# acbull/pyHGT

Hardware: NVIDIA H100
Metric: HGTConv fwd edges/sec (higher is better)
Workload: dtype f32

## Files before the change

include/hgt_b200.h:

```cpp
#ifndef HGT_B200_H
#define HGT_B200_H

#include <stddef.h>
#include <stdint.h>

#ifdef __cplusplus
extern "C" {
#endif

#define HGT_RTE_MAX_LEN 240

const char* hgt_last_error(void);
int hgt_abi_version(void);
uint64_t hgt_kernel_launches(void);


int hgt_plan_workspace_bytes(int64_t n_nodes, int64_t n_edges, size_t* out_bytes);

int hgt_plan_nodes(const int64_t* node_type, int64_t n_nodes, int32_t num_types,
                   int32_t* rank, int32_t* perm, int32_t* type_count, int32_t* sorted_flag,
                   void* workspace, size_t workspace_bytes, void* stream);

int hgt_plan_edges_sort(const int64_t* edge_index, const int64_t* edge_type, const int64_t* node_type,
                        const int32_t* rank, int64_t n_nodes, int64_t n_edges,
// ... 72 lines not shown

typedef struct {
  int64_t out_off;
  int64_t ld;
} hgt_lin_cblock;

int hgt_fold_weights(const float* const* wq, const float* const* bq,
                     const float* const* wk, const float* const* bk,
                     const float* const* wv, const float* const* bv,
                     const float* relation_att, const float* relation_msg, const float* relation_pri,
                     int32_t num_types, int32_t num_relations, int32_t n_heads, int32_t d_in, int32_t d_out,
                     int32_t n_pairs, const int32_t* pair_type, const int32_t* pair_rel,
                     const int32_t* cat_row0, const int32_t* q_row0,
                     float* w_cat, float* b_cat, void* stream);

int hgt_concat_linears(const float* const* w, const float* const* b, int32_t num_types,
                       int32_t rows, int32_t cols, float* w_cat, float* b_cat, void* stream);


int hgt_typed_linear_workspace_bytes(const hgt_lin_group* h_groups, int32_t n_groups, int32_t K,
                                     int32_t cb_width, int32_t impl, size_t* out_bytes);
int hgt_typed_linear(const float* A, int64_t lda, const float* W, const float* bias, int32_t K,
                     int32_t cb_width, const hgt_lin_group* groups, const hgt_lin_group* h_groups,
                     int32_t n_groups, const hgt_lin_cblock* cblocks, float* out, int32_t impl,
                     void* workspace, size_t workspace_bytes, void* stream);
int hgt_typed_linear_presplit_workspace_bytes(const hgt_lin_group* h_groups, int32_t n_groups, int32_t K,
                                              int32_t cb_width, size_t* out_bytes);
int hgt_typed_linear_presplit(const void* a_hi, const void* a_lo, const float* W, const float* bias, int32_t K,
                              int32_t cb_width, const hgt_lin_group* groups, const hgt_lin_group* h_groups,
                              int32_t n_groups, const hgt_lin_cblock* cblocks, float* out,
                              void* workspace, size_t workspace_bytes, void* stream);
int hgt_typed_linear_bf16(const float* A, int64_t lda, const float* W, const float* bias, int32_t K,
                          int32_t cb_width, const hgt_lin_group* groups, const hgt_lin_group* h_groups,
                          int32_t n_groups, const hgt_lin_cblock* cblocks, void* out, int32_t impl,
                          void* workspace, size_t workspace_bytes, void* stream);
int hgt_typed_linear_presplit_bf16(const void* a_hi, const void* a_lo, const float* W, const float* bias, int32_t K,
                                   int32_t cb_width, const hgt_lin_group* groups, const hgt_lin_group* h_groups,
                                   int32_t n_groups, const hgt_lin_cblock* cblocks, void* out,
                                   void* workspace, size_t workspace_bytes, void* stream);
int hgt_typed_linear_bf16a(const void* A, int64_t lda, const float* W, const float* bias, int32_t K, int32_t cb_width,
                           const hgt_lin_group* groups, const hgt_lin_group* h_groups, int32_t n_groups,
                           const hgt_lin_cblock* cblocks, float* out, int32_t impl, void* workspace,
                           size_t workspace_bytes, void* stream);

int hgt_typed_linear_t24(const float* A, int64_t lda, const float* W, const float* bias, int32_t K,
                         int32_t cb_width, const hgt_lin_group* groups, const hgt_lin_group* h_groups,
                         int32_t n_groups, const hgt_lin_cblock* cblocks, float* out, int64_t t24_off, void* out24,
                         int32_t impl, void* workspace, size_t workspace_bytes, void* stream);
int hgt_typed_linear_presplit_t24(const void* a_hi, const void* a_lo, const float* W, const float* bias, int32_t K,
                                  int32_t cb_width, const hgt_lin_group* groups, const hgt_lin_group* h_groups,
                                  int32_t n_groups, const hgt_lin_cblock* cblocks, float* out, int64_t t24_off,
                                  void* out24, void* workspace, size_t workspace_bytes, void* stream);


int hgt_edge_workspace_bytes(int32_t n_split_tiles, int32_t d, int32_t n_heads, size_t* out_bytes);
int hgt_edge_forward(const float* q, const float* kv, const float* kvr,
                     const int32_t* row_ptr, const int32_t* kv_row, const int32_t* rte_row,
                     const int32_t* csr_eid, const int32_t* tiles, int32_t n_tiles, int32_t n_split_tiles,
                     const int32_t* hubs, int32_t n_hubs,
                     int64_t n_nodes, int64_t n_edges, int32_t d, int32_t n_heads, int32_t apply_gelu,
                     float* agg_out, float* att_out, float* stats_out, void* g_hi, void* g_lo,
                     void* workspace, size_t workspace_bytes, int32_t variant, const int32_t* d_tile_counts,
                     const int32_t* type_row0, int32_t num_types, const int32_t* type_active, void* stream);

int hgt_edge_backward(const float* q, const float* kv, const float* kvr, const float* agg, const float* dagg,
                      const float* stats, const int32_t* row_ptr, const int32_t* kv_row, const int32_t* rte_row,
                      const int32_t* tiles, int32_t n_tiles, int64_t n_nodes, int32_t d, int32_t n_heads,
                      int64_t kv_rows_total, int64_t kvr_rows_total,
                      float* dq, float* dkv, float* dkvr, void* workspace, size_t workspace_bytes,
                      const int32_t* d_tile_counts, void* stream);

int hgt_edge_backward_det_workspace_bytes(int32_t n_split_dst, int32_t n_split_rows, int32_t d, size_t* out_bytes);
int hgt_edge_backward_dst(const float* q, const float* kv, const float* kvr, const float* agg, const float* dagg,
                          const float* stats, const int32_t* row_ptr, const int32_t* kv_row, const int32_t* rte_row,
                          const int32_t* tiles, int32_t n_tiles, int32_t n_split, const int32_t* hubs, int32_t n_hubs,
                          int64_t n_nodes, int32_t d, int32_t n_heads, float* dq, float* D,
                          void* workspace, size_t workspace_bytes, const int32_t* d_tile_counts, void* stream);
int hgt_edge_backward_rows(const float* q, const float* dagg, const float* stats, const float* D, const float* own,
                           const float* oth, const int32_t* src_ptr, const int32_t* src_dst, const int32_t* src_oth,
                           int32_t n_rows, int64_t own_rows_total, const int32_t* tiles, int32_t n_tiles,
                           int32_t n_split, const int32_t* hubs, int32_t n_hubs, int32_t d, int32_t n_heads,
                           float* grad, void* workspace, size_t workspace_bytes, const int32_t* d_tile_counts,
                           void* stream);

int hgt_edge_forward_bf16(const float* q, const void* kv, const void* kvr,
                          const int32_t* row_ptr, const int32_t* kv_row, const int32_t* rte_row,
                          const int32_t* csr_eid, const int32_t* tiles, int32_t n_tiles, int32_t n_split_tiles,
                          const int32_t* hubs, int32_t n_hubs,
                          int64_t n_nodes, int64_t n_edges, int32_t d, int32_t n_heads, int32_t apply_gelu,
                          float* agg_out, float* att_out, float* stats_out, void* g_hi, void* g_lo,
                          void* workspace, size_t workspace_bytes, int32_t variant, const int32_t* d_tile_counts,
                          const int32_t* type_row0, int32_t num_types, const int32_t* type_active, void* stream);
int hgt_edge_forward_t24(const float* q, const void* kv, const void* kvr,
                         const int32_t* row_ptr, const int32_t* kv_row, const int32_t* rte_row,
                         const int32_t* csr_eid, const int32_t* tiles, int32_t n_tiles, int32_t n_split_tiles,
                         const int32_t* hubs, int32_t n_hubs,
                         int64_t n_nodes, int64_t n_edges, int32_t d, int32_t n_heads, int32_t apply_gelu,
                         float* agg_out, float* att_out, float* stats_out, void* g_hi, void* g_lo,
                         void* workspace, size_t workspace_bytes, int32_t variant, const int32_t* d_tile_counts,
                         const int32_t* type_row0, int32_t num_types, const int32_t* type_active, void* stream);
int hgt_edge_backward_bf16(const float* q, const void* kv, const void* kvr, const float* agg, const float* dagg,
                           const float* stats, const int32_t* row_ptr, const int32_t* kv_row, const int32_t* rte_row,
                           const int32_t* tiles, int32_t n_tiles, int64_t n_nodes, int32_t d, int32_t n_heads,
                           int64_t kv_rows_total, int64_t kvr_rows_total,
                           float* dq, float* dkv, float* dkvr, void* workspace, size_t workspace_bytes,
                           const int32_t* d_tile_counts, void* stream);
int hgt_edge_backward_dst_bf16(const float* q, const void* kv, const void* kvr, const float* agg, const float* dagg,
                               const float* stats, const int32_t* row_ptr, const int32_t* kv_row,
                               const int32_t* rte_row, const int32_t* tiles, int32_t n_tiles, int32_t n_split,
                               const int32_t* hubs, int32_t n_hubs, int64_t n_nodes, int32_t d, int32_t n_heads,
                               float* dq, float* D, void* workspace, size_t workspace_bytes,
                               const int32_t* d_tile_counts, void* stream);
int hgt_edge_backward_rows_bf16(const float* q, const float* dagg, const float* stats, const float* D, const void* own,
                                const void* oth, const int32_t* src_ptr, const int32_t* src_dst,
                                const int32_t* src_oth, int32_t n_rows, int64_t own_rows_total, const int32_t* tiles,
                                int32_t n_tiles, int32_t n_split, const int32_t* hubs, int32_t n_hubs, int32_t d,
                                int32_t n_heads, float* grad, void* workspace, size_t workspace_bytes,
                                const int32_t* d_tile_counts, void* stream);

int hgt_edge_att_grad_workspace_bytes(int32_t n_split, int32_t n_heads, size_t* out_bytes);
int hgt_edge_att_grad_prep(const float* att, const float* datt, const int32_t* csr_eid, const int32_t* row_ptr,
                           const int32_t* tiles, int32_t n_tiles, int32_t n_split, const int32_t* hubs, int32_t n_hubs,
                           int64_t n_nodes, int32_t n_heads, float* c_att, float* datt_csr, void* workspace,
                           size_t workspace_bytes, const int32_t* d_tile_counts, void* stream);
int hgt_edge_backward_att(const float* q, const float* kv, const float* kvr, const float* agg, const float* dagg,
                          const float* stats, const float* datt_csr, const float* c_att, const int32_t* row_ptr,
                          const int32_t* kv_row, const int32_t* rte_row, const int32_t* tiles, int32_t n_tiles,
                          int64_t n_nodes, int32_t d, int32_t n_heads, int64_t kv_rows_total, int64_t kvr_rows_total,
                          float* dq, float* dkv, float* dkvr, void* workspace, size_t workspace_bytes,
                          const int32_t* d_tile_counts, void* stream);
int hgt_edge_backward_dst_att(const float* q, const float* kv, const float* kvr, const float* agg, const float* dagg,
                              const float* stats, const float* datt_csr, const float* c_att, const int32_t* row_ptr,
                              const int32_t* kv_row, const int32_t* rte_row, const int32_t* tiles, int32_t n_tiles,
                              int32_t n_split, const int32_t* hubs, int32_t n_hubs, int64_t n_nodes, int32_t d,
                              int32_t n_heads, float* dq, float* D, void* workspace, size_t workspace_bytes,
                              const int32_t* d_tile_counts, void* stream);
int hgt_edge_backward_rows_att(const float* q, const float* dagg, const float* stats, const float* D,
                               const float* datt_csr, const float* own, const float* oth, const int32_t* src_ptr,
                               const int32_t* src_dst, const int32_t* src_oth, const int32_t* src_pos, int32_t n_rows,
                               int64_t own_rows_total, const int32_t* tiles, int32_t n_tiles, int32_t n_split,
                               const int32_t* hubs, int32_t n_hubs, int32_t d, int32_t n_heads, float* grad,
                               void* workspace, size_t workspace_bytes, const int32_t* d_tile_counts, void* stream);
int hgt_edge_backward_att_bf16(const float* q, const void* kv, const void* kvr, const float* agg, const float* dagg,
                               const float* stats, const float* datt_csr, const float* c_att, const int32_t* row_ptr,
                               const int32_t* kv_row, const int32_t* rte_row, const int32_t* tiles, int32_t n_tiles,
                               int64_t n_nodes, int32_t d, int32_t n_heads, int64_t kv_rows_total,
                               int64_t kvr_rows_total, float* dq, float* dkv, float* dkvr, void* workspace,
                               size_t workspace_bytes, const int32_t* d_tile_counts, void* stream);
int hgt_edge_backward_dst_att_bf16(const float* q, const void* kv, const void* kvr, const float* agg, const float* dagg,
                                   const float* stats, const float* datt_csr, const float* c_att,
                                   const int32_t* row_ptr, const int32_t* kv_row, const int32_t* rte_row,
                                   const int32_t* tiles, int32_t n_tiles, int32_t n_split, const int32_t* hubs,
                                   int32_t n_hubs, int64_t n_nodes, int32_t d, int32_t n_heads, float* dq, float* D,
// ... 354 lines not shown
```

pyhgt_b200/_lib.py:

```python
import ctypes
import os

import numpy as np

HERE = os.path.dirname(os.path.abspath(__file__))
LIB_PATH = os.path.join(HERE, "libhgt_b200.so")

_c = ctypes
_p = _c.c_void_p
_i32 = _c.c_int32
_i64 = _c.c_int64
_sz = _c.c_size_t
_f32 = _c.c_float

SIGNATURES = {
    "hgt_abi_version": [],
    "hgt_plan_workspace_bytes": [_i64, _i64, _c.POINTER(_sz)],
    "hgt_plan_nodes": [_p, _i64, _i32, _p, _p, _p, _p, _p, _sz, _p],
    "hgt_plan_edges_sort": [_p, _p, _p, _p, _i64, _i64, _i32, _i32, _p, _p, _p, _p, _p, _sz, _p],
    "hgt_plan_edges_fill": [_p, _p, _p, _p, _p, _p, _i64, _i64, _i32, _i32, _p, _p, _p, _i32, _i32, _p, _p, _p, _p],
    "hgt_plan_tiles": [_p, _i64, _i64, _i32, _i32, _p, _i64, _p, _i64, _p, _c.POINTER(_i32), _p, _sz, _p],
    "hgt_gather_rows": [_p, _p, _i64, _i32, _p, _p],
    "hgt_halo_pull": [_c.c_uint64, _p, _p, _i64, _i32, _i64, _p, _p],
    "hgt_halo_pull_split": [_c.c_uint64, _p, _p, _p, _i64, _i32, _i32, _i64, _p, _p, _p, _p],
    "hgt_halo_push_split": [_p, _p, _p, _p, _i64, _i32, _i32, _i64, _c.c_uint64, _c.c_uint64, _p, _p],
    "hgt_fold_weights": [_p, _p, _p, _p, _p, _p, _p, _p, _p, _i32, _i32, _i32, _i32, _i32, _i32, _p, _p, _p, _p,
                         _p, _p, _p],
    "hgt_concat_linears": [_p, _p, _i32, _i32, _i32, _p, _p, _p],
    "hgt_typed_linear_workspace_bytes": [_p, _i32, _i32, _i32, _i32, _c.POINTER(_sz)],
    "hgt_typed_linear": [_p, _i64, _p, _p, _i32, _i32, _p, _p, _i32, _p, _p, _i32, _p, _sz, _p],
    "hgt_edge_workspace_bytes": [_i32, _i32, _i32, _c.POINTER(_sz)],
    "hgt_edge_forward": [_p, _p, _p, _p, _p, _p, _p, _p, _i32, _i32, _p, _i32, _i64, _i64, _i32, _i32, _i32, _p, _p,
                         _p, _p, _p, _p, _sz, _i32, _p, _p, _i32, _p, _p],
    "hgt_typed_linear_presplit_workspace_bytes": [_p, _i32, _i32, _i32, _c.POINTER(_sz)],
    "hgt_typed_linear_presplit": [_p, _p, _p, _p, _i32, _i32, _p, _p, _i32, _p, _p, _p, _sz, _p],
    "hgt_edge_backward": [_p, _p, _p, _p, _p, _p, _p, _p, _p, _p, _i32, _i64, _i32, _i32, _i64, _i64, _p, _p, _p, _p, _sz,
                          _p, _p],
    "hgt_typed_linear_bwd_workspace_bytes": [_p, _i32, _p, _i32, _i32, _i64, _i64, _i32, _i32, _i32, _c.POINTER(_sz)],
    "hgt_typed_linear_bwd": [_p, _p, _p, _i64, _p, _i64, _p, _p, _p, _i32, _i32, _p, _p, _i32, _p, _p, _i32, _p, _p, _p,
                             _i32, _p, _sz, _p],
    "hgt_act_split": [_p, _i64, _i64, _i32, _i32, _p, _p, _p, _p],
    "hgt_update_backward": [_p, _p, _p, _p, _i32, _p, _p, _p, _p, _i64, _i32, _p, _p, _p, _p, _p, _p],
    "hgt_fold_backward": [_p, _p, _p, _p, _p, _p, _p, _p, _p, _i32, _i32, _i32, _i32, _i32, _i32, _p, _p, _p, _p, _p, _p,
                          _p, _p, _p, _p, _p],
    "hgt_conv_workspace_bytes": [_p, _c.POINTER(_sz)],
    "hgt_conv_forward": [_p, _p, _sz, _p],
    "hgt_update_epilogue": [_p, _p, _p, _i32, _p, _p, _p, _p, _p, _i64, _i32, _p, _p, _p, _p],
    "hgt_plan_dst_end": [_p, _p, _p, _i64, _i32, _p, _p],
    "hgt_update_epilogue_dst": [_p, _p, _p, _i32, _p, _p, _p, _p, _p, _p, _i64, _i32, _p, _p, _p, _p],
    "hgt_plan_source_index": [_p, _p, _p, _i64, _i64, _i32, _p, _p, _p, _p, _sz, _p],
    "hgt_plan_source_index_pos": [_p, _p, _p, _i64, _i64, _i32, _p, _p, _p, _p, _p, _sz, _p],
    "hgt_edge_backward_det_workspace_bytes": [_i32, _i32, _i32, _c.POINTER(_sz)],
    "hgt_edge_backward_dst": [_p, _p, _p, _p, _p, _p, _p, _p, _p, _p, _i32, _i32, _p, _i32, _i64, _i32, _i32, _p, _p, _p,
                              _sz, _p, _p],
    "hgt_edge_backward_rows": [_p, _p, _p, _p, _p, _p, _p, _p, _p, _i32, _i64, _p, _i32, _i32, _p, _i32, _i32, _i32, _p,
                               _p, _sz, _p, _p],
    "hgt_typed_linear_bwd_det_workspace_bytes": [_p, _i32, _p, _i32, _i32, _i64, _i64, _i32, _i32, _i32,
                                                 _c.POINTER(_sz)],
    "hgt_typed_linear_bwd_det": [_p, _p, _p, _i64, _p, _i64, _p, _p, _p, _i32, _i32, _p, _p, _i32, _p, _p, _i32, _p, _p,
                                 _p, _i32, _p, _sz, _p],
    "hgt_update_backward_det_workspace_bytes": [_i64, _i32, _i32, _c.POINTER(_sz)],
    "hgt_update_backward_det": [_p, _p, _p, _p, _i32, _p, _p, _p, _p, _i64, _i32, _p, _p, _p, _p, _p, _p, _sz, _p],
    "hgt_fold_backward_det": [_p, _p, _p, _p, _p, _p, _p, _p, _p, _i32, _i32, _i32, _i32, _i32, _i32, _p, _p, _p, _p, _p,
                              _p, _p, _p, _p, _p, _p],
    "hgt_typed_linear_bf16": [_p, _i64, _p, _p, _i32, _i32, _p, _p, _i32, _p, _p, _i32, _p, _sz, _p],
    "hgt_typed_linear_presplit_bf16": [_p, _p, _p, _p, _i32, _i32, _p, _p, _i32, _p, _p, _p, _sz, _p],
    "hgt_typed_linear_t24": [_p, _i64, _p, _p, _i32, _i32, _p, _p, _i32, _p, _p, _i64, _p, _i32, _p, _sz, _p],
    "hgt_typed_linear_presplit_t24": [_p, _p, _p, _p, _i32, _i32, _p, _p, _i32, _p, _p, _i64, _p, _p, _sz, _p],
    "hgt_edge_forward_bf16": [_p, _p, _p, _p, _p, _p, _p, _p, _i32, _i32, _p, _i32, _i64, _i64, _i32, _i32, _i32, _p, _p,
                              _p, _p, _p, _p, _sz, _i32, _p, _p, _i32, _p, _p],
    "hgt_edge_forward_t24": [_p, _p, _p, _p, _p, _p, _p, _p, _i32, _i32, _p, _i32, _i64, _i64, _i32, _i32, _i32, _p, _p,
                             _p, _p, _p, _p, _sz, _i32, _p, _p, _i32, _p, _p],
    "hgt_edge_backward_bf16": [_p, _p, _p, _p, _p, _p, _p, _p, _p, _p, _i32, _i64, _i32, _i32, _i64, _i64, _p, _p, _p, _p,
                               _sz, _p, _p],
    "hgt_edge_backward_dst_bf16": [_p, _p, _p, _p, _p, _p, _p, _p, _p, _p, _i32, _i32, _p, _i32, _i64, _i32, _i32, _p, _p,
                                   _p, _sz, _p, _p],
    "hgt_edge_backward_rows_bf16": [_p, _p, _p, _p, _p, _p, _p, _p, _p, _i32, _i64, _p, _i32, _i32, _p, _i32, _i32, _i32,
                                    _p, _p, _sz, _p, _p],
    "hgt_edge_att_grad_workspace_bytes": [_i32, _i32, _c.POINTER(_sz)],
    "hgt_edge_att_grad_prep": [_p, _p, _p, _p, _p, _i32, _i32, _p, _i32, _i64, _i32, _p, _p, _p, _sz, _p, _p],
    "hgt_edge_backward_att": [_p, _p, _p, _p, _p, _p, _p, _p, _p, _p, _p, _p, _i32, _i64, _i32, _i32, _i64, _i64, _p, _p,
                              _p, _p, _sz, _p, _p],
    "hgt_edge_backward_dst_att": [_p, _p, _p, _p, _p, _p, _p, _p, _p, _p, _p, _p, _i32, _i32, _p, _i32, _i64, _i32, _i32,
                                  _p, _p, _p, _sz, _p, _p],
    "hgt_edge_backward_rows_att": [_p, _p, _p, _p, _p, _p, _p, _p, _p, _p, _p, _i32, _i64, _p, _i32, _i32, _p, _i32, _i32,
                                   _i32, _p, _p, _sz, _p, _p],
    "hgt_edge_backward_att_bf16": [_p, _p, _p, _p, _p, _p, _p, _p, _p, _p, _p, _p, _i32, _i64, _i32, _i32, _i64, _i64, _p,
                                   _p, _p, _p, _sz, _p, _p],
    "hgt_edge_backward_dst_att_bf16": [_p, _p, _p, _p, _p, _p, _p, _p, _p, _p, _p, _p, _i32, _i32, _p, _i32, _i64, _i32,
                                       _i32, _p, _p, _p, _sz, _p, _p],
    "hgt_edge_backward_rows_att_bf16": [_p, _p, _p, _p, _p, _p, _p, _p, _p, _p, _p, _i32, _i64, _p, _i32, _i32, _p, _i32,
                                        _i32, _i32, _p, _p, _sz, _p, _p],
    "hgt_gsample_batch_add_budget_workspace_bytes": [_i32, _i64, _i32, _i64, _c.POINTER(_sz)],
    "hgt_gsample_batch_add_budget": [_p, _p, _p, _i32, _p, _p, _p, _p, _i64, _p, _i64, _i32, _i64, _i64, _p, _p, _sz,
                                     _p],
    "hgt_gsample_batch_select_workspace_bytes": [_i32, _i64, _c.POINTER(_sz)],
    "hgt_gsample_batch_select": [_p, _p, _p, _p, _i64, _i64, _i64, _p, _p, _p, _p, _p, _sz, _p],
    "hgt_gsample_rebuild_workspace_bytes": [_i64, _c.POINTER(_sz)],
    "hgt_gsample_batch_rebuild_count": [_p, _p, _i32, _p, _p, _i64, _i64, _p, _p, _p, _p, _p, _sz, _p],
    "hgt_gsample_batch_rebuild_write": [_p, _p, _i32, _p, _p, _p, _p, _p, _p, _p, _i64, _p, _i64, _p, _i32, _p, _p, _p,
                                        _p, _p, _p, _p],
    "hgt_host_register": [_p, _sz, _c.POINTER(_p)],
    "hgt_host_unregister": [_p],
    "hgt_gsample_gather_features_bf16": [_p, _i32, _p, _p, _i64, _p, _p],
    "hgt_gsample_batch_rebuild_count_host": [_p, _p, _i32, _p, _p, _i64, _i64, _p, _p, _i64, _p, _p, _p, _p, _p, _sz,
                                             _p],
    "hgt_gsample_batch_rebuild_write_host": [_p, _p, _i32, _p, _p, _p, _p, _p, _p, _p, _i64, _p, _i64, _p, _i64, _p,
                                             _i32, _p, _p, _p, _p, _p, _p, _p],
    "hgt_gsample_hash_insert_seeds": [_p, _i64, _p, _p, _p, _p, _p, _p],
    "hgt_gsample_hash_add_budget": [_p, _p, _p, _i32, _p, _p, _p, _p, _i64, _p, _i64, _i32, _i64, _i64, _p, _p, _sz,
                                    _p],
    "hgt_gsample_hash_select_workspace_bytes": [_i32, _i64, _c.POINTER(_sz)],
    "hgt_gsample_hash_select": [_p, _p, _p, _p, _i64, _i64, _i64, _p, _p, _p, _p, _p, _sz, _p],
    "hgt_gsample_hash_rebuild_count": [_p, _p, _i32, _p, _p, _i64, _i64, _p, _p, _p, _p, _p, _sz, _p],
    "hgt_gsample_hash_rebuild_write": [_p, _p, _i32, _p, _p, _p, _p, _p, _p, _p, _i64, _p, _i64, _p, _i32, _p, _p, _p,
                                       _p, _p, _p, _p],
    "hgt_gsample_hash_rebuild_count_host": [_p, _p, _i32, _p, _p, _i64, _i64, _p, _p, _i64, _p, _p, _p, _p, _p, _sz,
                                            _p],
    "hgt_gsample_hash_rebuild_write_host": [_p, _p, _i32, _p, _p, _p, _p, _p, _p, _p, _i64, _p, _i64, _p, _i64, _p,
                                            _i32, _p, _p, _p, _p, _p, _p, _p],
    "hgt_merge_batches": [_p, _i32, _i32, _p, _p, _i64, _i64, _i64, _i32, _p, _p, _p, _p, _p, _p, _p],
    "hgt_gsample_gather_rows_bf16": [_p, _i32, _p, _p, _i64, _p, _p],
    "hgt_merge_batches_bf16": [_p, _i32, _i32, _p, _p, _i64, _i64, _i64, _i32, _p, _p, _p, _p, _p, _p, _p],
    "hgt_typed_linear_bf16a": [_p, _i64, _p, _p, _i32, _i32, _p, _p, _i32, _p, _p, _i32, _p, _sz, _p],
    "hgt_typed_linear_bwd_bf16a": [_p, _i64, _p, _i64, _i32, _i32, _p, _p, _i32, _p, _p, _p, _i32, _p, _sz, _p],
# ... 35 lines not shown
    _fields_ = ([(n, ctypes.c_int64) for n in _I64] + [(n, ctypes.c_int32) for n in _I32] +
                [(n, ctypes.c_void_p) for n in _PTR])


LIN_GROUP_DTYPE = np.dtype([("a_row0", "<i8"), ("m", "<i8"), ("w_row0", "<i4"), ("n_cblocks", "<i4"),
                            ("cb_first", "<i4"), ("has_bias", "<i4")])
LIN_CBLOCK_DTYPE = np.dtype([("out_off", "<i8"), ("ld", "<i8")])
assert LIN_GROUP_DTYPE.itemsize == 32 and LIN_CBLOCK_DTYPE.itemsize == 16

_lib = None


class HgtError(RuntimeError):
    pass


def load():
    global _lib
    if _lib is not None:
        return _lib
    if not os.path.exists(LIB_PATH):
        raise HgtError("libhgt_b200.so not found at %s — run `python -m pyhgt_b200.build` "
                       "(or __graft_entry__.build()); there is no CPU fallback" % LIB_PATH)
    lib = ctypes.CDLL(LIB_PATH)
    lib.hgt_last_error.restype = _c.c_char_p
    lib.hgt_last_error.argtypes = []
    for name, args in SIGNATURES.items():
        fn = getattr(lib, name)
        fn.restype = _c.c_int
        fn.argtypes = args
    lib.hgt_kernel_launches.restype = _c.c_uint64
    lib.hgt_kernel_launches.argtypes = []
    lib.hgt_conv_args_size.restype = _c.c_uint64
    lib.hgt_conv_args_size.argtypes = []
    lib.hgt_sampler_budget_update.restype = _c.c_int64
    lib.hgt_sampler_budget_update.argtypes = [_p, _p, _i64, _i64, _i64, _i64, _i64, _p, _p, _p, _p, _p, _p, _p]
    lib.hgt_sampler_add_budget.restype = _c.c_int64
    lib.hgt_sampler_add_budget.argtypes = [_p, _p, _i64, _p, _c.c_int32, _p, _c.c_int32, _i64, _p, _p, _i64, _i64, _p]
    _lib = lib
    return lib


def check(rc, what):
    if rc != 0:
        msg = load().hgt_last_error()
        raise HgtError("%s failed (code %d): %s" % (what, rc, msg.decode() if msg else "?"))


def call(name, *args):
    lib = load()
    check(getattr(lib, name)(*args), name)


def kernel_launches():
    return int(load().hgt_kernel_launches())


def ptr(t):
    return None if t is None else t.data_ptr()
```

pyhgt_b200/conv.py:

```python
import ctypes
import math

import torch
import torch.nn as nn
import torch.nn.functional as F

from . import _lib
from . import plan as _plan


def glorot(tensor):
    if tensor is not None:
        a = math.sqrt(6.0 / (tensor.size(-2) + tensor.size(-1)))
        tensor.data.uniform_(-a, a)


class RelTemporalEncoding(nn.Module):

    def __init__(self, n_hid, max_len=240, dropout=0.2):
        super().__init__()
        position = torch.arange(0., max_len).unsqueeze(1)
        div_term = torch.exp(torch.arange(0, n_hid, 2) * -(math.log(10000.0) / n_hid))
        emb = nn.Embedding(max_len, n_hid)
        emb.weight.data[:, 0::2] = torch.sin(position * div_term) / math.sqrt(n_hid)
        emb.weight.data[:, 1::2] = torch.cos(position * div_term) / math.sqrt(n_hid)
        emb.requires_grad = False
        self.emb = emb
        self.lin = nn.Linear(n_hid, n_hid)

    def forward(self, x, t):
        return x + self.lin(self.emb(t))


def _stream():
    return torch.cuda.current_stream().cuda_stream


_TABLE_SUFFIX = {torch.float32: "", torch.bfloat16: "_bf16", torch.uint8: "_t24"}


def _output_rows(rows, d, dev, lt, out_map):
    if lt.type_active_dev is not None and out_map is None:
        return torch.zeros((rows, d), dtype=torch.float32, device=dev)
    return torch.empty((rows, d), dtype=torch.float32, device=dev)


def _split_hint(node_inp, x, N, d_in, impl):
    hint = getattr(node_inp, "_hgt_split", None)
    if (hint is None or hint[2] != node_inp._version or x is not node_inp or tuple(hint[0].shape) != (N, d_in)
            or d_in % 16 or d_in < 64 or (hint[1] is None and impl != 3)):
        return None
    return (hint[0], None if impl == 3 else hint[1])


class _PointerTable:

    def __init__(self):
        self.key = None
        self.dev = None

    def get(self, tensors, device):
        key = tuple(t.data_ptr() for t in tensors) + (str(device),)
        if key != self.key:
            if torch.device(device).type == "cuda" and torch.cuda.is_current_stream_capturing():
                raise _lib.HgtError("a parameter moved while a CUDA graph was being captured: run the step once eagerly "
                                    "(warm-up) so the pointer tables match the parameters the graph will use")
            self.dev = torch.tensor([t.data_ptr() for t in tensors], dtype=torch.int64).to(device)
            self.key = key
        return self.dev


class HGTConv(nn.Module):
    keep_att = True
    recompute_tables = False
    fused_dropout = False
    edge_variant = 0
    linear_impl = 0
    event_sink = None
    _has_skip = True
    emit_split = False
    fused_call = True

    def __init__(self, in_dim, out_dim, num_types, num_relations, n_heads, dropout=0.2, use_norm=True,
                 use_RTE=True, **kwargs):
        super().__init__()
        self.in_dim = in_dim
        self.out_dim = out_dim
        self.num_types = num_types
        self.num_relations = num_relations
        self.total_rel = num_types * num_relations * num_types
        self.n_heads = n_heads
# ... 9 lines not shown
        self.a_linears = nn.ModuleList()
        self.norms = nn.ModuleList()
        for _ in range(num_types):
            self.k_linears.append(nn.Linear(in_dim, out_dim))
            self.q_linears.append(nn.Linear(in_dim, out_dim))
            self.v_linears.append(nn.Linear(in_dim, out_dim))
            self.a_linears.append(nn.Linear(out_dim, out_dim))
            if use_norm:
                self.norms.append(nn.LayerNorm(out_dim))
        self.relation_pri = nn.Parameter(torch.ones(num_relations, self.n_heads))
        self.relation_att = nn.Parameter(torch.Tensor(num_relations, n_heads, self.d_k, self.d_k))
        self.relation_msg = nn.Parameter(torch.Tensor(num_relations, n_heads, self.d_k, self.d_k))
        if self._has_skip:
            self.skip = nn.Parameter(torch.ones(num_types))
        self.drop = nn.Dropout(dropout)
        if self.use_RTE:
            self.emb = RelTemporalEncoding(in_dim)
        glorot(self.relation_att)
        glorot(self.relation_msg)
        self._ptr_tables = {}

    def __repr__(self):
        return '{}(in_dim={}, out_dim={}, num_types={}, num_types={})'.format(
            self.__class__.__name__, self.in_dim, self.out_dim, self.num_types, self.num_relations)

    def __getstate__(self):
        state = self.__dict__.copy()
        state.pop("_args_cache", None)
        state["_ptr_tables"] = {}
        if state.get("att") is not None:
            state["att"] = state["att"].detach()
        return state

    def _ptrs(self, name, tensors, device):
        tab = self._ptr_tables.get(name)
        if tab is None:
            tab = self._ptr_tables[name] = _PointerTable()
        return tab.get(tensors, device)

    @staticmethod
    def _stage(name):
        class _T:
            def __enter__(self_):
                self_.on = HGTConv.event_sink is not None
                if self_.on:
                    self_.a, self_.b = torch.cuda.Event(enable_timing=True), torch.cuda.Event(enable_timing=True)
                    self_.a.record()
            def __exit__(self_, *exc):
                if self_.on:
                    self_.b.record()
                    HGTConv.event_sink.append((name, self_.a, self_.b))
        return _T()

    def _typed_linear(self, a, lda, w, bias, k, width, table, out, impl, st, out32=None, t24_off=0):
        g_dev, g_host, n_g, c_dev = table
        ws_bytes = ctypes.c_size_t()
        _lib.call("hgt_typed_linear_workspace_bytes", g_host.ctypes.data, n_g, k, width, impl, ctypes.byref(ws_bytes))
        ws = torch.empty(max(ws_bytes.value, 1), dtype=torch.uint8, device=out.device)
        outs = (_lib.ptr(out32), t24_off, out.data_ptr()) if out.dtype == torch.uint8 else (out.data_ptr(),)
        fn = "hgt_typed_linear_bf16a" if a.dtype == torch.bfloat16 else "hgt_typed_linear" + _TABLE_SUFFIX[out.dtype]
        _lib.call(fn, a.data_ptr(), lda, w.data_ptr(), _lib.ptr(bias), k, width, g_dev.data_ptr(),
                  g_host.ctypes.data, n_g, c_dev.data_ptr(), *outs, impl, ws.data_ptr(), ws.numel(), st)

    def _check_inputs(self, node_inp, edge_time):
        if node_inp.device.type != "cuda":
            raise _lib.HgtError("pyhgt_b200.HGTConv runs on CUDA tensors only (got %s): there is no CPU "
                                "fallback" % node_inp.device)
        if node_inp.dtype != torch.float32:
            raise ValueError("node_inp must be float32 (the reference is fp32 throughout), got %s" % node_inp.dtype)
        if node_inp.dim() != 2 or node_inp.shape[1] != self.in_dim:
            raise ValueError("node_inp must be [N, %d], got %s" % (self.in_dim, tuple(node_inp.shape)))
        if self.in_dim != self.out_dim:
            raise ValueError("HGTConv needs in_dim == out_dim for the skip connection (conv.py:131)")
        if self.use_RTE and edge_time is None:
            raise ValueError("use_RTE=True needs edge_time (conv.py:91-92)")
        if self.out_dim % self.n_heads != 0:
            raise ValueError("out_dim=%d is not divisible by n_heads=%d" % (self.out_dim, self.n_heads))

    def forward(self, node_inp, node_type, edge_index, edge_type, edge_time=None):
        self._check_inputs(node_inp, edge_time)
        if torch.is_grad_enabled() and (node_inp.requires_grad or any(p.requires_grad for p in self.parameters())):
            from .autograd import hgt_conv_autograd
            return hgt_conv_autograd(self, node_inp, node_type, edge_index, edge_type, edge_time)
        out, att, _ = self._forward_impl(node_inp, node_type, edge_index, edge_type, edge_time,
                                         want_att=self.keep_att, save=False)
        self.att = att
        return out

    def _forward_view(self, node_inp, view, edge_time):
        self._check_inputs(node_inp, edge_time)
        self.att = None
        if torch.is_grad_enabled() and (node_inp.requires_grad or any(p.requires_grad for p in self.parameters())):
            from .autograd import hgt_conv_autograd
            return hgt_conv_autograd(self, node_inp, None, None, None, None, active=view.active,
                                     kv_runs=view.kv_runs, plan=view.plan, want_att=False)
        out, _, _ = self._forward_impl(node_inp, None, None, None, None, want_att=False, save=False,
                                       active_per_type=view.active, kv_runs=view.kv_runs, plan=view.plan)
        return out

    def _forward_fused(self, node_inp, node_type, edge_index, edge_type, edge_time, want_att,
                       active_per_type=None, out_map=None, out_rows=None, x_split=None, kv_runs=None, plan=None, impl=None,
                       dst=False):
        if impl is None:
            impl = self.linear_impl
        dev = node_inp.device
        d_in, d, H, T, R = self.in_dim, self.out_dim, self.n_heads, self.num_types, self.num_relations
        if plan is None:
            plan = _plan.get_plan(node_type, edge_index, edge_type, edge_time if self.use_RTE else None, T, R)
        N, E = plan.n_nodes, plan.n_edges
        if node_inp.shape[0] != N:
            raise ValueError("node_inp has %d rows but node_type has %d" % (node_inp.shape[0], N))
        lt = _plan.layer_tables(plan, d_in, d, active_per_type, kv_runs, dst)
        tabs = [self._ptrs("wq", [l.weight for l in self.q_linears], dev),
# ... 113 lines not shown
                          drop_seed(o.device).data_ptr(), p_fused, st)
            elif lt.type_dst_dev is not None:
                _lib.call("hgt_update_epilogue_dst", o.data_ptr(), x_sorted.data_ptr(), plan.type_row0_dev.data_ptr(), T,
                          self.skip.data_ptr(), _lib.ptr(norm_w), _lib.ptr(norm_b), perm_ptr, lt.type_dst_dev.data_ptr(),
                          c["ba_cat"].data_ptr(), N, d, out.data_ptr(), _lib.ptr(o_hi), _lib.ptr(o_lo), st)
            else:
                _lib.call("hgt_update_epilogue", o.data_ptr(), x_sorted.data_ptr(), plan.type_row0_dev.data_ptr(), T,
                          self.skip.data_ptr(), _lib.ptr(norm_w), _lib.ptr(norm_b), perm_ptr,
                          _lib.ptr(lt.type_active_dev), N, d, out.data_ptr(), _lib.ptr(o_hi), _lib.ptr(o_lo), st)
        if o_hi is not None:
            out._hgt_split = (o_hi, o_lo, out._version)
        return out, c["att"], (c if save else None)

    def _core(self, node_inp, node_type, edge_index, edge_type, edge_time, want_att, save, active_per_type,
              gelu_before_a, x_split=None, kv_runs=None, bf16=False, plan=None, impl=None, dst=False):
        if impl is None:
            impl = self.linear_impl
        one = impl == 3
        dev = node_inp.device
        d_in, d = self.in_dim, self.out_dim
        H, T, R = self.n_heads, self.num_types, self.num_relations
        st = _stream()
        if plan is None:
            plan = _plan.get_plan(node_type, edge_index, edge_type, edge_time if self.use_RTE else None, T, R)
        N, E, P = plan.n_nodes, plan.n_edges, plan.n_pairs
        if node_inp.shape[0] != N:
            raise ValueError("node_inp has %d rows but node_type has %d" % (node_inp.shape[0], N))
        lt = _plan.layer_tables(plan, d_in, d, active_per_type, kv_runs, dst)
        f32 = dict(dtype=torch.float32, device=dev)
        x = node_inp.contiguous()
        if x_split is None and plan.sorted_types and impl != 1:
            x_split = _split_hint(node_inp, x, N, d_in, impl)
        if plan.sorted_types:
            x_sorted = x
        else:
            with self._stage("gather_rows"):
                x_sorted = torch.empty_like(x)
                _lib.call("hgt_gather_rows", x.data_ptr(), plan.perm.data_ptr(), N, d_in, x_sorted.data_ptr(), st)

        w_cat = torch.empty((max(lt.cat_rows, 1), d_in), **f32)
        b_cat = torch.empty(max(lt.cat_rows, 1), **f32)
        wq = self._ptrs("wq", [l.weight for l in self.q_linears], dev)
        bq = self._ptrs("bq", [l.bias for l in self.q_linears], dev)
        wk = self._ptrs("wk", [l.weight for l in self.k_linears], dev)
        bk = self._ptrs("bk", [l.bias for l in self.k_linears], dev)
        wv = self._ptrs("wv", [l.weight for l in self.v_linears], dev)
        bv = self._ptrs("bv", [l.bias for l in self.v_linears], dev)
        _lib.call("hgt_fold_weights", wq.data_ptr(), bq.data_ptr(), wk.data_ptr(), bk.data_ptr(), wv.data_ptr(),
                  bv.data_ptr(), self.relation_att.data_ptr(), self.relation_msg.data_ptr(),
                  self.relation_pri.data_ptr(), T, R, H, d_in, d, P, plan.pair_type_dev.data_ptr(),
                  plan.pair_rel_dev.data_ptr(), lt.cat_row0_dev.data_ptr(), lt.q_row0_dev.data_ptr(),
                  w_cat.data_ptr(), b_cat.data_ptr(), st)

        t24 = not save and not bf16 and d % 8 == 0
        tab_dtype = torch.bfloat16 if bf16 else torch.uint8 if t24 else torch.float32
        row_len = 2 * d * (3 if t24 else 1)
        proj = None
        if bf16:
            q_tab = torch.empty(N * d, **f32)
            kv_tab = torch.empty((plan.kv_rows + 1) * row_len, dtype=tab_dtype, device=dev)
            calls = ((lt.q_groups, q_tab, None), (lt.kv_groups, kv_tab, None))
        elif t24:
            q_buf = torch.empty(lt.kv_off, **f32)
            q_tab = q_buf[lt.q_off:lt.q_off + N * d]
            kv_tab = torch.empty((plan.kv_rows + 1) * row_len, dtype=tab_dtype, device=dev)
            calls = ((lt.proj_groups, kv_tab, q_buf),)
        else:
            proj = torch.empty(lt.proj_elems, **f32)
            q_tab = proj[lt.q_off:lt.q_off + N * d]
            kv_tab = proj[lt.kv_off:]
            calls = ((lt.proj_groups, proj, None),)
        kv_tab[plan.kv_rows * row_len:].zero_()
        with self._stage("proj_linear"):
            xs = x_split if plan.sorted_types else None
            for tab, out, out32 in calls:
                if xs is None:
                    self._typed_linear(x_sorted, d_in, w_cat, b_cat, d_in, d, tab, out, impl, st, out32, lt.kv_off)
                    continue
                g_dev, g_host, n_g, c_dev = tab
                wsb = ctypes.c_size_t()
                _lib.call("hgt_typed_linear_presplit_workspace_bytes", g_host.ctypes.data, n_g, d_in, d,
                          ctypes.byref(wsb))
                ws1 = torch.empty(max(wsb.value, 1), dtype=torch.uint8, device=dev)
                outs = (out32.data_ptr(), lt.kv_off, out.data_ptr()) if t24 else (out.data_ptr(),)
                _lib.call("hgt_typed_linear_presplit" + _TABLE_SUFFIX[out.dtype], xs[0].data_ptr(),
                          None if one else _lib.ptr(xs[1]), w_cat.data_ptr(), b_cat.data_ptr(), d_in, d, g_dev.data_ptr(),
                          g_host.ctypes.data, n_g, c_dev.data_ptr(), *outs, ws1.data_ptr(), ws1.numel(), st)
        kvr = None
        if self.use_RTE:
            rt = torch.empty((_plan.RTE_MAX_LEN, d_in), **f32)
            self._typed_linear(self.emb.emb.weight, d_in, self.emb.lin.weight, self.emb.lin.bias, d_in, d_in,
                               lt.rt_group, rt, 1, st)
            kvr = torch.empty((P * _plan.RTE_MAX_LEN + 1) * row_len, dtype=tab_dtype, device=dev)
            kvr[P * _plan.RTE_MAX_LEN * row_len:].zero_()
            self._typed_linear(rt, d_in, w_cat, None, d_in, d, lt.rte_groups, kvr, 1, st)

        ws_bytes = ctypes.c_size_t()
        _lib.call("hgt_edge_workspace_bytes", plan.n_split, d, H, ctypes.byref(ws_bytes))
        ws = torch.empty(ws_bytes.value, dtype=torch.uint8, device=dev)
        fuse_split = (gelu_before_a and not save and impl != 1 and d % 16 == 0 and d >= 64
                      and not (self.training and self.drop.p > 0))
        g_act = None if fuse_split else torch.empty((N, d), **f32)
        g_hi = torch.empty((N, d), dtype=torch.bfloat16, device=dev) if fuse_split else None
        g_lo = torch.empty((N, d), dtype=torch.bfloat16, device=dev) if fuse_split and not one else None
        att = torch.empty((E, H), **f32) if want_att else None
        stats = torch.empty((N, 2 * H), **f32) if save else None
        with self._stage("edge"):
            _lib.call("hgt_edge_forward" + _TABLE_SUFFIX[tab_dtype], q_tab.data_ptr(), kv_tab.data_ptr(), _lib.ptr(kvr), plan.row_ptr.data_ptr(),
                      plan.kv_row.data_ptr(), _lib.ptr(plan.rte_row) if self.use_RTE else None,
                      plan.csr_eid.data_ptr(), plan.tiles.data_ptr(), plan.n_tiles, plan.n_split,
                      plan.hubs.data_ptr(), plan.n_hubs, N, E, d, H, 1 if (gelu_before_a and not save) else 0,
                      _lib.ptr(g_act), _lib.ptr(att), _lib.ptr(stats), _lib.ptr(g_hi), _lib.ptr(g_lo), ws.data_ptr(),
                      ws.numel(), self.edge_variant, _lib.ptr(plan.tile_counts_dev), plan.type_row0_dev.data_ptr(), T,
                      _lib.ptr(lt.type_active_dev if lt.type_dst_dev is None else lt.type_dst_dev), st)

        agg = None
        if save or not gelu_before_a:
            agg = g_act
            g_act = F.gelu(agg) if gelu_before_a else agg
        wa_cat = torch.empty((T * d, d), **f32)
        ba_cat = torch.empty(T * d, **f32)
        wa = self._ptrs("wa", [l.weight for l in self.a_linears], dev)
        ba = self._ptrs("ba", [l.bias for l in self.a_linears], dev)
        _lib.call("hgt_concat_linears", wa.data_ptr(), ba.data_ptr(), T, d, d, wa_cat.data_ptr(), ba_cat.data_ptr(), st)
        o = torch.empty((N, d), **f32)
        with self._stage("upd_linear"):
            if fuse_split:
                g_dev, g_host, n_g, c_dev = lt.upd_groups
                wsb = ctypes.c_size_t()
                _lib.call("hgt_typed_linear_presplit_workspace_bytes", g_host.ctypes.data, n_g, d, d, ctypes.byref(wsb))
                ws2 = torch.empty(max(wsb.value, 1), dtype=torch.uint8, device=dev)
                _lib.call("hgt_typed_linear_presplit", g_hi.data_ptr(), _lib.ptr(g_lo), wa_cat.data_ptr(),
                          ba_cat.data_ptr(), d, d, g_dev.data_ptr(), g_host.ctypes.data, n_g, c_dev.data_ptr(),
                          o.data_ptr(), ws2.data_ptr(), ws2.numel(), st)
            else:
                self._typed_linear(g_act, d, wa_cat, ba_cat, d, d, lt.upd_groups, o, impl, st)
        if self.training and self.drop.p > 0 and not self.fused_dropout:
            o = self.drop(o)
        return dict(plan=plan, lt=lt, x_sorted=x_sorted, w_cat=w_cat, proj=proj, q=q_tab, kv=kv_tab, kvr=kvr, agg=agg, o=o, stats=stats,
                    att=att, N=N, d=d, T=T, st=st, ba_cat=ba_cat)


class DenseHGTConv(HGTConv):
    _has_skip = False

    def __init__(self, in_dim, out_dim, num_types, num_relations, n_heads, dropout=0.2, use_norm=True,
                 use_RTE=True, **kwargs):
        super().__init__(in_dim, out_dim, num_types, num_relations, n_heads, dropout, use_norm, use_RTE, **kwargs)
        self.mid_linear = nn.Linear(out_dim, out_dim * 2)
        self.out_linear = nn.Linear(out_dim * 2, out_dim)
        self.out_norm = nn.LayerNorm(out_dim)

    def forward(self, node_inp, node_type, edge_index, edge_type, edge_time=None):
        self._check_inputs(node_inp, edge_time)
        from .autograd import dense_hgt_forward
        return dense_hgt_forward(self, node_inp, node_type, edge_index, edge_type, edge_time)


class GeneralConv(nn.Module):

    def __init__(self, conv_name, in_hid, out_hid, num_types, num_relations, n_heads, dropout, use_norm=True,
# ... 14 lines not shown
```

pyhgt_b200/csrc/common.cuh:

```cuda
#pragma once
#include <cuda_runtime.h>
#include <curand_philox4x32_x.h>
#include <stdint.h>
#include <stdio.h>
#include <stdarg.h>

#include "hgt_b200.h"

#define HGT_SM_COUNT_FALLBACK 132

void hgt_set_error(const char* fmt, ...);
int hgt_sm_count();

#define HGT_CHECK_CUDA(expr)                                                                      \
  do {                                                                                            \
    cudaError_t _e = (expr);                                                                      \
    if (_e != cudaSuccess) {                                                                      \
      hgt_set_error("%s:%d: %s failed: %s", __FILE__, __LINE__, #expr, cudaGetErrorString(_e));   \
      return 2;                                                                                   \
    }                                                                                             \
  } while (0)

#define HGT_REQUIRE(cond, ...)                                                                    \
  do {                                                                                            \
    if (!(cond)) {                                                                                \
      hgt_set_error(__VA_ARGS__);                                                                 \
      return 1;                                                                                   \
    }                                                                                             \
  } while (0)

extern unsigned long long g_hgt_launches;
#define HGT_LAUNCH_CHECK()                  \
  do {                                      \
    ++g_hgt_launches;                       \
    HGT_CHECK_CUDA(cudaGetLastError());     \
  } while (0)

static inline size_t hgt_align_up(size_t x, size_t a) { return (x + a - 1) / a * a; }

__device__ __forceinline__ float hgt_gelu_erf(float x) {
  return 0.5f * x * (1.0f + erff(x * 0.70710678118654752440f));
}

struct hgt_t24 {};

__host__ __device__ __forceinline__ uint32_t hgt_t24_round(uint32_t b) {
  const uint32_t r = (b + 0x7fu + ((b >> 8) & 1u)) & 0xffffff00u;
  return (b & 0x7fffffffu) > 0x7f800000u ? ((b | 0x00400000u) & 0xffffff00u) : r;
}

struct hgt_t24_at {
  unsigned char* hi;
  unsigned char* lo;
  __host__ __device__ __forceinline__ hgt_t24_at(void* base, int64_t off, int64_t ld) {
    const int64_t row = off / ld, col = off - row * ld;
    hi = static_cast<unsigned char*>(base) + row * 3 * ld + 2 * col;
    lo = static_cast<unsigned char*>(base) + row * 3 * ld + 2 * ld + col;
  }
};

struct HgtDrop {
  uint32_t thr;
  float scale;
  float keep;
};
static inline HgtDrop hgt_drop_params(float p) {
  HgtDrop r;
  if (p >= 1.0f) {
    r.thr = 0xffffffffu;
    r.scale = r.keep = 0.f;
  } else {
    r.thr = (uint32_t)((double)p * 4294967296.0);
    r.keep = 1.0f - p;
    r.scale = 1.0f / r.keep;
  }
  return r;
}

__device__ __forceinline__ uint2 hgt_drop_key(const uint64_t* __restrict__ seed) {
  const uint64_t s = *seed;
  return make_uint2((uint32_t)s, (uint32_t)(s >> 32));
}

__device__ __forceinline__ uint32_t hgt_drop_keep4(uint2 key, uint64_t q, uint32_t thr) {
  const uint4 r = curand_Philox4x32_10(make_uint4((uint32_t)q, (uint32_t)(q >> 32), 0u, 0u), key);
  return (uint32_t)(r.x >= thr) | ((uint32_t)(r.y >= thr) << 1) | ((uint32_t)(r.z >= thr) << 2) |
         ((uint32_t)(r.w >= thr) << 3);
}

template <int NPL>
__device__ __forceinline__ uint32_t hgt_drop_row_bits(uint2 key, int64_t row, int d, uint32_t thr, int lane) {
  const int nchunk = (d + 3) >> 2;
  uint32_t bits = 0;
#pragma unroll
  for (int i0 = 0; i0 < NPL; i0 += 4) {
    const int chunk = (lane >> 2) + 8 * (i0 + (lane & 3));
    const uint32_t mine = chunk < nchunk ? hgt_drop_keep4(key, (uint64_t)row * nchunk + chunk, thr) : 0u;
#pragma unroll
    for (int j = 0; j < 4; ++j) {
      const uint32_t theirs = __shfl_sync(0xffffffffu, mine, (lane & ~3) + j);
      if (i0 + j < NPL) bits |= ((theirs >> (lane & 3)) & 1u) << (i0 + j);
    }
  }
  return bits;
}

__device__ __forceinline__ float hgt_drop_apply(float v, uint32_t kept, float scale) { return kept ? v * scale : 0.f; }
```

pyhgt_b200/csrc/edge.cu:

```cuda
#include <cuda_bf16.h>

#include <type_traits>

#include "common.cuh"

namespace {

constexpr int kWarpsPerCta = 16;
constexpr int kCtaThreads = kWarpsPerCta * 32;

struct EdgeParams {
  const float* q;
  const void* kv;
  const void* kvr;
  const int32_t* row_ptr;
  const int32_t* kv_row;
  const int32_t* rte_row;
  const int32_t* csr_eid;
  const int32_t* tiles;
  int32_t n_tiles;
  const int32_t* d_counts;
  const int32_t* type_row0;
  const int32_t* type_active;
  int32_t T;
// ... 36 lines not shown
  if constexpr (VEC == 4) {
    asm volatile("ld.global.nc.L1::no_allocate.v4.f32 {%0,%1,%2,%3}, [%4];"
                 : "=f"(dst[0]), "=f"(dst[1]), "=f"(dst[2]), "=f"(dst[3]) : "l"(p));
  } else if constexpr (VEC == 2) {
    asm volatile("ld.global.nc.L1::no_allocate.v2.f32 {%0,%1}, [%2];" : "=f"(dst[0]), "=f"(dst[1]) : "l"(p));
  } else {
    asm volatile("ld.global.nc.L1::no_allocate.f32 %0, [%1];" : "=f"(dst[0]) : "l"(p));
  }
}
__device__ __forceinline__ float bf16_lo(uint32_t u) { return __uint_as_float(u << 16); }
__device__ __forceinline__ float bf16_hi(uint32_t u) { return __uint_as_float(u & 0xffff0000u); }

template <int VEC>
__device__ __forceinline__ void load_vec(float (&dst)[VEC], const __nv_bfloat16* p) {
  if constexpr (VEC == 4) {
    const uint2 u = *reinterpret_cast<const uint2*>(p);
    dst[0] = bf16_lo(u.x); dst[1] = bf16_hi(u.x); dst[2] = bf16_lo(u.y); dst[3] = bf16_hi(u.y);
  } else if constexpr (VEC == 2) {
    const uint32_t u = *reinterpret_cast<const uint32_t*>(p);
    dst[0] = bf16_lo(u); dst[1] = bf16_hi(u);
  } else {
    dst[0] = __bfloat162float(*p);
  }
}
template <int VEC>
__device__ __forceinline__ void load_vec_nc(float (&dst)[VEC], const __nv_bfloat16* p) {
  if constexpr (VEC == 4) {
    uint32_t a, b;
    asm volatile("ld.global.nc.L1::no_allocate.v2.b32 {%0,%1}, [%2];" : "=r"(a), "=r"(b) : "l"(p));
    dst[0] = bf16_lo(a); dst[1] = bf16_hi(a); dst[2] = bf16_lo(b); dst[3] = bf16_hi(b);
  } else if constexpr (VEC == 2) {
    uint32_t a;
    asm volatile("ld.global.nc.L1::no_allocate.b32 %0, [%1];" : "=r"(a) : "l"(p));
    dst[0] = bf16_lo(a); dst[1] = bf16_hi(a);
  } else {
    unsigned short a;
    asm volatile("ld.global.nc.L1::no_allocate.b16 %0, [%1];" : "=h"(a) : "l"(p));
    dst[0] = __uint_as_float((uint32_t)a << 16);
  }
}

template <int VEC>
__device__ __forceinline__ void t24_decode(float (&dst)[VEC], uint32_t h0, uint32_t h1, uint32_t l) {
  const uint32_t z0 = l << 8;
  dst[0] = __uint_as_float(__byte_perm(h0, z0, 0x1054));
  if constexpr (VEC >= 2) dst[1] = __uint_as_float(__byte_perm(h0, z0, 0x3264));
  if constexpr (VEC == 4) {
    const uint32_t z1 = l >> 8;
    dst[2] = __uint_as_float(__byte_perm(h1, z1, 0x1057));
    dst[3] = __uint_as_float(__byte_perm(h1, z1, 0x3267));
  }
}

template <class KV> constexpr int64_t kv_elem_bytes() { return std::is_same<KV, hgt_t24>::value ? 3 : sizeof(KV); }

template <class KV, int VEC, bool NC>
__device__ __forceinline__ void load_kv(float (&dst)[VEC], const unsigned char* row, int e, int n) {
  if constexpr (std::is_same<KV, hgt_t24>::value) {
    const unsigned char* hp = row + 2 * e;
    const unsigned char* lp = row + 2 * n + e;
    uint32_t h0 = 0, h1 = 0, l = 0;
    if constexpr (NC) {
      if constexpr (VEC == 4) {
        asm volatile("ld.global.nc.L1::no_allocate.v2.b32 {%0,%1}, [%2];" : "=r"(h0), "=r"(h1) : "l"(hp));
        asm volatile("ld.global.nc.L1::no_allocate.b32 %0, [%1];" : "=r"(l) : "l"(lp));
      } else if constexpr (VEC == 2) {
        asm volatile("ld.global.nc.L1::no_allocate.b32 %0, [%1];" : "=r"(h0) : "l"(hp));
        asm volatile("ld.global.nc.L1::no_allocate.u16 %0, [%1];" : "=r"(l) : "l"(lp));
      } else {
        asm volatile("ld.global.nc.L1::no_allocate.u16 %0, [%1];" : "=r"(h0) : "l"(hp));
        asm volatile("ld.global.nc.L1::no_allocate.u8 %0, [%1];" : "=r"(l) : "l"(lp));
      }
    } else {
      if constexpr (VEC == 4) {
        const uint2 h = *reinterpret_cast<const uint2*>(hp);
        h0 = h.x; h1 = h.y;
        l = *reinterpret_cast<const uint32_t*>(lp);
      } else if constexpr (VEC == 2) {
        h0 = *reinterpret_cast<const uint32_t*>(hp);
        l = *reinterpret_cast<const uint16_t*>(lp);
      } else {
        h0 = *reinterpret_cast<const uint16_t*>(hp);
        l = *lp;
      }
    }
    t24_decode<VEC>(dst, h0, h1, l);
  } else {
    const KV* p = reinterpret_cast<const KV*>(row) + e;
    if constexpr (NC) load_vec_nc<VEC>(dst, p);
    else load_vec<VEC>(dst, p);
  }
}

template <int VEC>
__device__ __forceinline__ void store_vec(float* p, const float (&src)[VEC]) {
  using V = typename VecT<VEC>::type;
  V v;
  float* f = reinterpret_cast<float*>(&v);
#pragma unroll
  for (int i = 0; i < VEC; ++i) f[i] = src[i];
  *reinterpret_cast<V*>(p) = v;
}

template <int VEC>
__device__ __forceinline__ void store_split_bf16(__nv_bfloat16* hi, __nv_bfloat16* lo, const float (&src)[VEC]) {
  __nv_bfloat16 h[VEC], l[VEC];
#pragma unroll
  for (int i = 0; i < VEC; ++i) {
    h[i] = __float2bfloat16_rn(src[i]);
    l[i] = __float2bfloat16_rn(src[i] - __bfloat162float(h[i]));
  }
  if constexpr (VEC == 4) {
    *reinterpret_cast<uint2*>(hi) = *reinterpret_cast<uint2*>(h);
    if (lo) *reinterpret_cast<uint2*>(lo) = *reinterpret_cast<uint2*>(l);
  } else if constexpr (VEC == 2) {
    *reinterpret_cast<uint32_t*>(hi) = *reinterpret_cast<uint32_t*>(h);
    if (lo) *reinterpret_cast<uint32_t*>(lo) = *reinterpret_cast<uint32_t*>(l);
  } else {
    hi[0] = h[0];
    if (lo) lo[0] = l[0];
  }
}

__device__ __forceinline__ float head_reduce(float v, int lph) {
  for (int o = lph >> 1; o > 0; o >>= 1) v += __shfl_xor_sync(0xffffffffu, v, o);
  return v;
}

template <int VEC, int NCH>
struct LaneState {
  float m, l;
  float acc[NCH][VEC];
  __device__ __forceinline__ void reset() {
    m = -INFINITY;
    l = 0.f;
#pragma unroll
    for (int t = 0; t < NCH; ++t)
#pragma unroll
      for (int v = 0; v < VEC; ++v) acc[t][v] = 0.f;
// ... 13 lines not shown
  }
  template <int VEC>
  __device__ __forceinline__ int off(int t) const {
    int o = (sub + t * lph) * VEC;
    return (head_ok && o < dk) ? base + o : -1;
  }
};

template <int VEC, int NCH>
__device__ __forceinline__ void finalize_destination(const EdgeParams& p, const LaneMap& lm, int lane, int dst,
                                                      LaneState<VEC, NCH>& st, int seg_begin, int seg_end,
                                                      bool split_piece, int pslot) {
  if (split_piece) {
    float* w = p.partial + (int64_t)pslot * partial_stride(p.H, p.d);
    if (lm.head_ok && lm.sub == 0) { w[lm.h] = st.m; w[p.H + lm.h] = st.l; }
#pragma unroll
    for (int t = 0; t < NCH; ++t) {
      int o = lm.off<VEC>(t);
      if (o >= 0) store_vec<VEC>(w + partial_acc_off(p.H) + o, st.acc[t]);
    }
    return;
  }
  const float inv = 1.0f / (st.l + 1e-16f);
  float* orow = p.agg_out + (int64_t)dst * p.d;
#pragma unroll
  for (int t = 0; t < NCH; ++t) {
    int o = lm.off<VEC>(t);
    if (o >= 0) {
      float r[VEC];
#pragma unroll
      for (int v = 0; v < VEC; ++v) {
        float x = st.acc[t][v] * inv;
        r[v] = p.apply_gelu ? hgt_gelu_erf(x) : x;
      }
      if (p.agg_out) store_vec<VEC>(orow + o, r);
      if (p.g_hi) store_split_bf16<VEC>(p.g_hi + (int64_t)dst * p.d + o, p.g_lo ? p.g_lo + (int64_t)dst * p.d + o : nullptr, r);
    }
  }
  if (p.stats_out && lm.head_ok && lm.sub == 0) {
    p.stats_out[(int64_t)dst * 2 * p.H + lm.h] = st.m;
    p.stats_out[(int64_t)dst * 2 * p.H + p.H + lm.h] = st.l;
  }
  if (p.att_out && lm.head_ok && lm.sub == 0) {
    for (int c = seg_begin; c < seg_end; ++c) {
      float* a = p.att_out + (int64_t)p.csr_eid[c] * p.H + lm.h;
      *a = __expf(*a - st.m) * inv;
    }
  }
}

template <class KV, int VEC, int NCH>
__global__ void __launch_bounds__(kCtaThreads, 1)
k_edge_fwd_ldg(EdgeParams p) {
  constexpr int W = std::is_same<KV, hgt_t24>::value ? 2 * NCH * VEC : NCH * VEC;
  constexpr int EDGE_UNROLL = (W >= 32) ? 1 : (W >= 16 ? 2 : 4);
  const int lane = threadIdx.x & 31;
  const LaneMap lm(p, lane);
  const unsigned char* const kvt = static_cast<const unsigned char*>(p.kv);
  const unsigned char* const kvrt = static_cast<const unsigned char*>(p.kvr);
  const bool rte = kvrt != nullptr;
  const int n = 2 * p.d;
  const int64_t row_bytes = n * kv_elem_bytes<KV>();
  int offs[NCH];
#pragma unroll
  for (int t = 0; t < NCH; ++t) offs[t] = lm.off<VEC>(t);

  const int n_tiles = p.d_counts ? p.d_counts[0] : p.n_tiles;
  for (;;) {
    int tile = 0;
    if (lane == 0) tile = atomicAdd(p.tile_counter, 1);
    tile = __shfl_sync(0xffffffffu, tile, 0);
    if (tile >= n_tiles) break;
    const int4 tl = reinterpret_cast<const int4*>(p.tiles)[tile];
    const bool split = tl.y < 0;
    const int d_begin = tl.x, d_end = split ? tl.x + 1 : tl.y;
    int seg_begin = tl.z;
    for (int dst = d_begin; dst < d_end; ++dst) {
      const int seg_end = split ? tl.w : p.row_ptr[dst + 1];
      if (p.type_active && seg_end == seg_begin && dst_inactive(p, dst)) continue;
      LaneState<VEC, NCH> st;
      st.reset();
      if (seg_end > seg_begin) {
        float q[NCH][VEC];
        const float* qrow = p.q + (int64_t)dst * p.d;
#pragma unroll
        for (int t = 0; t < NCH; ++t) {
          if (offs[t] >= 0) load_vec<VEC>(q[t], qrow + offs[t]);
          else {
#pragma unroll
            for (int v = 0; v < VEC; ++v) q[t][v] = 0.f;
          }
        }
        for (int c0 = seg_begin; c0 < seg_end; c0 += EDGE_UNROLL) {
          float kk[EDGE_UNROLL][NCH][VEC], vv[EDGE_UNROLL][NCH][VEC];
          int nb = min(EDGE_UNROLL, seg_end - c0);
#pragma unroll
          for (int u = 0; u < EDGE_UNROLL; ++u) {
            if (u < nb) {
              const unsigned char* row = kvt + (int64_t)p.kv_row[c0 + u] * row_bytes;
#pragma unroll
              for (int t = 0; t < NCH; ++t) {
                if (offs[t] >= 0) {
                  load_kv<KV, VEC, true>(kk[u][t], row, offs[t], n);
                  load_kv<KV, VEC, true>(vv[u][t], row, p.d + offs[t], n);
                } else {
#pragma unroll
                  for (int v = 0; v < VEC; ++v) { kk[u][t][v] = 0.f; vv[u][t][v] = 0.f; }
                }
              }
            }
          }
          if (rte) {
#pragma unroll
            for (int u = 0; u < EDGE_UNROLL; ++u) {
              if (u < nb) {
// ... 50 lines not shown
              for (int u = 0; u < EDGE_UNROLL; ++u)
                if (u < nb) a = fmaf(pw[u], vv[u][t][v], a);
              st.acc[t][v] = a;
            }
        }
      }
      finalize_destination<VEC, NCH>(p, lm, lane, dst, st, seg_begin, seg_end, split, split ? -tl.y - 1 : 0);
      seg_begin = seg_end;
    }
  }
}

__device__ __forceinline__ uint32_t smem_u32(const void* p) {
  return static_cast<uint32_t>(__cvta_generic_to_shared(p));
}
__device__ __forceinline__ void mbar_init(uint32_t bar, uint32_t count) {
  asm volatile("mbarrier.init.shared::cta.b64 [%0], %1;" ::"r"(bar), "r"(count) : "memory");
}
__device__ __forceinline__ void mbar_expect_tx(uint32_t bar, uint32_t bytes) {
  asm volatile("mbarrier.arrive.expect_tx.shared::cta.b64 _, [%0], %1;" ::"r"(bar), "r"(bytes) : "memory");
}
__device__ __forceinline__ bool mbar_try_wait(uint32_t bar, uint32_t parity) {
  uint32_t ok;
  asm volatile(
      "{\n\t"
      ".reg .pred p;\n\t"
      "mbarrier.try_wait.parity.shared::cta.b64 p, [%1], %2;\n\t"
      "selp.u32 %0, 1, 0, p;\n\t"
      "}"
      : "=r"(ok) : "r"(bar), "r"(parity) : "memory");
  return ok != 0;
}
__device__ __forceinline__ void mbar_wait(uint32_t bar, uint32_t parity) {
  while (!mbar_try_wait(bar, parity)) {}
}
__device__ __forceinline__ void bulk_g2s(uint32_t dst_smem, const void* src_gmem, uint32_t bytes, uint32_t bar) {
  asm volatile("cp.async.bulk.shared::cluster.global.mbarrier::complete_tx::bytes [%0], [%1], %2, [%3];" ::"r"(
                   dst_smem), "l"(src_gmem), "r"(bytes), "r"(bar)
               : "memory");
}

template <class KV, int VEC, int NCH>
__global__ void __launch_bounds__(kCtaThreads, (VEC * NCH <= 4) ? 2 : 1)
k_edge_fwd_tma(EdgeParams p) {
  extern __shared__ __align__(128) unsigned char smem_raw[];
  const int lane = threadIdx.x & 31;
  const int warp = threadIdx.x >> 5;
  const LaneMap lm(p, lane);
  const unsigned char* const kvt = static_cast<const unsigned char*>(p.kv);
  const unsigned char* const kvrt = static_cast<const unsigned char*>(p.kvr);
  const bool rte = kvrt != nullptr;
  const int S = p.stages;
  const int n = 2 * p.d;
  const uint32_t row_bytes = (uint32_t)(n * kv_elem_bytes<KV>());
  const uint32_t slot_bytes = rte ? 2u * row_bytes : row_bytes;
  unsigned char* ring = smem_raw + (size_t)warp * S * slot_bytes;
  uint64_t* bars = reinterpret_cast<uint64_t*>(smem_raw + (size_t)kWarpsPerCta * S * slot_bytes) + warp * S;
  if (lane == 0) {
    for (int s = 0; s < S; ++s) mbar_init(smem_u32(&bars[s]), 1);
    asm volatile("fence.mbarrier_init.release.cluster;" ::: "memory");
  }
  __syncwarp();
  int offs[NCH];
#pragma unroll
  for (int t = 0; t < NCH; ++t) offs[t] = lm.off<VEC>(t);

  uint32_t it = 0;

  const int n_tiles = p.d_counts ? p.d_counts[0] : p.n_tiles;
  for (;;) {
    int tile = 0;
    if (lane == 0) tile = atomicAdd(p.tile_counter, 1);
    tile = __shfl_sync(0xffffffffu, tile, 0);
    if (tile >= n_tiles) break;
    const int4 tl = reinterpret_cast<const int4*>(p.tiles)[tile];
    const bool split = tl.y < 0;
    const int d_begin = tl.x, d_end = split ? tl.x + 1 : tl.y;
    const int e0 = tl.z;
    const int e1 = tl.w;
    int ibase = e0;
    int idxA = (ibase + lane < e1) ? p.kv_row[ibase + lane] : 0;
    int idxB = (ibase + 32 + lane < e1) ? p.kv_row[ibase + 32 + lane] : 0;
    int ridxA = 0, ridxB = 0;
    if (rte) {
      ridxA = (ibase + lane < e1) ? p.rte_row[ibase + lane] : 0;
      ridxB = (ibase + 32 + lane < e1) ? p.rte_row[ibase + 32 + lane] : 0;
    }
    uint32_t issue_it = it;
    auto issue = [&](int c) {
      while (c - ibase >= 32) {
        ibase += 32;
        idxA = idxB;
        idxB = (ibase + 32 + lane < e1) ? p.kv_row[ibase + 32 + lane] : 0;
        if (rte) {
          ridxA = ridxB;
          ridxB = (ibase + 32 + lane < e1) ? p.rte_row[ibase + 32 + lane] : 0;
        }
      }
      const int row = __shfl_sync(0xffffffffu, idxA, c - ibase);
      const int rrow = rte ? __shfl_sync(0xffffffffu, ridxA, c - ibase) : 0;
      const uint32_t slot = issue_it % S;
      if (lane == 0) {
        const uint32_t bar = smem_u32(&bars[slot]);
        const uint32_t dst = smem_u32(ring + (size_t)slot * slot_bytes);
        mbar_expect_tx(bar, slot_bytes);
        bulk_g2s(dst, kvt + (int64_t)row * row_bytes, row_bytes, bar);
        if (rte) bulk_g2s(dst + row_bytes, kvrt + (int64_t)rrow * row_bytes, row_bytes, bar);
// ... 179 lines not shown
extern "C" int hgt_edge_workspace_bytes(int32_t n_split_tiles, int32_t d, int32_t n_heads, size_t* out_bytes) {
  HGT_REQUIRE(out_bytes, "hgt_edge_workspace_bytes: out_bytes is NULL");
  *out_bytes = 256 + sizeof(float) * (size_t)(n_split_tiles > 0 ? n_split_tiles : 0) * partial_stride(n_heads, d);
  return 0;
}

extern "C" int hgt_edge_forward(const float* q, const float* kv, const float* kvr, const int32_t* row_ptr,
                                const int32_t* kv_row, const int32_t* rte_row, const int32_t* csr_eid,
                                const int32_t* tiles, int32_t n_tiles, int32_t n_split_tiles, const int32_t* hubs,
                                int32_t n_hubs, int64_t n_nodes,
                                int64_t n_edges, int32_t d, int32_t n_heads, int32_t apply_gelu, float* agg_out,
                                float* att_out, float* stats_out, void* g_hi, void* g_lo, void* workspace,
                                size_t workspace_bytes, int32_t variant, const int32_t* d_tile_counts,
                                const int32_t* type_row0, int32_t num_types, const int32_t* type_active,
                                void* stream_) {
  (void)n_edges;
  return edge_forward<float>(q, kv, kvr, row_ptr, kv_row, rte_row, csr_eid, tiles, n_tiles, n_split_tiles, hubs, n_hubs,
                             n_nodes, d, n_heads, apply_gelu, agg_out, att_out, stats_out, g_hi, g_lo, workspace,
                             workspace_bytes, variant, d_tile_counts, type_row0, num_types, type_active,
                             (cudaStream_t)stream_);
}

extern "C" int hgt_edge_forward_bf16(const float* q, const void* kv, const void* kvr, const int32_t* row_ptr,
                                     const int32_t* kv_row, const int32_t* rte_row, const int32_t* csr_eid,
                                     const int32_t* tiles, int32_t n_tiles, int32_t n_split_tiles, const int32_t* hubs,
                                     int32_t n_hubs, int64_t n_nodes, int64_t n_edges, int32_t d, int32_t n_heads,
                                     int32_t apply_gelu, float* agg_out, float* att_out, float* stats_out, void* g_hi,
                                     void* g_lo, void* workspace, size_t workspace_bytes, int32_t variant,
                                     const int32_t* d_tile_counts, const int32_t* type_row0, int32_t num_types,
                                     const int32_t* type_active, void* stream_) {
  (void)n_edges;
  return edge_forward<__nv_bfloat16>(q, static_cast<const __nv_bfloat16*>(kv), static_cast<const __nv_bfloat16*>(kvr),
                                     row_ptr, kv_row, rte_row, csr_eid, tiles, n_tiles, n_split_tiles, hubs, n_hubs,
                                     n_nodes, d, n_heads, apply_gelu, agg_out, att_out, stats_out, g_hi, g_lo,
                                     workspace, workspace_bytes, variant, d_tile_counts, type_row0, num_types,
                                     type_active, (cudaStream_t)stream_);
}

extern "C" int hgt_edge_forward_t24(const float* q, const void* kv, const void* kvr, const int32_t* row_ptr,
                                    const int32_t* kv_row, const int32_t* rte_row, const int32_t* csr_eid,
                                    const int32_t* tiles, int32_t n_tiles, int32_t n_split_tiles, const int32_t* hubs,
                                    int32_t n_hubs, int64_t n_nodes, int64_t n_edges, int32_t d, int32_t n_heads,
                                    int32_t apply_gelu, float* agg_out, float* att_out, float* stats_out, void* g_hi,
                                    void* g_lo, void* workspace, size_t workspace_bytes, int32_t variant,
                                    const int32_t* d_tile_counts, const int32_t* type_row0, int32_t num_types,
                                    const int32_t* type_active, void* stream_) {
  (void)n_edges;
  return edge_forward<hgt_t24>(q, static_cast<const hgt_t24*>(kv), static_cast<const hgt_t24*>(kvr), row_ptr, kv_row,
                               rte_row, csr_eid, tiles, n_tiles, n_split_tiles, hubs, n_hubs, n_nodes, d, n_heads,
                               apply_gelu, agg_out, att_out, stats_out, g_hi, g_lo, workspace, workspace_bytes, variant,
                               d_tile_counts, type_row0, num_types, type_active, (cudaStream_t)stream_);
}

namespace {

template <class KV>
int edge_forward(const float* q, const KV* kv, const KV* kvr, const int32_t* row_ptr, const int32_t* kv_row,
                 const int32_t* rte_row, const int32_t* csr_eid, const int32_t* tiles, int32_t n_tiles,
                 int32_t n_split_tiles, const int32_t* hubs, int32_t n_hubs, int64_t n_nodes, int32_t d,
                 int32_t n_heads, int32_t apply_gelu, float* agg_out, float* att_out, float* stats_out, void* g_hi,
                 void* g_lo, void* workspace, size_t workspace_bytes, int32_t variant, const int32_t* d_tile_counts,
                 const int32_t* type_row0, int32_t num_types, const int32_t* type_active, cudaStream_t st) {
  HGT_REQUIRE(n_heads >= 1 && n_heads <= 32, "hgt_edge_forward: n_heads=%d unsupported (1..32)", n_heads);
  HGT_REQUIRE(d % n_heads == 0, "hgt_edge_forward: d=%d not divisible by n_heads=%d", d, n_heads);
  HGT_REQUIRE((kvr != nullptr) == (rte_row != nullptr), "hgt_edge_forward: kvr and rte_row must go together");
  HGT_REQUIRE((g_hi != nullptr || g_lo == nullptr) && (agg_out != nullptr || g_hi != nullptr),
              "hgt_edge_forward: need agg_out and/or g_hi (g_lo only with g_hi)");
  HGT_REQUIRE(g_hi == nullptr || d % 8 == 0, "hgt_edge_forward: split output needs d %% 8 == 0 (d=%d)", d);
  size_t need = 0;
  hgt_edge_workspace_bytes(n_split_tiles, d, n_heads, &need);
  HGT_REQUIRE(workspace_bytes >= need, "hgt_edge_forward: workspace too small (%zu < %zu)", workspace_bytes, need);
  if (n_nodes == 0 || n_tiles == 0) return 0;

  EdgeParams p;
  p.q = q; p.kv = kv; p.kvr = kvr; p.row_ptr = row_ptr; p.kv_row = kv_row; p.rte_row = rte_row;
  p.csr_eid = csr_eid; p.tiles = tiles; p.n_tiles = n_tiles; p.d_counts = d_tile_counts; p.d = d;
  p.type_row0 = type_row0; p.type_active = (type_row0 && num_types > 0) ? type_active : nullptr; p.T = num_types; p.H = n_heads; p.DK = d / n_heads;
  int hp = 1, shift = 5;
  while (hp < n_heads) hp <<= 1;
  p.LPH = 32 / hp;
  for (shift = 0; (1 << shift) < p.LPH; ++shift) {}
  p.lph_shift = shift;
  p.apply_gelu = apply_gelu;
  p.agg_out = agg_out; p.att_out = att_out; p.stats_out = stats_out;
  p.g_hi = reinterpret_cast<__nv_bfloat16*>(g_hi); p.g_lo = reinterpret_cast<__nv_bfloat16*>(g_lo);
  p.tile_counter = reinterpret_cast<int32_t*>(workspace);
  p.partial = reinterpret_cast<float*>(reinterpret_cast<char*>(workspace) + 256);

  int vec = 1;
  for (int v : {4, 2}) {
    if (p.DK % v == 0 && p.DK / v >= p.LPH) { vec = v; break; }
  }
  int chunks = (p.DK + vec * p.LPH - 1) / (vec * p.LPH);
  int nch = 1;
  while (nch < chunks) nch <<= 1;
  HGT_REQUIRE(nch <= 8, "hgt_edge_forward: head width d_k=%d with %d heads needs %d chunks per lane (max 8)",
              p.DK, n_heads, chunks);

  const int sms = hgt_sm_count();
  int grid = sms;
  size_t smem = 0;
  HGT_REQUIRE((!std::is_same<KV, hgt_t24>::value || d % 8 == 0), "hgt_edge_forward_t24: needs d %% 8 == 0 (d=%d)", d);
  const size_t row_bytes = 2 * (size_t)d * kv_elem_bytes<KV>();
  const size_t slot_bytes = kvr ? 2 * row_bytes : row_bytes;
  if (variant == 0) variant = 2;
  const bool two_ctas = vec * nch <= 4;
  if (variant == 2) {
    const size_t budget = two_ctas ? 100 * 1024 : 200 * 1024;
    int stages = (int)(budget / (kWarpsPerCta * slot_bytes));
    if (stages > 8) stages = 8;
    if (stages < 2 || row_bytes % 16 != 0) variant = 1;
    else {
      p.stages = stages;
      smem = (size_t)kWarpsPerCta * stages * (slot_bytes + 8);
    }
  }
  HGT_REQUIRE(variant == 1 || variant == 2, "hgt_edge_forward: unknown variant %d", variant);
  if (two_ctas && variant == 2) grid = 2 * sms;
  int max_ctas = (n_tiles + kWarpsPerCta - 1) / kWarpsPerCta;
  if (grid > max_ctas) grid = max_ctas;
  HGT_CHECK_CUDA(cudaMemsetAsync(p.tile_counter, 0, sizeof(int32_t), st));
  int rc;
  if (vec == 4) rc = dispatch_nch<KV, 4>(p, nch, variant, grid, smem, st);
  else if (vec == 2) rc = dispatch_nch<KV, 2>(p, nch, variant, grid, smem, st);
  else rc = dispatch_nch<KV, 1>(p, nch, variant, grid, smem, st);
  if (rc) return rc;
  if (n_split_tiles > 0) {
    HGT_REQUIRE(hubs != nullptr && n_hubs > 0, "hgt_edge_forward: split tiles present but no hub list given");
    k_merge_partials<<<n_hubs < 4 * sms ? n_hubs : 4 * sms, kMergeThreads, 0, st>>>(p, hubs, n_hubs);
    HGT_LAUNCH_CHECK();
  }
  return 0;
}

}
```

pyhgt_b200/csrc/layer.cu:

```cuda
#include "common.cuh"

int hgt_update_epilogue_impl(const float* o, const float* x, const int32_t* type_row0, int32_t num_types,
                             const float* skip, const float* norm_w, const float* norm_b, const float* const* norm_wp,
                             const float* const* norm_bp, const int32_t* perm, const int32_t* type_active,
                             const int32_t* type_dst, const float* bias, int64_t n_nodes, int32_t d, float* out,
                             void* out_hi, void* out_lo, const uint64_t* seed, float p, cudaStream_t st);
bool hgt_typed_linear_tc_supported(int64_t lda, int32_t K, int32_t cb_width);

namespace {

struct Carver {
  char* base;
  size_t off = 0;
  explicit Carver(void* b) : base(reinterpret_cast<char*>(b)) {}
  template <typename T>
  T* take(size_t count) {
    size_t o = off;
    off += hgt_align_up(count * sizeof(T), 256);
    return base ? reinterpret_cast<T*>(base + o) : nullptr;
  }
  void* take_bytes(size_t bytes) { return take<char>(bytes); }
};

struct Layout {
  float *x_sorted, *w_cat, *b_cat, *proj, *rt, *g_act, *wa_cat, *ba_cat, *o;
  void *kv, *kvr;
  void *g_hi, *g_lo, *ws_proj, *ws_edge, *ws_upd;
  size_t ws_proj_bytes, ws_edge_bytes, ws_upd_bytes, total;
  bool fuse_split, presplit_x, t24;
};

int plan_layout(const hgt_conv_args* a, void* base, Layout* L) {
  Carver c(base);
  const int64_t N = a->n_nodes;
  const int d = a->d_out, din = a->d_in;
  HGT_REQUIRE(a->linear_impl >= 0 && a->linear_impl <= 3, "hgt_conv_forward: unknown linear_impl %d", a->linear_impl);
  const bool one = a->linear_impl == 3;
  const bool tc_upd = a->linear_impl != 1 && hgt_typed_linear_tc_supported(d, d, d);
  L->fuse_split = tc_upd;
  L->presplit_x = a->x_hi != nullptr && (a->x_lo != nullptr || one) && a->perm == nullptr && a->linear_impl != 1 &&
                  hgt_typed_linear_tc_supported(din, din, d);
  L->x_sorted = a->perm ? c.take<float>((size_t)N * din) : nullptr;
  L->w_cat = c.take<float>((size_t)(a->cat_rows > 0 ? a->cat_rows : 1) * din);
  L->b_cat = c.take<float>((size_t)(a->cat_rows > 0 ? a->cat_rows : 1));
  L->t24 = d % 8 == 0;
  if (L->t24) {
    L->proj = c.take<float>((size_t)a->kv_off);
    L->kv = c.take_bytes((size_t)(a->kv_rows + 1) * 6 * d);
  } else {
    L->proj = c.take<float>((size_t)a->proj_elems);
    L->kv = base ? L->proj + a->kv_off : nullptr;
  }
  int rc;
  if (L->presplit_x)
    rc = hgt_typed_linear_presplit_workspace_bytes(a->h_proj_groups, a->n_proj_groups, din, d, &L->ws_proj_bytes);
  else
    rc = hgt_typed_linear_workspace_bytes(a->h_proj_groups, a->n_proj_groups, din, d, a->linear_impl, &L->ws_proj_bytes);
  if (rc) return rc;
  L->ws_proj = c.take_bytes(L->ws_proj_bytes + 256);
  L->rt = nullptr;
  L->kvr = nullptr;
  if (a->use_rte) {
    L->rt = c.take<float>((size_t)HGT_RTE_MAX_LEN * din);
    L->kvr = c.take_bytes(((size_t)a->n_pairs * HGT_RTE_MAX_LEN + 1) * 2 * d * (L->t24 ? 3 : 4));
  }
  if ((rc = hgt_edge_workspace_bytes(a->n_split, d, a->n_heads, &L->ws_edge_bytes))) return rc;
  L->ws_edge = c.take_bytes(L->ws_edge_bytes);
  L->g_act = nullptr;
  L->g_hi = L->g_lo = nullptr;
  if (L->fuse_split) {
    L->g_hi = c.take_bytes((size_t)N * d * 2);
    L->g_lo = one ? nullptr : c.take_bytes((size_t)N * d * 2);
  } else {
    L->g_act = c.take<float>((size_t)N * d);
  }
  L->wa_cat = c.take<float>((size_t)a->num_types * d * d);
  L->ba_cat = c.take<float>((size_t)a->num_types * d);
  if (L->fuse_split)
    rc = hgt_typed_linear_presplit_workspace_bytes(a->h_upd_groups, a->n_upd_groups, d, d, &L->ws_upd_bytes);
  else
    rc = hgt_typed_linear_workspace_bytes(a->h_upd_groups, a->n_upd_groups, d, d, a->linear_impl, &L->ws_upd_bytes);
  if (rc) return rc;
  L->ws_upd = c.take_bytes(L->ws_upd_bytes + 256);
  L->o = c.take<float>((size_t)N * d);
  L->total = c.off + 256;
  return 0;
}

}

extern "C" uint64_t hgt_conv_args_size(void) { return sizeof(hgt_conv_args); }

extern "C" int hgt_conv_workspace_bytes(const hgt_conv_args* a, size_t* out_bytes) {
  HGT_REQUIRE(a && out_bytes, "hgt_conv_workspace_bytes: NULL argument");
  Layout L;
  int rc = plan_layout(a, nullptr, &L);
  if (rc) return rc;
  *out_bytes = L.total;
  return 0;
}

extern "C" int hgt_conv_forward(const hgt_conv_args* a, void* workspace, size_t workspace_bytes, void* stream) {
  HGT_REQUIRE(a && workspace, "hgt_conv_forward: NULL argument");
  HGT_REQUIRE(a->d_in == a->d_out, "hgt_conv_forward: in_dim must equal out_dim (conv.py:131)");
  HGT_REQUIRE(!a->use_rte || a->rte_row, "hgt_conv_forward: use_rte needs rte_row");
  HGT_REQUIRE(!(a->type_active && a->type_dst), "hgt_conv_forward: type_active and type_dst exclude each other");
  cudaStream_t st = (cudaStream_t)stream;
  Layout L;
  void* base = reinterpret_cast<void*>(hgt_align_up(reinterpret_cast<size_t>(workspace), 256));
  int rc = plan_layout(a, base, &L);
  if (rc) return rc;
  HGT_REQUIRE(workspace_bytes >= L.total, "hgt_conv_forward: workspace too small (%zu < %zu)", workspace_bytes, L.total);
  const int64_t N = a->n_nodes;
  const int d = a->d_out, din = a->d_in, T = a->num_types, P = a->n_pairs;
  if (N == 0) return 0;

  const float* x_sorted = a->x;
  if (a->perm) {
    if ((rc = hgt_gather_rows(a->x, a->perm, N, din, L.x_sorted, stream))) return rc;
    x_sorted = L.x_sorted;
  }
  if ((rc = hgt_fold_weights(a->wq, a->bq, a->wk, a->bk, a->wv, a->bv, a->relation_att, a->relation_msg,
                             a->relation_pri, T, a->num_relations, a->n_heads, din, d, P, a->pair_type, a->pair_rel,
                             a->cat_row0, a->q_row0, L.w_cat, L.b_cat, stream)))
    return rc;
  const size_t row_bytes = (size_t)2 * d * (L.t24 ? 3 : 4);
  HGT_CHECK_CUDA(cudaMemsetAsync(static_cast<char*>(L.kv) + a->kv_rows * row_bytes, 0, row_bytes, st));
  const void* x_lo = a->linear_impl == 3 ? nullptr : a->x_lo;
  if (L.t24) {
    if (L.presplit_x)
      rc = hgt_typed_linear_presplit_t24(a->x_hi, x_lo, L.w_cat, L.b_cat, din, d, a->proj_groups, a->h_proj_groups,
                                         a->n_proj_groups, a->proj_cblocks, L.proj, a->kv_off, L.kv, L.ws_proj,
                                         L.ws_proj_bytes + 256, stream);
    else
      rc = hgt_typed_linear_t24(x_sorted, din, L.w_cat, L.b_cat, din, d, a->proj_groups, a->h_proj_groups,
                                a->n_proj_groups, a->proj_cblocks, L.proj, a->kv_off, L.kv, a->linear_impl, L.ws_proj,
                                L.ws_proj_bytes + 256, stream);
  } else if (L.presplit_x) {
    rc = hgt_typed_linear_presplit(a->x_hi, x_lo, L.w_cat, L.b_cat, din, d, a->proj_groups, a->h_proj_groups,
                                   a->n_proj_groups, a->proj_cblocks, L.proj, L.ws_proj, L.ws_proj_bytes + 256, stream);
  } else {
    rc = hgt_typed_linear(x_sorted, din, L.w_cat, L.b_cat, din, d, a->proj_groups, a->h_proj_groups, a->n_proj_groups,
                          a->proj_cblocks, L.proj, a->linear_impl, L.ws_proj, L.ws_proj_bytes + 256, stream);
  }
  if (rc) return rc;
  if (a->use_rte) {
    if ((rc = hgt_typed_linear(a->emb_weight, din, a->emb_lin_w, a->emb_lin_b, din, din, a->rt_groups, a->h_rt_groups, 1,
                               a->rt_cblocks, L.rt, 1, nullptr, 0, stream)))
      return rc;
    HGT_CHECK_CUDA(cudaMemsetAsync(static_cast<char*>(L.kvr) + (int64_t)P * HGT_RTE_MAX_LEN * row_bytes, 0, row_bytes, st));
    rc = L.t24 ? hgt_typed_linear_t24(L.rt, din, L.w_cat, nullptr, din, d, a->rte_groups, a->h_rte_groups,
                                      a->n_rte_groups, a->rte_cblocks, nullptr, 0, L.kvr, 1, nullptr, 0, stream)
               : hgt_typed_linear(L.rt, din, L.w_cat, nullptr, din, d, a->rte_groups, a->h_rte_groups, a->n_rte_groups,
                                  a->rte_cblocks, static_cast<float*>(L.kvr), 1, nullptr, 0, stream);
    if (rc) return rc;
  }
  const int32_t* dst_rows = a->type_active ? a->type_active : a->type_dst;
  const int32_t* rte_row = a->use_rte ? a->rte_row : nullptr;
  if (L.t24)
    rc = hgt_edge_forward_t24(L.proj + a->q_off, L.kv, L.kvr, a->row_ptr, a->kv_row, rte_row, a->csr_eid, a->tiles,
                              a->n_tiles, a->n_split, a->hubs, a->n_hubs, N, a->n_edges, d, a->n_heads, 1, L.g_act,
                              a->att, nullptr, L.g_hi, L.g_lo, L.ws_edge, L.ws_edge_bytes, a->edge_variant,
                              a->d_tile_counts, a->type_row0, T, dst_rows, stream);
  else
    rc = hgt_edge_forward(L.proj + a->q_off, static_cast<const float*>(L.kv), static_cast<const float*>(L.kvr),
                          a->row_ptr, a->kv_row, rte_row, a->csr_eid, a->tiles, a->n_tiles, a->n_split, a->hubs,
                          a->n_hubs, N, a->n_edges, d, a->n_heads, 1, L.g_act, a->att, nullptr, L.g_hi, L.g_lo,
                          L.ws_edge, L.ws_edge_bytes, a->edge_variant, a->d_tile_counts, a->type_row0, T, dst_rows,
                          stream);
  if (rc) return rc;
  if ((rc = hgt_concat_linears(a->wa, a->ba, T, d, d, L.wa_cat, L.ba_cat, stream))) return rc;
  if (L.fuse_split)
    rc = hgt_typed_linear_presplit(L.g_hi, L.g_lo, L.wa_cat, L.ba_cat, d, d, a->upd_groups, a->h_upd_groups,
                                   a->n_upd_groups, a->upd_cblocks, L.o, L.ws_upd, L.ws_upd_bytes + 256, stream);
  else
    rc = hgt_typed_linear(L.g_act, d, L.wa_cat, L.ba_cat, d, d, a->upd_groups, a->h_upd_groups, a->n_upd_groups,
                          a->upd_cblocks, L.o, a->linear_impl, L.ws_upd, L.ws_upd_bytes + 256, stream);
  if (rc) return rc;
  const int32_t* perm_out = a->out_map ? a->out_map : a->perm;
  return hgt_update_epilogue_impl(L.o, x_sorted, a->type_row0, T, a->skip, nullptr, nullptr,
                                  a->use_norm ? a->norm_w : nullptr, a->use_norm ? a->norm_b : nullptr, perm_out,
                                  a->type_active, a->type_dst, a->type_dst ? L.ba_cat : nullptr, N, d, a->out, a->out_hi,
                                  a->out_lo, nullptr, 0.f, st);
}
```

pyhgt_b200/csrc/linear.cu:

```cuda
#include <cuda_bf16.h>

#include <type_traits>

#include "common.cuh"

int hgt_typed_linear_tc(const float* A, int64_t lda, const float* W, const float* bias, int32_t K,
                        int32_t cb_width, const hgt_lin_group* groups, const hgt_lin_group* h_groups,
                        int32_t n_groups, const hgt_lin_cblock* cblocks, float* out, int32_t products,
                        void* workspace, size_t workspace_bytes, cudaStream_t st);
int hgt_typed_linear_tc(const float* A, int64_t lda, const float* W, const float* bias, int32_t K,
                        int32_t cb_width, const hgt_lin_group* groups, const hgt_lin_group* h_groups,
                        int32_t n_groups, const hgt_lin_cblock* cblocks, __nv_bfloat16* out, int32_t products,
                        void* workspace, size_t workspace_bytes, cudaStream_t st);
int hgt_typed_linear_tc(const float* A, int64_t lda, const float* W, const float* bias, int32_t K,
                        int32_t cb_width, const hgt_lin_group* groups, const hgt_lin_group* h_groups,
                        int32_t n_groups, const hgt_lin_cblock* cblocks, float* out32, int64_t t24_off, hgt_t24* out,
                        int32_t products, void* workspace, size_t workspace_bytes, cudaStream_t st);
int hgt_typed_linear_tc_bf16a(const __nv_bfloat16* A, int64_t lda, const float* W, const float* bias, int32_t K,
                              int32_t cb_width, const hgt_lin_group* groups, const hgt_lin_group* h_groups,
                              int32_t n_groups, const hgt_lin_cblock* cblocks, float* out, int32_t products,
                              void* workspace, size_t workspace_bytes, cudaStream_t st);
bool hgt_typed_linear_tc_supported(int64_t lda, int32_t K, int32_t cb_width);
size_t hgt_typed_linear_tc_workspace(const hgt_lin_group* h_groups, int32_t n_groups, int32_t K, int32_t cb_width,
                                     int32_t products);

namespace {

constexpr int kMaxGroups = 64;

__global__ void k_fold_pairs(const float* const* __restrict__ wk, const float* const* __restrict__ bk,
                             const float* const* __restrict__ wv, const float* const* __restrict__ bv,
                             const float* __restrict__ rel_att, const float* __restrict__ rel_msg,
                             const float* __restrict__ rel_pri, int H, int d_in, int d_out, int n_pairs,
                             const int32_t* __restrict__ pair_type, const int32_t* __restrict__ pair_rel,
                             const int32_t* __restrict__ cat_row0, float* __restrict__ w_cat,
                             float* __restrict__ b_cat) {
  const int dk = d_out / H;
  const int64_t per_block = (int64_t)d_out * (d_in + 1);
  int64_t i = blockIdx.x * (int64_t)blockDim.x + threadIdx.x;
  if (i >= per_block * 2 * n_pairs) return;
  int p = (int)(i / (2 * per_block));
  int64_t rem = i - (int64_t)p * 2 * per_block;
  int which = (int)(rem / per_block);
  rem -= which * per_block;
  int row = (int)(rem / (d_in + 1));
  int col = (int)(rem - (int64_t)row * (d_in + 1));
  int h = row / dk, c = row - h * dk;
  int t = pair_type[p], r = pair_rel[p];
  const float* rel = (which ? rel_msg : rel_att) + ((int64_t)(r * H + h) * dk) * dk;
  const float* w = which ? wv[t] : wk[t];
  const float* b = which ? bv[t] : bk[t];
  float acc = 0.f;
  if (col < d_in) {
    for (int a = 0; a < dk; ++a) acc = fmaf(rel[a * dk + c], w[(int64_t)(h * dk + a) * d_in + col], acc);
  } else {
    for (int a = 0; a < dk; ++a) acc = fmaf(rel[a * dk + c], b[h * dk + a], acc);
  }
  if (!which) acc *= rel_pri[r * H + h] * rsqrtf((float)dk);
  int64_t out_row = (int64_t)cat_row0[p] + which * d_out + row;
  if (col < d_in) w_cat[out_row * d_in + col] = acc;
  else b_cat[out_row] = acc;
}

__global__ void k_copy_linears(const float* const* __restrict__ w, const float* const* __restrict__ b, int T,
                               int rows, int cols, const int32_t* __restrict__ row0,
                               float* __restrict__ w_cat, float* __restrict__ b_cat) {
  const int64_t per = (int64_t)rows * (cols + 1);
  int64_t i = blockIdx.x * (int64_t)blockDim.x + threadIdx.x;
  if (i >= per * T) return;
// ... 45 lines not shown
  const int64_t w_row0 = (int64_t)grp.w_row0 + (int64_t)cb * cb_width + n0;
  const int rows_here = (int)min((int64_t)BM, grp.m - m0);
  const int cols_here = min(BN, cb_width - n0);

  const int tid = threadIdx.x;
  const int tm = tid / 16, tn = tid % 16;
  float acc[8][4];
#pragma unroll
  for (int i = 0; i < 8; ++i)
#pragma unroll
    for (int j = 0; j < 4; ++j) acc[i][j] = 0.f;

  const AT* Ag = A + (grp.a_row0 + m0) * lda;
  const float* Wg = W + w_row0 * (int64_t)K;

  for (int k0 = 0; k0 < K; k0 += BK) {
#pragma unroll
    for (int it = 0; it < 8; ++it) {
      int idx = tid + it * GEMM_THREADS;
      int r = idx / BK, kk = idx % BK;
      float v = 0.f;
      if (r < rows_here && k0 + kk < K) v = load_a(Ag + (int64_t)r * lda + k0 + kk);
      As[kk][r] = v;
    }
#pragma unroll
    for (int it = 0; it < 4; ++it) {
      int idx = tid + it * GEMM_THREADS;
      int r = idx / BK, kk = idx % BK;
      float v = 0.f;
      if (r < cols_here && k0 + kk < K) v = Wg[(int64_t)r * K + k0 + kk];
      Ws[kk][r] = v;
    }
    __syncthreads();
#pragma unroll
    for (int kk = 0; kk < BK; ++kk) {
      float4 a0 = *reinterpret_cast<const float4*>(&As[kk][tm * 8]);
      float4 a1 = *reinterpret_cast<const float4*>(&As[kk][tm * 8 + 4]);
      float4 b0 = *reinterpret_cast<const float4*>(&Ws[kk][tn * 4]);
      float a[8] = {a0.x, a0.y, a0.z, a0.w, a1.x, a1.y, a1.z, a1.w};
      float b[4] = {b0.x, b0.y, b0.z, b0.w};
#pragma unroll
      for (int i = 0; i < 8; ++i)
#pragma unroll
        for (int j = 0; j < 4; ++j) acc[i][j] = fmaf(a[i], b[j], acc[i][j]);
    }
    __syncthreads();
  }
  float bj[4] = {0.f, 0.f, 0.f, 0.f};
  if (grp.has_bias && bias) {
#pragma unroll
    for (int j = 0; j < 4; ++j)
      if (tn * 4 + j < cols_here) bj[j] = bias[w_row0 + tn * 4 + j];
  }
  if (std::is_same<OutT, hgt_t24>::value && cblk.out_off < t24_off) {
    float* Og = out32 + cblk.out_off + m0 * cblk.ld + n0;
#pragma unroll
    for (int i = 0; i < 8; ++i) {
      int r = tm * 8 + i;
      if (r >= rows_here) continue;
#pragma unroll
      for (int j = 0; j < 4; ++j) {
        int c = tn * 4 + j;
        if (c < cols_here) Og[(int64_t)r * cblk.ld + c] = acc[i][j] + bj[j];
      }
    }
  } else if constexpr (std::is_same<OutT, hgt_t24>::value) {
    const hgt_t24_at e(out, cblk.out_off - t24_off + m0 * cblk.ld + n0, cblk.ld);
    const int64_t rb = 3 * cblk.ld;
#pragma unroll
    for (int i = 0; i < 8; ++i) {
      int r = tm * 8 + i;
      if (r >= rows_here) continue;
#pragma unroll
      for (int j = 0; j < 4; ++j) {
        int c = tn * 4 + j;
        if (c < cols_here) {
          const uint32_t w = hgt_t24_round(__float_as_uint(acc[i][j] + bj[j]));
          *reinterpret_cast<uint16_t*>(e.hi + r * rb + 2 * c) = (uint16_t)(w >> 16);
          e.lo[r * rb + c] = (unsigned char)(w >> 8);
        }
      }
    }
  } else {
    OutT* Og = out + cblk.out_off + m0 * cblk.ld + n0;
#pragma unroll
    for (int i = 0; i < 8; ++i) {
      int r = tm * 8 + i;
      if (r >= rows_here) continue;
#pragma unroll
      for (int j = 0; j < 4; ++j) {
        int c = tn * 4 + j;
        if (c < cols_here) store_out(Og + (int64_t)r * cblk.ld + c, acc[i][j] + bj[j]);
      }
    }
  }
}

}

extern "C" int hgt_fold_weights(const float* const* wq, const float* const* bq, const float* const* wk,
                                const float* const* bk, const float* const* wv, const float* const* bv,
                                const float* relation_att, const float* relation_msg, const float* relation_pri,
                                int32_t num_types, int32_t num_relations, int32_t n_heads, int32_t d_in,
                                int32_t d_out, int32_t n_pairs, const int32_t* pair_type, const int32_t* pair_rel,
                                const int32_t* cat_row0, const int32_t* q_row0, float* w_cat, float* b_cat,
                                void* stream_) {
  cudaStream_t st = (cudaStream_t)stream_;
  HGT_REQUIRE(n_heads > 0 && d_out % n_heads == 0, "hgt_fold_weights: d_out=%d not divisible by n_heads=%d",
              d_out, n_heads);
  (void)num_relations;
  {
    int64_t total = (int64_t)num_types * d_out * (d_in + 1);
    k_copy_linears<<<(unsigned)((total + 255) / 256), 256, 0, st>>>(wq, bq, num_types, d_out, d_in, q_row0,
                                                                    w_cat, b_cat);
    HGT_LAUNCH_CHECK();
  }
  if (n_pairs > 0) {
    int64_t total = (int64_t)n_pairs * 2 * d_out * (d_in + 1);
    k_fold_pairs<<<(unsigned)((total + 255) / 256), 256, 0, st>>>(wk, bk, wv, bv, relation_att, relation_msg,
                                                                  relation_pri, n_heads, d_in, d_out, n_pairs,
                                                                  pair_type, pair_rel, cat_row0, w_cat, b_cat);
    HGT_LAUNCH_CHECK();
  }
  return 0;
}

extern "C" int hgt_concat_linears(const float* const* w, const float* const* b, int32_t num_types, int32_t rows,
                                  int32_t cols, float* w_cat, float* b_cat, void* stream_) {
  cudaStream_t st = (cudaStream_t)stream_;
  int64_t total = (int64_t)num_types * rows * (cols + 1);
  if (total == 0) return 0;
  k_copy_linears<<<(unsigned)((total + 255) / 256), 256, 0, st>>>(w, b, num_types, rows, cols, nullptr, w_cat,
                                                                  b_cat);
  HGT_LAUNCH_CHECK();
  return 0;
}

extern "C" int hgt_typed_linear_workspace_bytes(const hgt_lin_group* h_groups, int32_t n_groups, int32_t K,
                                                int32_t cb_width, int32_t impl, size_t* out_bytes) {
  HGT_REQUIRE(out_bytes && (h_groups || n_groups == 0), "hgt_typed_linear_workspace_bytes: NULL argument");
  HGT_REQUIRE(impl >= 0 && impl <= 3, "hgt_typed_linear_workspace_bytes: unknown impl %d", impl);
  const bool tc = hgt_typed_linear_tc_supported(K, K, cb_width);
  if (impl == 0) impl = tc ? 2 : 1;
  if (impl == 3 && !tc) impl = 1;
  *out_bytes = (impl >= 2 && n_groups > 0)
                   ? hgt_typed_linear_tc_workspace(h_groups, n_groups, K, cb_width, impl == 3 ? 1 : 3)
                   : 0;
  return 0;
}

namespace {

template <class AT, class OutT>
int typed_linear(const AT* A, int64_t lda, const float* W, const float* bias, int32_t K, int32_t cb_width,
                 const hgt_lin_group* groups, const hgt_lin_group* h_groups, int32_t n_groups,
                 const hgt_lin_cblock* cblocks, OutT* out, int32_t impl, void* workspace, size_t workspace_bytes,
                 cudaStream_t st, float* out32 = nullptr, int64_t t24_off = 0) {
  HGT_REQUIRE(n_groups >= 0, "hgt_typed_linear: n_groups=%d", n_groups);
  HGT_REQUIRE(K > 0 && cb_width > 0, "hgt_typed_linear: K=%d cb_width=%d", K, cb_width);
  if (n_groups == 0) return 0;
  if (n_groups > kMaxGroups) {
    for (int g0 = 0; g0 < n_groups; g0 += kMaxGroups) {
      const int n = n_groups - g0 < kMaxGroups ? n_groups - g0 : kMaxGroups;
      int rc = typed_linear(A, lda, W, bias, K, cb_width, groups + g0, h_groups + g0, n, cblocks, out, impl, workspace,
                            workspace_bytes, st, out32, t24_off);
      if (rc) return rc;
    }
    return 0;
  }
  const bool tc = hgt_typed_linear_tc_supported(lda, K, cb_width);
  if (impl == 0) impl = tc ? 2 : 1;
  if (impl == 3 && !tc) impl = 1;
  if (impl == 2 || impl == 3) {
    HGT_REQUIRE(tc, "hgt_typed_linear: tensor-core kernel does not support lda=%lld K=%d cb_width=%d",
                (long long)lda, K, cb_width);
    if constexpr (std::is_same<AT, __nv_bfloat16>::value)
      return hgt_typed_linear_tc_bf16a(A, lda, W, bias, K, cb_width, groups, h_groups, n_groups, cblocks, out,
                                       impl == 3 ? 1 : 3, workspace, workspace_bytes, st);
    else if constexpr (std::is_same<OutT, hgt_t24>::value)
      return hgt_typed_linear_tc(A, lda, W, bias, K, cb_width, groups, h_groups, n_groups, cblocks, out32, t24_off, out,
                                 impl == 3 ? 1 : 3, workspace, workspace_bytes, st);
    else
      return hgt_typed_linear_tc(A, lda, W, bias, K, cb_width, groups, h_groups, n_groups, cblocks, out,
                                 impl == 3 ? 1 : 3, workspace, workspace_bytes, st);
  }
  HGT_REQUIRE(impl == 1, "hgt_typed_linear: unknown impl %d", impl);
  TilePrefix tp;
  tp.n_tiles_n = (cb_width + BN - 1) / BN;
  int64_t total = 0;
  for (int g = 0; g < n_groups; ++g) {
    tp.first_tile[g] = (int32_t)total;
    int64_t mt = (h_groups[g].m + BM - 1) / BM;
    total += mt * h_groups[g].n_cblocks * tp.n_tiles_n;
    HGT_REQUIRE(total < 2147483647ll, "hgt_typed_linear: too many tiles");
  }
  tp.first_tile[n_groups] = (int32_t)total;
  if (total == 0) return 0;
  k_typed_linear_simt<AT, OutT><<<(unsigned)total, GEMM_THREADS, 0, st>>>(A, lda, W, bias, K, cb_width, groups, n_groups,
                                                                      cblocks, out, tp, out32, t24_off);
  HGT_LAUNCH_CHECK();
  return 0;
}

}

extern "C" int hgt_typed_linear(const float* A, int64_t lda, const float* W, const float* bias, int32_t K,
                                int32_t cb_width, const hgt_lin_group* groups, const hgt_lin_group* h_groups,
                                int32_t n_groups, const hgt_lin_cblock* cblocks, float* out, int32_t impl,
                                void* workspace, size_t workspace_bytes, void* stream_) {
  return typed_linear(A, lda, W, bias, K, cb_width, groups, h_groups, n_groups, cblocks, out, impl, workspace,
                      workspace_bytes, (cudaStream_t)stream_);
}

extern "C" int hgt_typed_linear_bf16(const float* A, int64_t lda, const float* W, const float* bias, int32_t K,
                                     int32_t cb_width, const hgt_lin_group* groups, const hgt_lin_group* h_groups,
                                     int32_t n_groups, const hgt_lin_cblock* cblocks, void* out, int32_t impl,
                                     void* workspace, size_t workspace_bytes, void* stream_) {
  return typed_linear(A, lda, W, bias, K, cb_width, groups, h_groups, n_groups, cblocks,
                      static_cast<__nv_bfloat16*>(out), impl, workspace, workspace_bytes, (cudaStream_t)stream_);
}

extern "C" int hgt_typed_linear_t24(const float* A, int64_t lda, const float* W, const float* bias, int32_t K,
                                    int32_t cb_width, const hgt_lin_group* groups, const hgt_lin_group* h_groups,
                                    int32_t n_groups, const hgt_lin_cblock* cblocks, float* out, int64_t t24_off,
                                    void* out24, int32_t impl, void* workspace, size_t workspace_bytes, void* stream_) {
  return typed_linear(A, lda, W, bias, K, cb_width, groups, h_groups, n_groups, cblocks, static_cast<hgt_t24*>(out24),
                      impl, workspace, workspace_bytes, (cudaStream_t)stream_, out, t24_off);
}

extern "C" int hgt_typed_linear_bf16a(const void* A, int64_t lda, const float* W, const float* bias, int32_t K,
                                      int32_t cb_width, const hgt_lin_group* groups, const hgt_lin_group* h_groups,
                                      int32_t n_groups, const hgt_lin_cblock* cblocks, float* out, int32_t impl,
                                      void* workspace, size_t workspace_bytes, void* stream_) {
  return typed_linear(static_cast<const __nv_bfloat16*>(A), lda, W, bias, K, cb_width, groups, h_groups, n_groups,
                      cblocks, out, impl, workspace, workspace_bytes, (cudaStream_t)stream_);
}
```

pyhgt_b200/csrc/linear_tc.cu:

```cuda
#include <cuda.h>
#include <cuda_bf16.h>

#include <stdlib.h>

#include "common.cuh"
#include "tc_ptx.cuh"

namespace {

using namespace tcp;

constexpr int kMaxGroups = 64;
template <int BN> constexpr int fwd_bk() { return BN == 64 ? 64 : 32; }
template <int BN> constexpr bool fwd_tma_store() { return BN != 64; }
template <int BN> constexpr uint32_t fwd_out_stage() { return fwd_tma_store<BN>() ? TMA_STAGE_BYTES : OUT_STAGE_BYTES; }

__global__ void k_split_bf16(const float* __restrict__ in, int64_t ld_in, int64_t rows, int K, int Kp,
                             __nv_bfloat16* __restrict__ hi, __nv_bfloat16* __restrict__ lo) {
  const int vec_per_row = Kp / 4;
  int64_t i = blockIdx.x * (int64_t)blockDim.x + threadIdx.x;
  if (i >= rows * vec_per_row) return;
  int64_t r = i / vec_per_row;
  int c = (int)(i - r * vec_per_row) * 4;
  float v[4];
// ... 13 lines not shown
  }
  *reinterpret_cast<uint2*>(hi + r * Kp + c) = *reinterpret_cast<uint2*>(h);
  if (lo) *reinterpret_cast<uint2*>(lo + r * Kp + c) = *reinterpret_cast<uint2*>(l);
}

__global__ void k_pad_bf16(const __nv_bfloat16* __restrict__ in, int64_t ld_in, int64_t rows, int K, int Kp,
                           __nv_bfloat16* __restrict__ out) {
  const int vec_per_row = Kp / 4;
  int64_t i = blockIdx.x * (int64_t)blockDim.x + threadIdx.x;
  if (i >= rows * vec_per_row) return;
  int64_t r = i / vec_per_row;
  int c = (int)(i - r * vec_per_row) * 4;
  const __nv_bfloat16* src = in + r * ld_in + c;
  __nv_bfloat16 v[4];
#pragma unroll
  for (int j = 0; j < 4; ++j) v[j] = (c + j < K) ? src[j] : __float2bfloat16_rn(0.f);
  *reinterpret_cast<uint2*>(out + r * Kp + c) = *reinterpret_cast<uint2*>(v);
}

__device__ __forceinline__ void store4(float* p, float4 v, bool aligned) {
  if (aligned) {
    *reinterpret_cast<float4*>(p) = v;
  } else if ((reinterpret_cast<uintptr_t>(p) & 7) == 0) {
    *reinterpret_cast<float2*>(p) = make_float2(v.x, v.y);
    *reinterpret_cast<float2*>(p + 2) = make_float2(v.z, v.w);
  } else {
    p[0] = v.x; p[1] = v.y; p[2] = v.z; p[3] = v.w;
  }
}
__device__ __forceinline__ void store4(__nv_bfloat16* p, float4 v, bool aligned) {
  const __nv_bfloat162 a = __floats2bfloat162_rn(v.x, v.y), b = __floats2bfloat162_rn(v.z, v.w);
  if (aligned) {
    *reinterpret_cast<uint2*>(p) = make_uint2(*reinterpret_cast<const uint32_t*>(&a), *reinterpret_cast<const uint32_t*>(&b));
  } else {
    p[0] = a.x; p[1] = a.y; p[2] = b.x; p[3] = b.y;
  }
}
__device__ __forceinline__ void store4_t24(unsigned char* hi, unsigned char* lo, float4 v, bool aligned) {
  uint32_t h01, l01, h23, l23;
  t24_pair(make_float2(v.x, v.y), h01, l01);
  t24_pair(make_float2(v.z, v.w), h23, l23);
  if (aligned) {
    *reinterpret_cast<uint2*>(hi) = make_uint2(h01, h23);
    *reinterpret_cast<uint32_t*>(lo) = __byte_perm(l01, l23, 0x5410);
  } else {
    const uint32_t h[4] = {h01 & 0xffffu, h01 >> 16, h23 & 0xffffu, h23 >> 16}, l[4] = {l01 & 0xffu, l01 >> 8, l23 & 0xffu, l23 >> 8};
#pragma unroll
    for (int i = 0; i < 4; ++i) {
      hi[2 * i] = (unsigned char)h[i];
      hi[2 * i + 1] = (unsigned char)(h[i] >> 8);
      lo[i] = (unsigned char)l[i];
    }
  }
}

template <class OutT, bool AF = false>
struct FwdJob {
  CUtensorMap a_hi, a_lo, w_hi, w_lo;
  const float* bias;
  const hgt_lin_group* groups;
  const hgt_lin_cblock* cblocks;
  OutT* out;
  float* out32;
  int64_t t24_off;
  const CUtensorMap* out_maps;
  int n_groups, cb_width, k_blocks, tile_n, n_tiles_n;
  int32_t first_tile[kMaxGroups + 1];
  int32_t map_first[kMaxGroups];

  struct Tile {
    int a_row, w_row, cols, m0, n0;
    int64_t rows, ld;
    OutT* out;
    float* out32;
    unsigned char *hi, *lo;
    const float* bias;
    const CUtensorMap* map;
  };

  __device__ int decode(int tile, Tile& t) const {
    int g = 0;
    while (g + 1 < n_groups && tile >= first_tile[g + 1]) ++g;
    const hgt_lin_group grp = groups[g];
    int local = tile - first_tile[g];
    const int per_m = grp.n_cblocks * n_tiles_n;
    const int mt = local / per_m;
    local -= mt * per_m;
    const int cb = local / n_tiles_n;
    const int n0 = (local - cb * n_tiles_n) * tile_n;
    const hgt_lin_cblock cblk = cblocks[grp.cb_first + cb];
    const int64_t m0 = (int64_t)mt * BM;
    t.a_row = (int)(grp.a_row0 + m0);
    t.w_row = grp.w_row0 + cb * cb_width + n0;
    t.cols = cb_width - n0;
    t.rows = grp.m - m0;
    t.ld = cblk.ld;
    if constexpr (is_t24<OutT>()) {
      const int64_t off = cblk.out_off + m0 * cblk.ld + n0;
      t.out32 = cblk.out_off < t24_off ? out32 + off : nullptr;
      const hgt_t24_at e(out, off - t24_off, cblk.ld);
      t.hi = e.hi;
      t.lo = e.lo;
    } else {
      t.out = out + cblk.out_off + m0 * cblk.ld + n0;
    }
    t.bias = (grp.has_bias && bias) ? bias + t.w_row : nullptr;
    t.m0 = (int)m0;
    t.n0 = n0;
    t.map = out_maps + out_maps_per_block<OutT>() * (map_first[g] + cb);
    return k_blocks;
  }
  __device__ void prefetch(const Tile&) const {
    prefetch_map(&a_hi); prefetch_map(&a_lo); prefetch_map(&w_hi); prefetch_map(&w_lo);
  }
  template <int BN, int KB, int P>
  __device__ void load(const Tile& t, int kb, uint32_t sa, uint32_t bar) const {
    constexpr uint32_t A = a_bytes<KB>(), B = b_offset<KB, P, AF>();
    const int k = kb * KB;
    if constexpr (AF) {
#pragma unroll
      for (int j = 0; j < KB / 32; ++j) tma_load_2d(sa + j * A32_BOX, &a_hi, k + 32 * j, t.a_row, bar);
    } else {
      tma_load_2d(sa, &a_hi, k, t.a_row, bar);
      if constexpr (has_a_lo<P>()) tma_load_2d(sa + A, &a_lo, k, t.a_row, bar);
    }
    tma_load_2d(sa + B, &w_hi, k, t.w_row, bar);
    if constexpr (has_b_lo<P>()) tma_load_2d(sa + B + BN * KB * 2, &w_lo, k, t.w_row, bar);
  }
  template <int BN, class T, class Pair>
  __device__ void store_plain(const Tile& t, T* o, const float* acc, float* stage, int c, int wq, int lane,
                              Pair pair) const {
    o += (int64_t)(64 * c) * t.ld;
    const int64_t rows = t.rows - 64 * c, ld = t.ld;
    const int cols = t.cols;
    const uintptr_t align = reinterpret_cast<uintptr_t>(o) | (uintptr_t)(ld * sizeof(T));
    if constexpr (fwd_tma_store<BN>()) {
      if ((align & 15) == 0) {
        store_tma<BN, T>(acc, reinterpret_cast<unsigned char*>(stage), c, wq, lane, pair, t.map, t.n0, t.m0 + 64 * c,
                         cols);
        return;
      }
      if (wq == 0 && lane == 0) bulk_wait_read<0>();
    }
    const bool vec4 = (align & (4 * sizeof(T) - 1)) == 0;
    store_staged<BN>(acc, stage, c, wq, lane, pair, [&](int r, int col, float4 v) {
      if (r < rows && col < cols) store4(o + r * ld + col, v, vec4);
    });
  }
  template <int BN>
  __device__ void store(const Tile& t, const float* acc, float* stage, int c, int wq, int lane) const {
    const float* b = t.bias;
    const int cols = t.cols;
    auto pair = [&](int, int col, float v0, float v1) {
      if (b && col < cols) v0 += __ldg(b + col), v1 += __ldg(b + col + 1);
      return make_float2(v0, v1);
    };
    if constexpr (is_t24<OutT>()) {
      if (t.out32) {
        store_plain<BN>(t, t.out32, acc, stage, c, wq, lane, pair);
        return;
      }
      const int64_t rows = t.rows - 64 * c;
      const int64_t rb = 3 * t.ld;
      unsigned char* hi = t.hi + 64 * c * rb;
      unsigned char* lo = t.lo + 64 * c * rb;
      if constexpr (fwd_tma_store<BN>()) {
        if (((reinterpret_cast<uintptr_t>(hi) | reinterpret_cast<uintptr_t>(lo) | (uintptr_t)rb) & 15) == 0) {
          store_tma<BN, OutT>(acc, reinterpret_cast<unsigned char*>(stage), c, wq, lane, pair, t.map, t.n0,
                              t.m0 + 64 * c, cols);
          return;
        }
        if (wq == 0 && lane == 0) bulk_wait_read<0>();
      }
      const bool vec4 = ((reinterpret_cast<uintptr_t>(hi) | (uintptr_t)rb) & 7) == 0 &&
                        ((reinterpret_cast<uintptr_t>(lo) | (uintptr_t)rb) & 3) == 0;
      store_staged<BN>(acc, stage, c, wq, lane, pair, [&](int r, int col, float4 v) {
        if (r < rows && col < cols) store4_t24(hi + r * rb + 2 * col, lo + r * rb + col, v, vec4);
      });
    } else {
      store_plain<BN>(t, t.out, acc, stage, c, wq, lane, pair);
    }
  }
};

template <int BN, class OutT, int P = 3, int KB = fwd_bk<BN>(), bool AF = false>
__global__ void __launch_bounds__(TILE_THREADS, 1)
    k_typed_linear_tc(const __grid_constant__ FwdJob<OutT, AF> job, int n_tiles) {
  split3_tile<BN, false, KB, fwd_out_stage<BN>(), P, AF>(job, n_tiles);
}

struct MapFirst {
  int32_t v[kMaxGroups];
};

__device__ __forceinline__ void put_map(CUtensorMap* m, const CUtensorMap& tmpl, const void* base, int64_t rows,
                                        uint64_t stride) {
#pragma unroll
  for (int i = 0; i < 8; ++i) reinterpret_cast<uint4*>(m)[i] = reinterpret_cast<const uint4*>(&tmpl)[i];
  const uint64_t gm = (uint64_t)__cvta_generic_to_global(m);
  asm volatile("tensormap.replace.tile.global_address.global.b1024.b64 [%0], %1;" ::"l"(gm), "l"(base) : "memory");
  asm volatile("tensormap.replace.tile.global_dim.global.b1024.b32 [%0], 1, %1;" ::"l"(gm), "r"((uint32_t)rows)
               : "memory");
  asm volatile("tensormap.replace.tile.global_stride.global.b1024.b64 [%0], 0, %1;" ::"l"(gm), "l"(stride) : "memory");
}

template <class OutT>
__global__ void k_out_maps(const __grid_constant__ CUtensorMap tmpl, const __grid_constant__ CUtensorMap tmpl_lo,
                           const __grid_constant__ CUtensorMap tmpl_f32, const hgt_lin_group* __restrict__ groups,
                           const hgt_lin_cblock* __restrict__ cblocks, OutT* out, float* out32, int64_t t24_off,
                           const MapFirst first, CUtensorMap* maps) {
  const hgt_lin_group grp = groups[blockIdx.x];
  for (int cb = threadIdx.x; cb < grp.n_cblocks; cb += blockDim.x) {
    const hgt_lin_cblock cblk = cblocks[grp.cb_first + cb];
    CUtensorMap* m = maps + out_maps_per_block<OutT>() * (first.v[blockIdx.x] + cb);
    if (grp.m <= 0) continue;
    if (is_t24<OutT>() && cblk.out_off < t24_off) {
      const float* base = out32 + cblk.out_off;
      const uint64_t stride = (uint64_t)cblk.ld * 4;
      if (((reinterpret_cast<uintptr_t>(base) | stride) & 15) != 0) continue;
      put_map(m, tmpl_f32, base, grp.m, stride);
    } else if constexpr (is_t24<OutT>()) {
      const hgt_t24_at e(out, cblk.out_off - t24_off, cblk.ld);
      const uint64_t stride = 3 * (uint64_t)cblk.ld;
      if (((reinterpret_cast<uintptr_t>(e.hi) | reinterpret_cast<uintptr_t>(e.lo) | stride) & 15) != 0) continue;
      put_map(m, tmpl, e.hi, grp.m, stride);
      put_map(m + 1, tmpl_lo, e.lo, grp.m, stride);
    } else {
      OutT* base = out + cblk.out_off;
      const uint64_t stride = (uint64_t)cblk.ld * sizeof(OutT);
      if (((reinterpret_cast<uintptr_t>(base) | stride) & 15) != 0) continue;
      put_map(m, tmpl, base, grp.m, stride);
    }
  }
  asm volatile("fence.proxy.tensormap::generic.release.gpu;" ::: "memory");
}

typedef CUresult (*EncodeTiledFn)(CUtensorMap*, CUtensorMapDataType, cuuint32_t, void*, const cuuint64_t*,
                                  const cuuint64_t*, const cuuint32_t*, const cuuint32_t*, CUtensorMapInterleave,
                                  CUtensorMapSwizzle, CUtensorMapL2promotion, CUtensorMapFloatOOBfill);

EncodeTiledFn get_encode_fn() {
  static EncodeTiledFn fn = nullptr;
  if (fn) return fn;
  void* p = nullptr;
  cudaDriverEntryPointQueryResult q;
  if (cudaGetDriverEntryPoint("cuTensorMapEncodeTiled", &p, cudaEnableDefault, &q) != cudaSuccess ||
      q != cudaDriverEntryPointSuccess)
    return nullptr;
  fn = reinterpret_cast<EncodeTiledFn>(p);
  return fn;
}

int make_map(CUtensorMap* m, const void* base, int64_t rows, int Kp, int box_rows, int kb, int64_t ld = 0) {
  EncodeTiledFn fn = get_encode_fn();
  HGT_REQUIRE(fn != nullptr, "hgt_typed_linear: cuTensorMapEncodeTiled not available from the driver");
  cuuint64_t dims[2] = {(cuuint64_t)Kp, (cuuint64_t)rows};
  cuuint64_t strides[1] = {(cuuint64_t)(ld ? ld : Kp) * 2};
  cuuint32_t box[2] = {(cuuint32_t)kb, (cuuint32_t)box_rows};
  cuuint32_t estr[2] = {1, 1};
  CUresult r = fn(m, CU_TENSOR_MAP_DATA_TYPE_BFLOAT16, 2, const_cast<void*>(base), dims, strides, box, estr,
                  CU_TENSOR_MAP_INTERLEAVE_NONE, kb == 64 ? CU_TENSOR_MAP_SWIZZLE_128B : CU_TENSOR_MAP_SWIZZLE_64B,
                  CU_TENSOR_MAP_L2_PROMOTION_L2_256B,
                  CU_TENSOR_MAP_FLOAT_OOB_FILL_NONE);
  HGT_REQUIRE(r == CUDA_SUCCESS, "hgt_typed_linear: cuTensorMapEncodeTiled failed (%d) rows=%lld Kp=%d box=%d",
              (int)r, (long long)rows, Kp, box_rows);
  return 0;
}

int make_map_f32(CUtensorMap* m, const float* base, int64_t rows, int K, int64_t lda) {
  EncodeTiledFn fn = get_encode_fn();
  HGT_REQUIRE(fn != nullptr, "hgt_typed_linear: cuTensorMapEncodeTiled not available from the driver");
  cuuint64_t dims[2] = {(cuuint64_t)K, (cuuint64_t)rows};
  cuuint64_t strides[1] = {(cuuint64_t)lda * 4};
  cuuint32_t box[2] = {32, (cuuint32_t)BM};
  cuuint32_t estr[2] = {1, 1};
  CUresult r = fn(m, CU_TENSOR_MAP_DATA_TYPE_FLOAT32, 2, const_cast<float*>(base), dims, strides, box, estr,
                  CU_TENSOR_MAP_INTERLEAVE_NONE, CU_TENSOR_MAP_SWIZZLE_128B, CU_TENSOR_MAP_L2_PROMOTION_L2_256B,
                  CU_TENSOR_MAP_FLOAT_OOB_FILL_NONE);
  HGT_REQUIRE(r == CUDA_SUCCESS, "hgt_typed_linear: cuTensorMapEncodeTiled (fp32 A) failed (%d) rows=%lld K=%d lda=%lld",
              (int)r, (long long)rows, K, (long long)lda);
  return 0;
}

bool a_fp32_loadable(const float* A, int64_t lda) {
  return A && (reinterpret_cast<uintptr_t>(A) & 15) == 0 && lda % 4 == 0;
}

int make_out_template(CUtensorMap* m, void* dummy, int cb_width, int elem) {
  EncodeTiledFn fn = get_encode_fn();
  HGT_REQUIRE(fn != nullptr, "hgt_typed_linear: cuTensorMapEncodeTiled not available from the driver");
  cuuint64_t dims[2] = {(cuuint64_t)cb_width, 64};
  cuuint64_t strides[1] = {(cuuint64_t)hgt_align_up((size_t)cb_width * elem, 16)};
  cuuint32_t box[2] = {elem == 1 ? 64u : 128 / (cuuint32_t)elem, 64};
  cuuint32_t estr[2] = {1, 1};
  const CUtensorMapDataType type = elem == 4 ? CU_TENSOR_MAP_DATA_TYPE_FLOAT32
                                   : elem == 2 ? CU_TENSOR_MAP_DATA_TYPE_BFLOAT16 : CU_TENSOR_MAP_DATA_TYPE_UINT8;
  CUresult r = fn(m, type, 2, dummy, dims, strides, box, estr, CU_TENSOR_MAP_INTERLEAVE_NONE,
                  elem == 1 ? CU_TENSOR_MAP_SWIZZLE_64B : CU_TENSOR_MAP_SWIZZLE_128B, CU_TENSOR_MAP_L2_PROMOTION_NONE,
                  CU_TENSOR_MAP_FLOAT_OOB_FILL_NONE);
  HGT_REQUIRE(r == CUDA_SUCCESS, "hgt_typed_linear: cuTensorMapEncodeTiled (output) failed (%d) cb_width=%d", (int)r,
              cb_width);
  return 0;
}

int64_t n_out_maps(const hgt_lin_group* h_groups, int n_groups) {
  int64_t n = 0;
  for (int g = 0; g < n_groups; ++g) n += h_groups[g].n_cblocks;
  return n;
}

void extents(const hgt_lin_group* h_groups, int n_groups, int cb_width, int64_t* a_rows, int64_t* w_rows) {
  *a_rows = 0;
  *w_rows = 0;
  for (int g = 0; g < n_groups; ++g) {
    int64_t a = h_groups[g].a_row0 + h_groups[g].m;
    int64_t w = (int64_t)h_groups[g].w_row0 + (int64_t)h_groups[g].n_cblocks * cb_width;
    if (a > *a_rows) *a_rows = a;
    if (w > *w_rows) *w_rows = w;
  }
}

struct FwdOps {
  const float* a32;
  int64_t lda, a_ld = 0;
  const __nv_bfloat16 *a_hi, *a_lo, *w_hi, *w_lo;
  int64_t a_rows, w_rows;
  int K, Kp;
  float* out32;
  int64_t t24_off;
};

template <int BN, class OutT, int P = 3, int KB = fwd_bk<BN>(), bool AF = false>
int launch_fwd(FwdJob<OutT, AF>& job, const FwdOps& ops, int tiles, cudaStream_t st) {
  int rc;
  if constexpr (AF) {
    if ((rc = make_map_f32(&job.a_hi, ops.a32, ops.a_rows, ops.K, ops.lda))) return rc;
    job.a_lo = job.a_hi;
  } else {
    if ((rc = make_map(&job.a_hi, ops.a_hi, ops.a_rows, ops.Kp, BM, KB, ops.a_ld))) return rc;
    if ((rc = make_map(&job.a_lo, has_a_lo<P>() ? ops.a_lo : ops.a_hi, ops.a_rows, ops.Kp, BM, KB, ops.a_ld))) return rc;
  }
  if ((rc = make_map(&job.w_hi, ops.w_hi, ops.w_rows, ops.Kp, BN, KB))) return rc;
  if ((rc = make_map(&job.w_lo, has_b_lo<P>() ? ops.w_lo : ops.w_hi, ops.w_rows, ops.Kp, BN, KB))) return rc;
  job.k_blocks = (ops.Kp + KB - 1) / KB;
  if constexpr (fwd_tma_store<BN>()) {
    CUtensorMap tmpl, tmpl_lo, tmpl_f32;
    MapFirst first;
    void* dummy = const_cast<CUtensorMap*>(job.out_maps);
    if ((rc = make_out_template(&tmpl, dummy, job.cb_width, is_t24<OutT>() ? 2 : (int)sizeof(OutT)))) return rc;
    tmpl_lo = tmpl_f32 = tmpl;
    if (is_t24<OutT>() && ((rc = make_out_template(&tmpl_lo, dummy, job.cb_width, 1)) ||
                           (rc = make_out_template(&tmpl_f32, dummy, job.cb_width, 4))))
      return rc;
    for (int g = 0; g < job.n_groups; ++g) first.v[g] = job.map_first[g];
    k_out_maps<OutT><<<job.n_groups, 64, 0, st>>>(tmpl, tmpl_lo, tmpl_f32, job.groups, job.cblocks, job.out, job.out32,
                                                  job.t24_off, first, const_cast<CUtensorMap*>(job.out_maps));
    HGT_LAUNCH_CHECK();
  }
  const size_t smem = tile_smem_bytes<BN, KB, fwd_out_stage<BN>(), P, AF>();
  HGT_CHECK_CUDA(cudaFuncSetAttribute(k_typed_linear_tc<BN, OutT, P, KB, AF>,
                                      cudaFuncAttributeMaxDynamicSharedMemorySize, (int)smem));
  k_typed_linear_tc<BN, OutT, P, KB, AF><<<persistent_grid(tiles), TILE_THREADS, smem, st>>>(job, tiles);
  HGT_LAUNCH_CHECK();
  return 0;
}

template <class OutT, bool AF>
int run_fwd(const FwdOps& ops, const float* bias, int32_t cb_width, const hgt_lin_group* groups,
            const hgt_lin_group* h_groups, int32_t n_groups, const hgt_lin_cblock* cblocks, OutT* out,
            CUtensorMap* out_maps, bool one, cudaStream_t st, bool a_exact = false) {
  FwdJob<OutT, AF> job;
  job.tile_n = pick_tile_n(cb_width);
  job.n_tiles_n = (cb_width + job.tile_n - 1) / job.tile_n;
  int64_t total = 0, maps = 0;
  for (int g = 0; g < n_groups; ++g) {
    job.map_first[g] = (int32_t)maps;
    maps += h_groups[g].n_cblocks;
    job.first_tile[g] = (int32_t)total;
    total += (h_groups[g].m + BM - 1) / BM * h_groups[g].n_cblocks * job.n_tiles_n;
    HGT_REQUIRE(total < 2147483647ll, "hgt_typed_linear(tc): too many tiles");
  }
  job.first_tile[n_groups] = (int32_t)total;
  if (total == 0) return 0;
  job.bias = bias;
  job.groups = groups;
  job.cblocks = cblocks;
  job.out = out;
  job.out32 = ops.out32;
  job.t24_off = ops.t24_off;
  job.out_maps = out_maps;
  job.n_groups = n_groups;
  job.cb_width = cb_width;
  const int tiles = (int)total;
  if constexpr (AF) HGT_REQUIRE(job.tile_n != 64, "hgt_typed_linear(tc): no fp32-A kernel for 64-column tiles");
  if constexpr (!AF && std::is_same<OutT, float>::value) {
    if (a_exact && !one) {
      switch (job.tile_n) {
        case 64: return launch_fwd<64, OutT, 2, fwd_bk<64>()>(job, ops, tiles, st);
        case 128: return launch_fwd<128, OutT, 2, fwd_bk<128>()>(job, ops, tiles, st);
        default: return launch_fwd<256, OutT, 2, fwd_bk<256>()>(job, ops, tiles, st);
      }
    }
  }
  HGT_REQUIRE(!a_exact || one, "hgt_typed_linear_bf16a(tc): fp32 output only");
  if (one) {
    static const int kb_env = [] {
// ... 23 lines not shown
}

}

bool hgt_typed_linear_tc_supported(int64_t lda, int32_t K, int32_t cb_width) {
  (void)lda;
  return cb_width % 16 == 0 && cb_width > 0 && K >= BK;
}

static bool splits_a_first(int32_t cb_width) { return pick_tile_n(cb_width) == 64; }

size_t hgt_typed_linear_tc_workspace(const hgt_lin_group* h_groups, int32_t n_groups, int32_t K, int32_t cb_width,
                                     int32_t products) {
  int64_t a_rows, w_rows;
  extents(h_groups, n_groups, cb_width, &a_rows, &w_rows);
  const int Kp = (K + 7) / 8 * 8;
  const size_t halves = products == 1 ? 1 : 2;
  const size_t a = splits_a_first(cb_width) ? halves * hgt_align_up((size_t)a_rows * Kp * 2, 256) : 0;
  return 4 * 256 + a + halves * hgt_align_up((size_t)w_rows * Kp * 2, 256) +
         hgt_align_up((size_t)n_out_maps(h_groups, n_groups) * 2 * sizeof(CUtensorMap), 256);
}

template <class OutT>
static int tc_run(const float* A, int64_t lda, const __nv_bfloat16* a_hi_in, const __nv_bfloat16* a_lo_in,
                  const float* W, const float* bias, int32_t K, int32_t cb_width, const hgt_lin_group* groups,
                  const hgt_lin_group* h_groups, int32_t n_groups, const hgt_lin_cblock* cblocks, OutT* out,
                  int32_t products, void* workspace, size_t workspace_bytes, cudaStream_t st, float* out32 = nullptr,
                  int64_t t24_off = 0);

int hgt_typed_linear_tc(const float* A, int64_t lda, const float* W, const float* bias, int32_t K, int32_t cb_width,
                        const hgt_lin_group* groups, const hgt_lin_group* h_groups, int32_t n_groups,
                        const hgt_lin_cblock* cblocks, float* out, int32_t products, void* workspace,
                        size_t workspace_bytes, cudaStream_t st) {
  return tc_run(A, lda, nullptr, nullptr, W, bias, K, cb_width, groups, h_groups, n_groups, cblocks, out, products,
                workspace, workspace_bytes, st);
}

int hgt_typed_linear_tc(const float* A, int64_t lda, const float* W, const float* bias, int32_t K, int32_t cb_width,
                        const hgt_lin_group* groups, const hgt_lin_group* h_groups, int32_t n_groups,
                        const hgt_lin_cblock* cblocks, __nv_bfloat16* out, int32_t products, void* workspace,
                        size_t workspace_bytes, cudaStream_t st) {
  return tc_run(A, lda, nullptr, nullptr, W, bias, K, cb_width, groups, h_groups, n_groups, cblocks, out, products,
                workspace, workspace_bytes, st);
}

int hgt_typed_linear_tc(const float* A, int64_t lda, const float* W, const float* bias, int32_t K, int32_t cb_width,
                        const hgt_lin_group* groups, const hgt_lin_group* h_groups, int32_t n_groups,
                        const hgt_lin_cblock* cblocks, float* out32, int64_t t24_off, hgt_t24* out,
                        int32_t products, void* workspace, size_t workspace_bytes, cudaStream_t st) {
  return tc_run(A, lda, nullptr, nullptr, W, bias, K, cb_width, groups, h_groups, n_groups, cblocks, out, products,
                workspace, workspace_bytes, st, out32, t24_off);
}

extern "C" int hgt_typed_linear_presplit_workspace_bytes(const hgt_lin_group* h_groups, int32_t n_groups, int32_t K,
                                                         int32_t cb_width, size_t* out_bytes) {
  HGT_REQUIRE(out_bytes && (h_groups || n_groups == 0), "hgt_typed_linear_presplit_workspace_bytes: NULL argument");
  *out_bytes = n_groups > 0 ? hgt_typed_linear_tc_workspace(h_groups, n_groups, K, cb_width, 3) : 0;
  return 0;
}

template <class OutT>
static int typed_linear_presplit(const void* a_hi, const void* a_lo, const float* W, const float* bias, int32_t K,
                                 int32_t cb_width, const hgt_lin_group* groups, const hgt_lin_group* h_groups,
                                 int32_t n_groups, const hgt_lin_cblock* cblocks, OutT* out, void* workspace,
                                 size_t workspace_bytes, cudaStream_t st, float* out32 = nullptr,
                                 int64_t t24_off = 0) {
  HGT_REQUIRE(a_hi, "hgt_typed_linear_presplit: NULL operand");
  HGT_REQUIRE(K % 8 == 0 && hgt_typed_linear_tc_supported(K, K, cb_width),
              "hgt_typed_linear_presplit: unsupported shape K=%d cb_width=%d", K, cb_width);
  if (n_groups == 0) return 0;
  if (n_groups > kMaxGroups) {
    for (int g0 = 0; g0 < n_groups; g0 += kMaxGroups) {
      const int n = n_groups - g0 < kMaxGroups ? n_groups - g0 : kMaxGroups;
      int rc = typed_linear_presplit(a_hi, a_lo, W, bias, K, cb_width, groups + g0, h_groups + g0, n, cblocks, out,
                                     workspace, workspace_bytes, st, out32, t24_off);
      if (rc) return rc;
    }
    return 0;
  }
  return tc_run(nullptr, 0, reinterpret_cast<const __nv_bfloat16*>(a_hi), reinterpret_cast<const __nv_bfloat16*>(a_lo),
                W, bias, K, cb_width, groups, h_groups, n_groups, cblocks, out, a_lo ? 3 : 1, workspace, workspace_bytes,
                st, out32, t24_off);
}

extern "C" int hgt_typed_linear_presplit(const void* a_hi, const void* a_lo, const float* W, const float* bias,
                                         int32_t K, int32_t cb_width, const hgt_lin_group* groups,
                                         const hgt_lin_group* h_groups, int32_t n_groups,
                                         const hgt_lin_cblock* cblocks, float* out, void* workspace,
                                         size_t workspace_bytes, void* stream_) {
  return typed_linear_presplit(a_hi, a_lo, W, bias, K, cb_width, groups, h_groups, n_groups, cblocks, out, workspace,
                               workspace_bytes, (cudaStream_t)stream_);
}

extern "C" int hgt_typed_linear_presplit_bf16(const void* a_hi, const void* a_lo, const float* W, const float* bias,
                                              int32_t K, int32_t cb_width, const hgt_lin_group* groups,
                                              const hgt_lin_group* h_groups, int32_t n_groups,
                                              const hgt_lin_cblock* cblocks, void* out, void* workspace,
                                              size_t workspace_bytes, void* stream_) {
  return typed_linear_presplit(a_hi, a_lo, W, bias, K, cb_width, groups, h_groups, n_groups, cblocks,
                               static_cast<__nv_bfloat16*>(out), workspace, workspace_bytes, (cudaStream_t)stream_);
}

extern "C" int hgt_typed_linear_presplit_t24(const void* a_hi, const void* a_lo, const float* W, const float* bias,
                                             int32_t K, int32_t cb_width, const hgt_lin_group* groups,
                                             const hgt_lin_group* h_groups, int32_t n_groups,
                                             const hgt_lin_cblock* cblocks, float* out, int64_t t24_off, void* out24,
                                             void* workspace, size_t workspace_bytes, void* stream_) {
  return typed_linear_presplit(a_hi, a_lo, W, bias, K, cb_width, groups, h_groups, n_groups, cblocks,
                               static_cast<hgt_t24*>(out24), workspace, workspace_bytes, (cudaStream_t)stream_, out,
                               t24_off);
}

template <class OutT>
static int tc_run(const float* A, int64_t lda, const __nv_bfloat16* a_hi_in, const __nv_bfloat16* a_lo_in,
                  const float* W, const float* bias, int32_t K, int32_t cb_width, const hgt_lin_group* groups,
                  const hgt_lin_group* h_groups, int32_t n_groups, const hgt_lin_cblock* cblocks, OutT* out,
                  int32_t products, void* workspace, size_t workspace_bytes, cudaStream_t st, float* out32,
                  int64_t t24_off) {
  HGT_REQUIRE(hgt_typed_linear_tc_supported(lda, K, cb_width), "hgt_typed_linear(tc): unsupported K=%d cb_width=%d", K,
              cb_width);
  HGT_REQUIRE(products == 3 || products == 1, "hgt_typed_linear(tc): products=%d", products);
  const bool one = products == 1;
  FwdOps ops;
  ops.out32 = out32;
  ops.t24_off = t24_off;
  ops.K = K;
  ops.Kp = (K + 7) / 8 * 8;
  extents(h_groups, n_groups, cb_width, &ops.a_rows, &ops.w_rows);
  size_t need = hgt_typed_linear_tc_workspace(h_groups, n_groups, K, cb_width, products);
  HGT_REQUIRE(workspace && workspace_bytes >= need, "hgt_typed_linear(tc): workspace too small (%zu < %zu)",
              workspace_bytes, need);
  const size_t w_half = hgt_align_up((size_t)ops.w_rows * ops.Kp * 2, 256);
  const size_t a_half = hgt_align_up((size_t)ops.a_rows * ops.Kp * 2, 256);
  char* p = reinterpret_cast<char*>(hgt_align_up(reinterpret_cast<size_t>(workspace), 256));
  __nv_bfloat16* a_ws = nullptr;
  if (splits_a_first(cb_width)) a_ws = reinterpret_cast<__nv_bfloat16*>(p), p += (one ? 1 : 2) * a_half;
  __nv_bfloat16* w_hi = reinterpret_cast<__nv_bfloat16*>(p); p += w_half;
  __nv_bfloat16* w_lo = one ? nullptr : reinterpret_cast<__nv_bfloat16*>(p); p += one ? 0 : w_half;
  CUtensorMap* out_maps = reinterpret_cast<CUtensorMap*>(p);
  ops.w_hi = w_hi;
  ops.w_lo = w_lo;
  int64_t n = ops.w_rows * (ops.Kp / 4);
  if (n > 0) k_split_bf16<<<(unsigned)((n + 255) / 256), 256, 0, st>>>(W, K, ops.w_rows, K, ops.Kp, w_hi, w_lo);
  HGT_LAUNCH_CHECK();
  ops.a32 = A;
  ops.lda = lda;
  ops.a_hi = a_hi_in;
  ops.a_lo = one ? nullptr : a_lo_in;
  if (a_hi_in)
    return run_fwd<OutT, false>(ops, bias, cb_width, groups, h_groups, n_groups, cblocks, out, out_maps, one, st);
  n = ops.a_rows * (ops.Kp / 4);
  if (a_ws) {
    if (n == 0) return 0;
    ops.a_hi = a_ws;
    ops.a_lo = one ? nullptr : a_ws + a_half / 2;
    k_split_bf16<<<(unsigned)((n + 255) / 256), 256, 0, st>>>(A, lda, ops.a_rows, K, ops.Kp, a_ws,
                                                              const_cast<__nv_bfloat16*>(ops.a_lo));
    HGT_LAUNCH_CHECK();
    return run_fwd<OutT, false>(ops, bias, cb_width, groups, h_groups, n_groups, cblocks, out, out_maps, one, st);
  }
  if (a_fp32_loadable(A, lda))
    return run_fwd<OutT, true>(ops, bias, cb_width, groups, h_groups, n_groups, cblocks, out, out_maps, one, st);
// ... 72 lines not shown
```

pyhgt_b200/csrc/tc_ptx.cuh:

```cuda
#pragma once
#include <cuda.h>
#include <cuda_bf16.h>
#include <stdint.h>

#include <type_traits>

#include "common.cuh"

namespace tcp {

__device__ __forceinline__ uint32_t s_u32(const void* p) { return static_cast<uint32_t>(__cvta_generic_to_shared(p)); }

__device__ __forceinline__ void mbar_init(uint32_t bar, uint32_t count) {
  asm volatile("mbarrier.init.shared::cta.b64 [%0], %1;" ::"r"(bar), "r"(count) : "memory");
}
__device__ __forceinline__ void mbar_expect_tx(uint32_t bar, uint32_t bytes) {
  asm volatile("mbarrier.arrive.expect_tx.shared::cta.b64 _, [%0], %1;" ::"r"(bar), "r"(bytes) : "memory");
}
__device__ __forceinline__ void mbar_arrive(uint32_t bar) {
  asm volatile("mbarrier.arrive.shared::cta.b64 _, [%0];" ::"r"(bar) : "memory");
}
__device__ __forceinline__ bool mbar_try_wait(uint32_t bar, uint32_t parity) {
  uint32_t ok;
  asm volatile(
// ... 227 lines not shown
}

template <int BN, class Pair, class Write>
__device__ __forceinline__ void store_staged(const float* acc, float* stage, int c, int wq, int lane, Pair pair,
                                             Write write) {
  const int tid = 32 * wq + lane, r0 = 16 * wq + (lane >> 2), c0 = 2 * (lane & 3);
#pragma unroll
  for (int blk = 0; blk < BN / 64; ++blk) {
    bar_sync_named(1 + c, 128);
#pragma unroll
    for (int j = 8 * blk; j < 8 * blk + 8; ++j) {
#pragma unroll
      for (int h = 0; h < 2; ++h) {
        const int r = r0 + 8 * h, lc = 8 * j + c0 - 64 * blk;
        const float2 v = pair(r, 8 * j + c0, acc[4 * j + 2 * h], acc[4 * j + 2 * h + 1]);
        *reinterpret_cast<float2*>(stage + r * 64 + (((lc >> 2) ^ ((r & 7) << 1)) << 2) + (lc & 3)) = v;
      }
    }
    bar_sync_named(1 + c, 128);
    const int q = tid & 15;
#pragma unroll
    for (int i = 0; i < 8; ++i) {
      const int r = (tid >> 4) + 8 * i;
      write(r, 64 * blk + 4 * q, *reinterpret_cast<const float4*>(stage + r * 64 + ((q ^ ((r & 7) << 1)) << 2)));
    }
  }
}

__device__ __forceinline__ void tma_store_2d(const CUtensorMap* map, uint32_t smem_src, int c0, int c1) {
  asm volatile("cp.async.bulk.tensor.2d.global.shared::cta.bulk_group [%0, {%2, %3}], [%1];"
               ::"l"(map), "r"(smem_src), "r"(c0), "r"(c1) : "memory");
}
__device__ __forceinline__ void tensormap_acquire(const CUtensorMap* m) {
  asm volatile("fence.proxy.tensormap::generic.acquire.gpu [%0], 128;" ::"l"(m) : "memory");
}
__device__ __forceinline__ void bulk_commit() { asm volatile("cp.async.bulk.commit_group;" ::: "memory"); }
template <int N>
__device__ __forceinline__ void bulk_wait_read() { asm volatile("cp.async.bulk.wait_group.read %0;" ::"n"(N) : "memory"); }
__device__ __forceinline__ void bulk_wait_all() { asm volatile("cp.async.bulk.wait_group 0;" ::: "memory"); }
__device__ __forceinline__ void fence_proxy_async_smem() { asm volatile("fence.proxy.async.shared::cta;" ::: "memory"); }

__device__ __forceinline__ void put2(float* p, float2 v) { *reinterpret_cast<float2*>(p) = v; }
__device__ __forceinline__ void put2(__nv_bfloat16* p, float2 v) {
  *reinterpret_cast<__nv_bfloat162*>(p) = __floats2bfloat162_rn(v.x, v.y);
}

__device__ __forceinline__ void t24_pair(float2 v, uint32_t& hi, uint32_t& lo) {
  const uint32_t a = hgt_t24_round(__float_as_uint(v.x)), b = hgt_t24_round(__float_as_uint(v.y));
  hi = __byte_perm(a, b, 0x7632);
  lo = __byte_perm(a, b, 0x0051);
}

template <class OutT> constexpr bool is_t24() { return std::is_same<OutT, hgt_t24>::value; }
template <class OutT> constexpr int out_maps_per_block() { return is_t24<OutT>() ? 2 : 1; }

template <int BN, class OutT, class Pair>
__device__ __forceinline__ void store_tma(const float* acc, unsigned char* stage, int c, int wq, int lane, Pair pair,
                                          const CUtensorMap* map, int col0, int row0, int cols) {
  static_assert(BN % 128 == 0, "the two buffers alternate across tiles only for an even number of 64-column blocks");
  constexpr bool T24 = is_t24<OutT>();
  constexpr int BOX_COLS = T24 ? 64 : 128 / (int)sizeof(OutT);
  const bool issuer = wq == 0 && lane == 0;
  const int r0 = 16 * wq + (lane >> 2), c0 = 2 * (lane & 3);
  if (issuer) {
    tensormap_acquire(map);
    if constexpr (T24) tensormap_acquire(map + 1);
  }
#pragma unroll
  for (int blk = 0; blk < BN / 64; ++blk) {
    unsigned char* buf = stage + (blk & 1) * TMA_BUF_BYTES;
    if (issuer) bulk_wait_read<1>();
    bar_sync_named(1 + c, 128);
#pragma unroll
    for (int j = 8 * blk; j < 8 * blk + 8; ++j) {
#pragma unroll
      for (int h = 0; h < 2; ++h) {
        const int r = r0 + 8 * h, lc = 8 * j + c0 - 64 * blk;
        const float2 v = pair(r, 8 * j + c0, acc[4 * j + 2 * h], acc[4 * j + 2 * h + 1]);
        if constexpr (T24) {
          uint32_t hi, lo;
          t24_pair(v, hi, lo);
          const uint32_t x = (uint32_t)lc * 2;
          *reinterpret_cast<uint32_t*>(buf + r * 128 + ((((x >> 4) ^ (r & 7)) << 4) | (x & 15))) = hi;
          *reinterpret_cast<uint16_t*>(buf + 8192 + r * 64 + ((((lc >> 4) ^ ((r >> 1) & 3)) << 4) | (lc & 15))) =
              (uint16_t)lo;
        } else {
          const uint32_t x = (uint32_t)(lc % BOX_COLS) * sizeof(OutT);
          put2(reinterpret_cast<OutT*>(buf + (lc / BOX_COLS) * 8192 + r * 128 + ((((x >> 4) ^ (r & 7)) << 4) | (x & 15))),
               v);
        }
      }
    }
    fence_proxy_async_smem();
    bar_sync_named(1 + c, 128);
    if (issuer) {
#pragma unroll
      for (int bx = 0; bx < 64 / BOX_COLS; ++bx)
        if (64 * blk + BOX_COLS * bx < cols) tma_store_2d(map, s_u32(buf + bx * 8192), col0 + 64 * blk + BOX_COLS * bx, row0);
      if constexpr (T24)
        if (64 * blk < cols) tma_store_2d(map + 1, s_u32(buf + 8192), col0 + 64 * blk, row0);
      bulk_commit();
    }
  }
}

template <int BN, bool MN, int KB, uint32_t OUT = OUT_STAGE_BYTES, int P = 3, bool AF = false, class Job>
__device__ __forceinline__ void split3_tile(const Job& job, int n_tiles) {
  static_assert(!AF || !MN, "fp32 A is loaded K-major");
  constexpr int S = n_stages<BN, KB, OUT, P, AF>();
  constexpr uint32_t STAGE = stage_bytes<BN, KB, P, AF>();
  constexpr uint32_t ATOM = atom_bytes<KB>(), B = b_offset<KB, P, AF>();
  constexpr uint32_t A = AF ? (KB == 32 ? 512u : A32_BOX) : a_bytes<KB>();
  constexpr uint32_t A_SBO = AF ? 1024u : 16u * KB;
  constexpr uint32_t SLAB = AF ? 64u * 128u : ATOM;
  extern __shared__ unsigned char smem_dyn[];
  unsigned char* smem = smem_dyn + ((1024u - (s_u32(smem_dyn) & 1023u)) & 1023u);
  unsigned char* out_stage = smem + (size_t)S * STAGE;
  uint64_t* full_bar = reinterpret_cast<uint64_t*>(smem + (size_t)S * STAGE + OUT);
  uint64_t* empty_bar = full_bar + S;
  const uint32_t base = s_u32(smem);
  const int wg = threadIdx.x >> 7, warp = threadIdx.x >> 5, lane = threadIdx.x & 31;

  if (threadIdx.x == 0) {
    for (int s = 0; s < S; ++s) {
      mbar_init(s_u32(&full_bar[s]), 1);
      mbar_init(s_u32(&empty_bar[s]), 8);
    }
    asm volatile("fence.mbarrier_init.release.cluster;" ::: "memory");
  }
  __syncthreads();

  int s = 0;
  uint32_t phase = 0;
  if (wg == 0) {
    asm volatile("setmaxnreg.dec.sync.aligned.u32 40;" ::: "memory");
    if (threadIdx.x == 0) {
      for (int tile = blockIdx.x; tile < n_tiles; tile += gridDim.x) {
        typename Job::Tile t;
        const int iters = job.decode(tile, t);
        job.prefetch(t);
        for (int it = 0; it < iters; ++it) {
          mbar_wait(s_u32(&empty_bar[s]), phase ^ 1u);
          const uint32_t bar = s_u32(&full_bar[s]);
          mbar_expect_tx(bar, STAGE);
          job.template load<BN, KB, P>(t, it, base + (uint32_t)s * STAGE, bar);
          if (++s == S) s = 0, phase ^= 1u;
        }
      }
    }
  } else {
    asm volatile("setmaxnreg.inc.sync.aligned.u32 232;" ::: "memory");
    const int c = wg - 1;
    for (int tile = blockIdx.x; tile < n_tiles; tile += gridDim.x) {
// ... 38 lines not shown
```

Baseline: 1.042 billion.

## Add block-scaled 16-bit gather table format selected by L2 fit

Adds a new KV/RTE table encoding (bs16): 16-bit integer mantissas with a shared bf16-style scale per 16 elements. The typed-linear TMA epilogue quantizes into this format and the edge kernels decode it. A runtime chooser picks f32, t24 or bs16 from d, table rows and L2 size. The aim is to shrink gathered row bytes below the 3-byte t24 format so more of the table stays in L2 and edge gathers move less data, at the cost of lower precision and extra decode and scale work.

Measured after the change: 1.161 billion, median of 6. 11.4% higher.

```diff
diff --git a/include/hgt_b200.h b/include/hgt_b200.h
--- a/include/hgt_b200.h
+++ b/include/hgt_b200.h
@@ -148,6 +148,21 @@
                                   int32_t n_groups, const hgt_lin_cblock* cblocks, float* out, int64_t t24_off,
                                   void* out24, void* workspace, size_t workspace_bytes, void* stream);
 
+int hgt_typed_linear_bs16(const float* A, int64_t lda, const float* W, const float* bias, int32_t K,
+                          int32_t cb_width, const hgt_lin_group* groups, const hgt_lin_group* h_groups,
+                          int32_t n_groups, const hgt_lin_cblock* cblocks, float* out, int64_t t24_off, void* out16,
+                          int32_t impl, void* workspace, size_t workspace_bytes, void* stream);
+int hgt_typed_linear_presplit_bs16(const void* a_hi, const void* a_lo, const float* W, const float* bias, int32_t K,
+                                   int32_t cb_width, const hgt_lin_group* groups, const hgt_lin_group* h_groups,
+                                   int32_t n_groups, const hgt_lin_cblock* cblocks, float* out, int64_t t24_off,
+                                   void* out16, void* workspace, size_t workspace_bytes, void* stream);
+
+#define HGT_TABLE_F32 0
+#define HGT_TABLE_T24 1
+#define HGT_TABLE_BS16 2
+int hgt_gather_table_format(int32_t d, int64_t table_rows, int64_t l2_bytes, int32_t* out_format);
+int hgt_gather_table_row_bytes(int32_t format, int64_t n, int64_t* out_bytes);
+
 
 int hgt_edge_workspace_bytes(int32_t n_split_tiles, int32_t d, int32_t n_heads, size_t* out_bytes);
 int hgt_edge_forward(const float* q, const float* kv, const float* kvr,
@@ -195,6 +210,14 @@
                          float* agg_out, float* att_out, float* stats_out, void* g_hi, void* g_lo,
                          void* workspace, size_t workspace_bytes, int32_t variant, const int32_t* d_tile_counts,
                          const int32_t* type_row0, int32_t num_types, const int32_t* type_active, void* stream);
+int hgt_edge_forward_bs16(const float* q, const void* kv, const void* kvr,
+                          const int32_t* row_ptr, const int32_t* kv_row, const int32_t* rte_row,
+                          const int32_t* csr_eid, const int32_t* tiles, int32_t n_tiles, int32_t n_split_tiles,
+                          const int32_t* hubs, int32_t n_hubs,
+                          int64_t n_nodes, int64_t n_edges, int32_t d, int32_t n_heads, int32_t apply_gelu,
+                          float* agg_out, float* att_out, float* stats_out, void* g_hi, void* g_lo,
+                          void* workspace, size_t workspace_bytes, int32_t variant, const int32_t* d_tile_counts,
+                          const int32_t* type_row0, int32_t num_types, const int32_t* type_active, void* stream);
 int hgt_edge_backward_bf16(const float* q, const void* kv, const void* kvr, const float* agg, const float* dagg,
                            const float* stats, const int32_t* row_ptr, const int32_t* kv_row, const int32_t* rte_row,
                            const int32_t* tiles, int32_t n_tiles, int64_t n_nodes, int32_t d, int32_t n_heads,
diff --git a/pyhgt_b200/_lib.py b/pyhgt_b200/_lib.py
--- a/pyhgt_b200/_lib.py
+++ b/pyhgt_b200/_lib.py
@@ -67,10 +67,16 @@
     "hgt_typed_linear_presplit_bf16": [_p, _p, _p, _p, _i32, _i32, _p, _p, _i32, _p, _p, _p, _sz, _p],
     "hgt_typed_linear_t24": [_p, _i64, _p, _p, _i32, _i32, _p, _p, _i32, _p, _p, _i64, _p, _i32, _p, _sz, _p],
     "hgt_typed_linear_presplit_t24": [_p, _p, _p, _p, _i32, _i32, _p, _p, _i32, _p, _p, _i64, _p, _p, _sz, _p],
+    "hgt_gather_table_format": [_i32, _i64, _i64, _c.POINTER(_i32)],
+    "hgt_gather_table_row_bytes": [_i32, _i64, _c.POINTER(_i64)],
+    "hgt_typed_linear_bs16": [_p, _i64, _p, _p, _i32, _i32, _p, _p, _i32, _p, _p, _i64, _p, _i32, _p, _sz, _p],
+    "hgt_typed_linear_presplit_bs16": [_p, _p, _p, _p, _i32, _i32, _p, _p, _i32, _p, _p, _i64, _p, _p, _sz, _p],
     "hgt_edge_forward_bf16": [_p, _p, _p, _p, _p, _p, _p, _p, _i32, _i32, _p, _i32, _i64, _i64, _i32, _i32, _i32, _p, _p,
                               _p, _p, _p, _p, _sz, _i32, _p, _p, _i32, _p, _p],
     "hgt_edge_forward_t24": [_p, _p, _p, _p, _p, _p, _p, _p, _i32, _i32, _p, _i32, _i64, _i64, _i32, _i32, _i32, _p, _p,
                              _p, _p, _p, _p, _sz, _i32, _p, _p, _i32, _p, _p],
+    "hgt_edge_forward_bs16": [_p, _p, _p, _p, _p, _p, _p, _p, _i32, _i32, _p, _i32, _i64, _i64, _i32, _i32, _i32, _p, _p,
+                              _p, _p, _p, _p, _sz, _i32, _p, _p, _i32, _p, _p],
     "hgt_edge_backward_bf16": [_p, _p, _p, _p, _p, _p, _p, _p, _p, _p, _i32, _i64, _i32, _i32, _i64, _i64, _p, _p, _p, _p,
                                _sz, _p, _p],
     "hgt_edge_backward_dst_bf16": [_p, _p, _p, _p, _p, _p, _p, _p, _p, _p, _i32, _i32, _p, _i32, _i64, _i32, _i32, _p, _p,
@@ -212,6 +218,24 @@
     check(getattr(lib, name)(*args), name)
 
 
+TABLE_F32, TABLE_T24, TABLE_BS16 = 0, 1, 2
+TABLE_SUFFIX = {TABLE_F32: "", TABLE_T24: "_t24", TABLE_BS16: "_bs16"}
+
+
+def gather_table_format(d, table_rows, device):
+    import torch
+    out = _c.c_int32()
+    call("hgt_gather_table_format", d, table_rows, torch.cuda.get_device_properties(device).L2_cache_size,
+         _c.byref(out))
+    return out.value
+
+
+def gather_table_row_bytes(fmt, n):
+    out = _c.c_int64()
+    call("hgt_gather_table_row_bytes", fmt, n, _c.byref(out))
+    return out.value
+
+
 def kernel_launches():
     return int(load().hgt_kernel_launches())
 
diff --git a/pyhgt_b200/conv.py b/pyhgt_b200/conv.py
--- a/pyhgt_b200/conv.py
+++ b/pyhgt_b200/conv.py
@@ -36,7 +36,8 @@
     return torch.cuda.current_stream().cuda_stream
 
 
-_TABLE_SUFFIX = {torch.float32: "", torch.bfloat16: "_bf16", torch.uint8: "_t24"}
+_TABLE_SUFFIX = {"f32": "", "bf16": "_bf16", _lib.TABLE_T24: "_t24", _lib.TABLE_BS16: "_bs16", _lib.TABLE_F32: ""}
+_BYTE_TABLES = ("_t24", "_bs16")
 
 
 def _output_rows(rows, d, dev, lt, out_map):
@@ -152,13 +153,14 @@
                     HGTConv.event_sink.append((name, self_.a, self_.b))
         return _T()
 
-    def _typed_linear(self, a, lda, w, bias, k, width, table, out, impl, st, out32=None, t24_off=0):
+    def _typed_linear(self, a, lda, w, bias, k, width, table, out, impl, st, out32=None, t24_off=0, fmt=None):
         g_dev, g_host, n_g, c_dev = table
         ws_bytes = ctypes.c_size_t()
         _lib.call("hgt_typed_linear_workspace_bytes", g_host.ctypes.data, n_g, k, width, impl, ctypes.byref(ws_bytes))
         ws = torch.empty(max(ws_bytes.value, 1), dtype=torch.uint8, device=out.device)
-        outs = (_lib.ptr(out32), t24_off, out.data_ptr()) if out.dtype == torch.uint8 else (out.data_ptr(),)
-        fn = "hgt_typed_linear_bf16a" if a.dtype == torch.bfloat16 else "hgt_typed_linear" + _TABLE_SUFFIX[out.dtype]
+        sfx = "_bf16" if out.dtype == torch.bfloat16 else _TABLE_SUFFIX[fmt] if out.dtype == torch.uint8 else ""
+        outs = (_lib.ptr(out32), t24_off, out.data_ptr()) if sfx in _BYTE_TABLES else (out.data_ptr(),)
+        fn = "hgt_typed_linear_bf16a" if a.dtype == torch.bfloat16 else "hgt_typed_linear" + sfx
         _lib.call(fn, a.data_ptr(), lda, w.data_ptr(), _lib.ptr(bias), k, width, g_dev.data_ptr(),
                   g_host.ctypes.data, n_g, c_dev.data_ptr(), *outs, impl, ws.data_ptr(), ws.numel(), st)
 
@@ -378,15 +380,16 @@
                   plan.pair_rel_dev.data_ptr(), lt.cat_row0_dev.data_ptr(), lt.q_row0_dev.data_ptr(),
                   w_cat.data_ptr(), b_cat.data_ptr(), st)
 
-        t24 = not save and not bf16 and d % 8 == 0
-        tab_dtype = torch.bfloat16 if bf16 else torch.uint8 if t24 else torch.float32
-        row_len = 2 * d * (3 if t24 else 1)
+        fmt = "bf16" if bf16 else _lib.TABLE_F32 if save else _lib.gather_table_format(d, plan.kv_rows + 1, dev)
+        byte_tab = fmt in (_lib.TABLE_T24, _lib.TABLE_BS16)
+        tab_dtype = torch.bfloat16 if bf16 else torch.uint8 if byte_tab else torch.float32
+        row_len = _lib.gather_table_row_bytes(fmt, 2 * d) if byte_tab else 2 * d
         proj = None
         if bf16:
             q_tab = torch.empty(N * d, **f32)
             kv_tab = torch.empty((plan.kv_rows + 1) * row_len, dtype=tab_dtype, device=dev)
             calls = ((lt.q_groups, q_tab, None), (lt.kv_groups, kv_tab, None))
-        elif t24:
+        elif byte_tab:
             q_buf = torch.empty(lt.kv_off, **f32)
             q_tab = q_buf[lt.q_off:lt.q_off + N * d]
             kv_tab = torch.empty((plan.kv_rows + 1) * row_len, dtype=tab_dtype, device=dev)
@@ -401,15 +404,17 @@
             xs = x_split if plan.sorted_types else None
             for tab, out, out32 in calls:
                 if xs is None:
-                    self._typed_linear(x_sorted, d_in, w_cat, b_cat, d_in, d, tab, out, impl, st, out32, lt.kv_off)
+                    self._typed_linear(x_sorted, d_in, w_cat, b_cat, d_in, d, tab, out, impl, st, out32, lt.kv_off,
+                                       fmt)
                     continue
                 g_dev, g_host, n_g, c_dev = tab
                 wsb = ctypes.c_size_t()
                 _lib.call("hgt_typed_linear_presplit_workspace_bytes", g_host.ctypes.data, n_g, d_in, d,
                           ctypes.byref(wsb))
                 ws1 = torch.empty(max(wsb.value, 1), dtype=torch.uint8, device=dev)
-                outs = (out32.data_ptr(), lt.kv_off, out.data_ptr()) if t24 else (out.data_ptr(),)
-                _lib.call("hgt_typed_linear_presplit" + _TABLE_SUFFIX[out.dtype], xs[0].data_ptr(),
+                outs = (out32.data_ptr(), lt.kv_off, out.data_ptr()) if byte_tab else (out.data_ptr(),)
+                sfx = _TABLE_SUFFIX[fmt] if out is kv_tab else ""
+                _lib.call("hgt_typed_linear_presplit" + sfx, xs[0].data_ptr(),
                           None if one else _lib.ptr(xs[1]), w_cat.data_ptr(), b_cat.data_ptr(), d_in, d, g_dev.data_ptr(),
                           g_host.ctypes.data, n_g, c_dev.data_ptr(), *outs, ws1.data_ptr(), ws1.numel(), st)
         kvr = None
@@ -419,7 +424,7 @@
                                lt.rt_group, rt, 1, st)
             kvr = torch.empty((P * _plan.RTE_MAX_LEN + 1) * row_len, dtype=tab_dtype, device=dev)
             kvr[P * _plan.RTE_MAX_LEN * row_len:].zero_()
-            self._typed_linear(rt, d_in, w_cat, None, d_in, d, lt.rte_groups, kvr, 1, st)
+            self._typed_linear(rt, d_in, w_cat, None, d_in, d, lt.rte_groups, kvr, 1, st, fmt=fmt)
 
         ws_bytes = ctypes.c_size_t()
         _lib.call("hgt_edge_workspace_bytes", plan.n_split, d, H, ctypes.byref(ws_bytes))
@@ -432,7 +437,7 @@
         att = torch.empty((E, H), **f32) if want_att else None
         stats = torch.empty((N, 2 * H), **f32) if save else None
         with self._stage("edge"):
-            _lib.call("hgt_edge_forward" + _TABLE_SUFFIX[tab_dtype], q_tab.data_ptr(), kv_tab.data_ptr(), _lib.ptr(kvr), plan.row_ptr.data_ptr(),
+            _lib.call("hgt_edge_forward" + _TABLE_SUFFIX[fmt], q_tab.data_ptr(), kv_tab.data_ptr(), _lib.ptr(kvr), plan.row_ptr.data_ptr(),
                       plan.kv_row.data_ptr(), _lib.ptr(plan.rte_row) if self.use_RTE else None,
                       plan.csr_eid.data_ptr(), plan.tiles.data_ptr(), plan.n_tiles, plan.n_split,
                       plan.hubs.data_ptr(), plan.n_hubs, N, E, d, H, 1 if (gelu_before_a and not save) else 0,
diff --git a/pyhgt_b200/csrc/common.cuh b/pyhgt_b200/csrc/common.cuh
--- a/pyhgt_b200/csrc/common.cuh
+++ b/pyhgt_b200/csrc/common.cuh
@@ -59,6 +59,54 @@
   }
 };
 
+struct hgt_bs16 {};
+
+__host__ __device__ __forceinline__ int64_t hgt_bs16_row_bytes(int64_t n) { return (2 * n + n / 8 + 15) / 16 * 16; }
+
+struct HgtBs16RcpTab {
+  float v[128];
+};
+constexpr HgtBs16RcpTab hgt_bs16_rcp_tab() {
+  HgtBs16RcpTab t{};
+  for (int i = 0; i < 128; ++i) t.v[i] = 1.0f / (1.0f + (float)i / 128.0f);
+  return t;
+}
+static __device__ const HgtBs16RcpTab kHgtBs16Rcp = hgt_bs16_rcp_tab();
+
+__device__ __forceinline__ uint32_t hgt_bs16_scale(uint32_t amax, float& r) {
+  const float t = __fmul_rn(__uint_as_float(amax), 3.0518509447574615e-05f);
+  const uint32_t sb = (__float_as_uint(t) + 0xffffu) >> 16;
+  const int e = (int)((sb >> 7) & 0xffu);
+  float rr = __uint_as_float(__float_as_uint(__ldg(&kHgtBs16Rcp.v[sb & 0x7fu])) + ((uint32_t)(127 - e) << 23));
+  rr = sb >= 0x7780u ? __fmul_rn(rr, 0.999969482421875f) : rr;
+  const bool nonfinite = amax >= 0x7f800000u;
+  const bool tiny = sb < 0x80u;
+  r = nonfinite || tiny ? 0.f : rr;
+  return nonfinite ? 0x7fc0u : tiny ? 0u : sb;
+}
+
+__device__ __forceinline__ uint32_t hgt_bs16_pack(float x0, float x1, float r, uint32_t sb) {
+  const float y0 = __fadd_rn(__fmul_rn(x0, r), 12582912.f), y1 = __fadd_rn(__fmul_rn(x1, r), 12582912.f);
+  return sb == 0x7fc0u ? 0u : __byte_perm(__float_as_uint(y0), __float_as_uint(y1), 0x5410);
+}
+
+__device__ __forceinline__ uint32_t hgt_bs16_quad_amax(uint32_t a) {
+  a = max(a, __shfl_xor_sync(0xffffffffu, a, 1));
+  return max(a, __shfl_xor_sync(0xffffffffu, a, 2));
+}
+__device__ __forceinline__ uint32_t hgt_abs_bits(float x) { return __float_as_uint(x) & 0x7fffffffu; }
+
+struct hgt_bs16_at {
+  unsigned char* m;
+  unsigned char* s;
+  __host__ __device__ __forceinline__ hgt_bs16_at(void* base, int64_t off, int64_t ld) {
+    const int64_t row = off / ld, col = off - row * ld;
+    unsigned char* r = static_cast<unsigned char*>(base) + row * hgt_bs16_row_bytes(ld);
+    m = r + 2 * col;
+    s = r + 2 * ld + 2 * (col / 16);
+  }
+};
+
 struct HgtDrop {
   uint32_t thr;
   float scale;
diff --git a/pyhgt_b200/csrc/edge.cu b/pyhgt_b200/csrc/edge.cu
--- a/pyhgt_b200/csrc/edge.cu
+++ b/pyhgt_b200/csrc/edge.cu
@@ -112,7 +112,22 @@
   }
 }
 
-template <class KV> constexpr int64_t kv_elem_bytes() { return std::is_same<KV, hgt_t24>::value ? 3 : sizeof(KV); }
+template <int VEC>
+__device__ __forceinline__ void bs16_decode(float (&dst)[VEC], uint32_t m0, uint32_t m1, uint32_t sb) {
+  const float s = __uint_as_float(sb << 16);
+  dst[0] = __fmul_rn(__int2float_rn((int)(int16_t)(m0 & 0xffffu)), s);
+  if constexpr (VEC >= 2) dst[1] = __fmul_rn(__int2float_rn((int)m0 >> 16), s);
+  if constexpr (VEC == 4) {
+    dst[2] = __fmul_rn(__int2float_rn((int)(int16_t)(m1 & 0xffffu)), s);
+    dst[3] = __fmul_rn(__int2float_rn((int)m1 >> 16), s);
+  }
+}
+
+template <class KV> constexpr bool is_bs16() { return std::is_same<KV, hgt_bs16>::value; }
+template <class KV> __host__ __device__ __forceinline__ int64_t kv_row_bytes(int64_t n) {
+  if constexpr (is_bs16<KV>()) return hgt_bs16_row_bytes(n);
+  return n * (std::is_same<KV, hgt_t24>::value ? 3 : (int64_t)sizeof(KV));
+}
 
 template <class KV, int VEC, bool NC>
 __device__ __forceinline__ void load_kv(float (&dst)[VEC], const unsigned char* row, int e, int n) {
@@ -145,6 +160,27 @@
       }
     }
     t24_decode<VEC>(dst, h0, h1, l);
+  } else if constexpr (is_bs16<KV>()) {
+    const unsigned char* mp = row + 2 * e;
+    const unsigned char* sp = row + 2 * n + 2 * (e >> 4);
+    uint32_t m0 = 0, m1 = 0, sb = 0;
+    if constexpr (NC) {
+      if constexpr (VEC == 4) asm volatile("ld.global.nc.L1::no_allocate.v2.b32 {%0,%1}, [%2];" : "=r"(m0), "=r"(m1) : "l"(mp));
+      else if constexpr (VEC == 2) asm volatile("ld.global.nc.L1::no_allocate.b32 %0, [%1];" : "=r"(m0) : "l"(mp));
+      else asm volatile("ld.global.nc.L1::no_allocate.u16 %0, [%1];" : "=r"(m0) : "l"(mp));
+      asm volatile("ld.global.nc.L1::no_allocate.u16 %0, [%1];" : "=r"(sb) : "l"(sp));
+    } else {
+      if constexpr (VEC == 4) {
+        const uint2 m = *reinterpret_cast<const uint2*>(mp);
+        m0 = m.x; m1 = m.y;
+      } else if constexpr (VEC == 2) {
+        m0 = *reinterpret_cast<const uint32_t*>(mp);
+      } else {
+        m0 = *reinterpret_cast<const uint16_t*>(mp);
+      }
+      sb = *reinterpret_cast<const uint16_t*>(sp);
+    }
+    bs16_decode<VEC>(dst, m0, m1, sb);
   } else {
     const KV* p = reinterpret_cast<const KV*>(row) + e;
     if constexpr (NC) load_vec_nc<VEC>(dst, p);
@@ -264,7 +300,7 @@
 template <class KV, int VEC, int NCH>
 __global__ void __launch_bounds__(kCtaThreads, 1)
 k_edge_fwd_ldg(EdgeParams p) {
-  constexpr int W = std::is_same<KV, hgt_t24>::value ? 2 * NCH * VEC : NCH * VEC;
+  constexpr int W = std::is_same<KV, hgt_t24>::value || is_bs16<KV>() ? 2 * NCH * VEC : NCH * VEC;
   constexpr int EDGE_UNROLL = (W >= 32) ? 1 : (W >= 16 ? 2 : 4);
   const int lane = threadIdx.x & 31;
   const LaneMap lm(p, lane);
@@ -272,7 +308,7 @@
   const unsigned char* const kvrt = static_cast<const unsigned char*>(p.kvr);
   const bool rte = kvrt != nullptr;
   const int n = 2 * p.d;
-  const int64_t row_bytes = n * kv_elem_bytes<KV>();
+  const int64_t row_bytes = kv_row_bytes<KV>(n);
   int offs[NCH];
 #pragma unroll
   for (int t = 0; t < NCH; ++t) offs[t] = lm.off<VEC>(t);
@@ -429,7 +465,7 @@
   const bool rte = kvrt != nullptr;
   const int S = p.stages;
   const int n = 2 * p.d;
-  const uint32_t row_bytes = (uint32_t)(n * kv_elem_bytes<KV>());
+  const uint32_t row_bytes = (uint32_t)kv_row_bytes<KV>(n);
   const uint32_t slot_bytes = rte ? 2u * row_bytes : row_bytes;
   unsigned char* ring = smem_raw + (size_t)warp * S * slot_bytes;
   uint64_t* bars = reinterpret_cast<uint64_t*>(smem_raw + (size_t)kWarpsPerCta * S * slot_bytes) + warp * S;
@@ -715,6 +751,21 @@
                                d_tile_counts, type_row0, num_types, type_active, (cudaStream_t)stream_);
 }
 
+extern "C" int hgt_edge_forward_bs16(const float* q, const void* kv, const void* kvr, const int32_t* row_ptr,
+                                     const int32_t* kv_row, const int32_t* rte_row, const int32_t* csr_eid,
+                                     const int32_t* tiles, int32_t n_tiles, int32_t n_split_tiles, const int32_t* hubs,
+                                     int32_t n_hubs, int64_t n_nodes, int64_t n_edges, int32_t d, int32_t n_heads,
+                                     int32_t apply_gelu, float* agg_out, float* att_out, float* stats_out, void* g_hi,
+                                     void* g_lo, void* workspace, size_t workspace_bytes, int32_t variant,
+                                     const int32_t* d_tile_counts, const int32_t* type_row0, int32_t num_types,
+                                     const int32_t* type_active, void* stream_) {
+  (void)n_edges;
+  return edge_forward<hgt_bs16>(q, static_cast<const hgt_bs16*>(kv), static_cast<const hgt_bs16*>(kvr), row_ptr, kv_row,
+                                rte_row, csr_eid, tiles, n_tiles, n_split_tiles, hubs, n_hubs, n_nodes, d, n_heads,
+                                apply_gelu, agg_out, att_out, stats_out, g_hi, g_lo, workspace, workspace_bytes, variant,
+                                d_tile_counts, type_row0, num_types, type_active, (cudaStream_t)stream_);
+}
+
 namespace {
 
 template <class KV>
@@ -764,14 +815,16 @@
   int grid = sms;
   size_t smem = 0;
   HGT_REQUIRE((!std::is_same<KV, hgt_t24>::value || d % 8 == 0), "hgt_edge_forward_t24: needs d %% 8 == 0 (d=%d)", d);
-  const size_t row_bytes = 2 * (size_t)d * kv_elem_bytes<KV>();
+  HGT_REQUIRE((!is_bs16<KV>() || d % 16 == 0), "hgt_edge_forward_bs16: needs d %% 16 == 0 (d=%d)", d);
+  const size_t row_bytes = (size_t)kv_row_bytes<KV>(2 * (int64_t)d);
   const size_t slot_bytes = kvr ? 2 * row_bytes : row_bytes;
   if (variant == 0) variant = 2;
   const bool two_ctas = vec * nch <= 4;
   if (variant == 2) {
     const size_t budget = two_ctas ? 100 * 1024 : 200 * 1024;
     int stages = (int)(budget / (kWarpsPerCta * slot_bytes));
-    if (stages > 8) stages = 8;
+    const int max_stages = is_bs16<KV>() ? 12 : 8;
+    if (stages > max_stages) stages = max_stages;
     if (stages < 2 || row_bytes % 16 != 0) variant = 1;
     else {
       p.stages = stages;
diff --git a/pyhgt_b200/csrc/layer.cu b/pyhgt_b200/csrc/layer.cu
--- a/pyhgt_b200/csrc/layer.cu
+++ b/pyhgt_b200/csrc/layer.cu
@@ -27,7 +27,9 @@
   void *kv, *kvr;
   void *g_hi, *g_lo, *ws_proj, *ws_edge, *ws_upd;
   size_t ws_proj_bytes, ws_edge_bytes, ws_upd_bytes, total;
-  bool fuse_split, presplit_x, t24;
+  size_t row_bytes;
+  int32_t fmt;
+  bool fuse_split, presplit_x;
 };
 
 int plan_layout(const hgt_conv_args* a, void* base, Layout* L) {
@@ -43,15 +45,20 @@
   L->x_sorted = a->perm ? c.take<float>((size_t)N * din) : nullptr;
   L->w_cat = c.take<float>((size_t)(a->cat_rows > 0 ? a->cat_rows : 1) * din);
   L->b_cat = c.take<float>((size_t)(a->cat_rows > 0 ? a->cat_rows : 1));
-  L->t24 = d % 8 == 0;
-  if (L->t24) {
+  int dev = 0, l2 = 0;
+  HGT_CHECK_CUDA(cudaGetDevice(&dev));
+  HGT_CHECK_CUDA(cudaDeviceGetAttribute(&l2, cudaDevAttrL2CacheSize, dev));
+  int rc = hgt_gather_table_format(d, a->kv_rows + 1, l2, &L->fmt);
+  int64_t rbytes = 0;
+  if (rc || (rc = hgt_gather_table_row_bytes(L->fmt, 2 * (int64_t)d, &rbytes))) return rc;
+  const size_t row_bytes = L->row_bytes = (size_t)rbytes;
+  if (L->fmt != HGT_TABLE_F32) {
     L->proj = c.take<float>((size_t)a->kv_off);
-    L->kv = c.take_bytes((size_t)(a->kv_rows + 1) * 6 * d);
+    L->kv = c.take_bytes((size_t)(a->kv_rows + 1) * row_bytes);
   } else {
     L->proj = c.take<float>((size_t)a->proj_elems);
     L->kv = base ? L->proj + a->kv_off : nullptr;
   }
-  int rc;
   if (L->presplit_x)
     rc = hgt_typed_linear_presplit_workspace_bytes(a->h_proj_groups, a->n_proj_groups, din, d, &L->ws_proj_bytes);
   else
@@ -62,7 +69,7 @@
   L->kvr = nullptr;
   if (a->use_rte) {
     L->rt = c.take<float>((size_t)HGT_RTE_MAX_LEN * din);
-    L->kvr = c.take_bytes(((size_t)a->n_pairs * HGT_RTE_MAX_LEN + 1) * 2 * d * (L->t24 ? 3 : 4));
+    L->kvr = c.take_bytes(((size_t)a->n_pairs * HGT_RTE_MAX_LEN + 1) * row_bytes);
   }
   if ((rc = hgt_edge_workspace_bytes(a->n_split, d, a->n_heads, &L->ws_edge_bytes))) return rc;
   L->ws_edge = c.take_bytes(L->ws_edge_bytes);
@@ -89,6 +96,21 @@
 
 }
 
+extern "C" int hgt_gather_table_format(int32_t d, int64_t table_rows, int64_t l2_bytes, int32_t* out_format) {
+  HGT_REQUIRE(out_format, "hgt_gather_table_format: out_format is NULL");
+  if (d % 128 == 0 && table_rows * 6 * (int64_t)d > l2_bytes) *out_format = HGT_TABLE_BS16;
+  else *out_format = d % 8 == 0 ? HGT_TABLE_T24 : HGT_TABLE_F32;
+  return 0;
+}
+
+extern "C" int hgt_gather_table_row_bytes(int32_t format, int64_t n, int64_t* out_bytes) {
+  HGT_REQUIRE(out_bytes, "hgt_gather_table_row_bytes: out_bytes is NULL");
+  HGT_REQUIRE(format == HGT_TABLE_F32 || format == HGT_TABLE_T24 || format == HGT_TABLE_BS16,
+              "hgt_gather_table_row_bytes: unknown format %d", format);
+  *out_bytes = format == HGT_TABLE_BS16 ? hgt_bs16_row_bytes(n) : n * (format == HGT_TABLE_T24 ? 3 : 4);
+  return 0;
+}
+
 extern "C" uint64_t hgt_conv_args_size(void) { return sizeof(hgt_conv_args); }
 
 extern "C" int hgt_conv_workspace_bytes(const hgt_conv_args* a, size_t* out_bytes) {
@@ -124,10 +146,19 @@
                              a->relation_pri, T, a->num_relations, a->n_heads, din, d, P, a->pair_type, a->pair_rel,
                              a->cat_row0, a->q_row0, L.w_cat, L.b_cat, stream)))
     return rc;
-  const size_t row_bytes = (size_t)2 * d * (L.t24 ? 3 : 4);
+  const size_t row_bytes = L.row_bytes;
   HGT_CHECK_CUDA(cudaMemsetAsync(static_cast<char*>(L.kv) + a->kv_rows * row_bytes, 0, row_bytes, st));
   const void* x_lo = a->linear_impl == 3 ? nullptr : a->x_lo;
-  if (L.t24) {
+  if (L.fmt == HGT_TABLE_BS16) {
+    if (L.presplit_x)
+      rc = hgt_typed_linear_presplit_bs16(a->x_hi, x_lo, L.w_cat, L.b_cat, din, d, a->proj_groups, a->h_proj_groups,
+                                          a->n_proj_groups, a->proj_cblocks, L.proj, a->kv_off, L.kv, L.ws_proj,
+                                          L.ws_proj_bytes + 256, stream);
+    else
+      rc = hgt_typed_linear_bs16(x_sorted, din, L.w_cat, L.b_cat, din, d, a->proj_groups, a->h_proj_groups,
+                                 a->n_proj_groups, a->proj_cblocks, L.proj, a->kv_off, L.kv, a->linear_impl, L.ws_proj,
+                                 L.ws_proj_bytes + 256, stream);
+  } else if (L.fmt == HGT_TABLE_T24) {
     if (L.presplit_x)
       rc = hgt_typed_linear_presplit_t24(a->x_hi, x_lo, L.w_cat, L.b_cat, din, d, a->proj_groups, a->h_proj_groups,
                                          a->n_proj_groups, a->proj_cblocks, L.proj, a->kv_off, L.kv, L.ws_proj,
@@ -149,15 +180,25 @@
                                a->rt_cblocks, L.rt, 1, nullptr, 0, stream)))
       return rc;
     HGT_CHECK_CUDA(cudaMemsetAsync(static_cast<char*>(L.kvr) + (int64_t)P * HGT_RTE_MAX_LEN * row_bytes, 0, row_bytes, st));
-    rc = L.t24 ? hgt_typed_linear_t24(L.rt, din, L.w_cat, nullptr, din, d, a->rte_groups, a->h_rte_groups,
-                                      a->n_rte_groups, a->rte_cblocks, nullptr, 0, L.kvr, 1, nullptr, 0, stream)
-               : hgt_typed_linear(L.rt, din, L.w_cat, nullptr, din, d, a->rte_groups, a->h_rte_groups, a->n_rte_groups,
-                                  a->rte_cblocks, static_cast<float*>(L.kvr), 1, nullptr, 0, stream);
+    if (L.fmt == HGT_TABLE_BS16)
+      rc = hgt_typed_linear_bs16(L.rt, din, L.w_cat, nullptr, din, d, a->rte_groups, a->h_rte_groups, a->n_rte_groups,
+                                 a->rte_cblocks, nullptr, 0, L.kvr, 1, nullptr, 0, stream);
+    else if (L.fmt == HGT_TABLE_T24)
+      rc = hgt_typed_linear_t24(L.rt, din, L.w_cat, nullptr, din, d, a->rte_groups, a->h_rte_groups, a->n_rte_groups,
+                                a->rte_cblocks, nullptr, 0, L.kvr, 1, nullptr, 0, stream);
+    else
+      rc = hgt_typed_linear(L.rt, din, L.w_cat, nullptr, din, d, a->rte_groups, a->h_rte_groups, a->n_rte_groups,
+                            a->rte_cblocks, static_cast<float*>(L.kvr), 1, nullptr, 0, stream);
     if (rc) return rc;
   }
   const int32_t* dst_rows = a->type_active ? a->type_active : a->type_dst;
   const int32_t* rte_row = a->use_rte ? a->rte_row : nullptr;
-  if (L.t24)
+  if (L.fmt == HGT_TABLE_BS16)
+    rc = hgt_edge_forward_bs16(L.proj + a->q_off, L.kv, L.kvr, a->row_ptr, a->kv_row, rte_row, a->csr_eid, a->tiles,
+                               a->n_tiles, a->n_split, a->hubs, a->n_hubs, N, a->n_edges, d, a->n_heads, 1, L.g_act,
+                               a->att, nullptr, L.g_hi, L.g_lo, L.ws_edge, L.ws_edge_bytes, a->edge_variant,
+                               a->d_tile_counts, a->type_row0, T, dst_rows, stream);
+  else if (L.fmt == HGT_TABLE_T24)
     rc = hgt_edge_forward_t24(L.proj + a->q_off, L.kv, L.kvr, a->row_ptr, a->kv_row, rte_row, a->csr_eid, a->tiles,
                               a->n_tiles, a->n_split, a->hubs, a->n_hubs, N, a->n_edges, d, a->n_heads, 1, L.g_act,
                               a->att, nullptr, L.g_hi, L.g_lo, L.ws_edge, L.ws_edge_bytes, a->edge_variant,
diff --git a/pyhgt_b200/csrc/linear.cu b/pyhgt_b200/csrc/linear.cu
--- a/pyhgt_b200/csrc/linear.cu
+++ b/pyhgt_b200/csrc/linear.cu
@@ -15,6 +15,10 @@
 int hgt_typed_linear_tc(const float* A, int64_t lda, const float* W, const float* bias, int32_t K,
                         int32_t cb_width, const hgt_lin_group* groups, const hgt_lin_group* h_groups,
                         int32_t n_groups, const hgt_lin_cblock* cblocks, float* out32, int64_t t24_off, hgt_t24* out,
+                        int32_t products, void* workspace, size_t workspace_bytes, cudaStream_t st);
+int hgt_typed_linear_tc(const float* A, int64_t lda, const float* W, const float* bias, int32_t K,
+                        int32_t cb_width, const hgt_lin_group* groups, const hgt_lin_group* h_groups,
+                        int32_t n_groups, const hgt_lin_cblock* cblocks, float* out32, int64_t t24_off, hgt_bs16* out,
                         int32_t products, void* workspace, size_t workspace_bytes, cudaStream_t st);
 int hgt_typed_linear_tc_bf16a(const __nv_bfloat16* A, int64_t lda, const float* W, const float* bias, int32_t K,
                               int32_t cb_width, const hgt_lin_group* groups, const hgt_lin_group* h_groups,
@@ -166,7 +170,8 @@
     for (int j = 0; j < 4; ++j)
       if (tn * 4 + j < cols_here) bj[j] = bias[w_row0 + tn * 4 + j];
   }
-  if (std::is_same<OutT, hgt_t24>::value && cblk.out_off < t24_off) {
+  constexpr bool table = std::is_same<OutT, hgt_t24>::value || std::is_same<OutT, hgt_bs16>::value;
+  if (table && cblk.out_off < t24_off) {
     float* Og = out32 + cblk.out_off + m0 * cblk.ld + n0;
 #pragma unroll
     for (int i = 0; i < 8; ++i) {
@@ -193,6 +198,26 @@
           *reinterpret_cast<uint16_t*>(e.hi + r * rb + 2 * c) = (uint16_t)(w >> 16);
           e.lo[r * rb + c] = (unsigned char)(w >> 8);
         }
+      }
+    }
+  } else if constexpr (std::is_same<OutT, hgt_bs16>::value) {
+    const hgt_bs16_at e(out, cblk.out_off - t24_off + m0 * cblk.ld + n0, cblk.ld);
+    const int64_t rb = hgt_bs16_row_bytes(cblk.ld);
+    const int lane = tid & 31;
+#pragma unroll
+    for (int i = 0; i < 8; ++i) {
+      const int r = tm * 8 + i, c = tn * 4;
+      float v[4];
+#pragma unroll
+      for (int j = 0; j < 4; ++j) v[j] = acc[i][j] + bj[j];
+      const uint32_t a = hgt_bs16_quad_amax(max(max(hgt_abs_bits(v[0]), hgt_abs_bits(v[1])),
+                                                max(hgt_abs_bits(v[2]), hgt_abs_bits(v[3]))));
+      float rc;
+      const uint32_t sb = hgt_bs16_scale(a, rc);
+      if (r < rows_here && c < cols_here) {
+        *reinterpret_cast<uint2*>(e.m + r * rb + 2 * c) =
+            make_uint2(hgt_bs16_pack(v[0], v[1], rc, sb), hgt_bs16_pack(v[2], v[3], rc, sb));
+        if ((lane & 3) == 0) *reinterpret_cast<uint16_t*>(e.s + r * rb + 2 * (c / 16)) = (uint16_t)sb;
       }
     }
   } else {
@@ -291,7 +316,7 @@
     if constexpr (std::is_same<AT, __nv_bfloat16>::value)
       return hgt_typed_linear_tc_bf16a(A, lda, W, bias, K, cb_width, groups, h_groups, n_groups, cblocks, out,
                                        impl == 3 ? 1 : 3, workspace, workspace_bytes, st);
-    else if constexpr (std::is_same<OutT, hgt_t24>::value)
+    else if constexpr (std::is_same<OutT, hgt_t24>::value || std::is_same<OutT, hgt_bs16>::value)
       return hgt_typed_linear_tc(A, lda, W, bias, K, cb_width, groups, h_groups, n_groups, cblocks, out32, t24_off, out,
                                  impl == 3 ? 1 : 3, workspace, workspace_bytes, st);
     else
@@ -342,6 +367,15 @@
                       impl, workspace, workspace_bytes, (cudaStream_t)stream_, out, t24_off);
 }
 
+extern "C" int hgt_typed_linear_bs16(const float* A, int64_t lda, const float* W, const float* bias, int32_t K,
+                                     int32_t cb_width, const hgt_lin_group* groups, const hgt_lin_group* h_groups,
+                                     int32_t n_groups, const hgt_lin_cblock* cblocks, float* out, int64_t t24_off,
+                                     void* out16, int32_t impl, void* workspace, size_t workspace_bytes, void* stream_) {
+  HGT_REQUIRE(cb_width % 16 == 0, "hgt_typed_linear_bs16: needs cb_width %% 16 == 0 (cb_width=%d)", cb_width);
+  return typed_linear(A, lda, W, bias, K, cb_width, groups, h_groups, n_groups, cblocks, static_cast<hgt_bs16*>(out16),
+                      impl, workspace, workspace_bytes, (cudaStream_t)stream_, out, t24_off);
+}
+
 extern "C" int hgt_typed_linear_bf16a(const void* A, int64_t lda, const float* W, const float* bias, int32_t K,
                                       int32_t cb_width, const hgt_lin_group* groups, const hgt_lin_group* h_groups,
                                       int32_t n_groups, const hgt_lin_cblock* cblocks, float* out, int32_t impl,
diff --git a/pyhgt_b200/csrc/linear_tc.cu b/pyhgt_b200/csrc/linear_tc.cu
--- a/pyhgt_b200/csrc/linear_tc.cu
+++ b/pyhgt_b200/csrc/linear_tc.cu
@@ -89,6 +89,16 @@
       lo[i] = (unsigned char)l[i];
     }
   }
+}
+
+__device__ __forceinline__ void store4_bs16(unsigned char* m, unsigned char* s, float4 v, bool store, int lane) {
+  const uint32_t a = hgt_bs16_quad_amax(max(max(hgt_abs_bits(v.x), hgt_abs_bits(v.y)),
+                                            max(hgt_abs_bits(v.z), hgt_abs_bits(v.w))));
+  float r;
+  const uint32_t sb = hgt_bs16_scale(a, r);
+  if (!store) return;
+  *reinterpret_cast<uint2*>(m) = make_uint2(hgt_bs16_pack(v.x, v.y, r, sb), hgt_bs16_pack(v.z, v.w, r, sb));
+  if ((lane & 3) == 0) *reinterpret_cast<uint16_t*>(s) = (uint16_t)sb;
 }
 
 template <class OutT, bool AF = false>
@@ -138,6 +148,12 @@
       const hgt_t24_at e(out, off - t24_off, cblk.ld);
       t.hi = e.hi;
       t.lo = e.lo;
+    } else if constexpr (is_bs16<OutT>()) {
+      const int64_t off = cblk.out_off + m0 * cblk.ld + n0;
+      t.out32 = cblk.out_off < t24_off ? out32 + off : nullptr;
+      const hgt_bs16_at e(out, off - t24_off, cblk.ld);
+      t.hi = e.m;
+      t.lo = e.s;
     } else {
       t.out = out + cblk.out_off + m0 * cblk.ld + n0;
     }
@@ -214,6 +230,27 @@
       store_staged<BN>(acc, stage, c, wq, lane, pair, [&](int r, int col, float4 v) {
         if (r < rows && col < cols) store4_t24(hi + r * rb + 2 * col, lo + r * rb + col, v, vec4);
       });
+    } else if constexpr (is_bs16<OutT>()) {
+      if (t.out32) {
+        if (fwd_tma_store<BN>() && wq == 0 && lane == 0) bulk_wait_read<0>();
+        store_plain<BN>(t, t.out32, acc, stage, c, wq, lane, pair);
+        return;
+      }
+      const int64_t rows = t.rows - 64 * c;
+      const int64_t rb = hgt_bs16_row_bytes(t.ld);
+      unsigned char* m = t.hi + 64 * c * rb;
+      unsigned char* sc = t.lo + 64 * c * rb;
+      if constexpr (fwd_tma_store<BN>()) {
+        if (((reinterpret_cast<uintptr_t>(m) | reinterpret_cast<uintptr_t>(sc)) & 15) == 0 && cols >= BN) {
+          store_tma<BN, OutT>(acc, reinterpret_cast<unsigned char*>(stage), c, wq, lane, pair, t.map, t.n0,
+                              t.m0 + 64 * c, cols);
+          return;
+        }
+        if (wq == 0 && lane == 0) bulk_wait_read<0>();
+      }
+      store_staged<BN>(acc, stage, c, wq, lane, pair, [&](int r, int col, float4 v) {
+        store4_bs16(m + r * rb + 2 * col, sc + r * rb + 2 * (col / 16), v, r < rows && col < cols, lane);
+      });
     } else {
       store_plain<BN>(t, t.out, acc, stage, c, wq, lane, pair);
     }
@@ -251,7 +288,7 @@
     const hgt_lin_cblock cblk = cblocks[grp.cb_first + cb];
     CUtensorMap* m = maps + out_maps_per_block<OutT>() * (first.v[blockIdx.x] + cb);
     if (grp.m <= 0) continue;
-    if (is_t24<OutT>() && cblk.out_off < t24_off) {
+    if (is_table<OutT>() && cblk.out_off < t24_off) {
       const float* base = out32 + cblk.out_off;
       const uint64_t stride = (uint64_t)cblk.ld * 4;
       if (((reinterpret_cast<uintptr_t>(base) | stride) & 15) != 0) continue;
@@ -262,6 +299,12 @@
       if (((reinterpret_cast<uintptr_t>(e.hi) | reinterpret_cast<uintptr_t>(e.lo) | stride) & 15) != 0) continue;
       put_map(m, tmpl, e.hi, grp.m, stride);
       put_map(m + 1, tmpl_lo, e.lo, grp.m, stride);
+    } else if constexpr (is_bs16<OutT>()) {
+      const hgt_bs16_at e(out, cblk.out_off - t24_off, cblk.ld);
+      const uint64_t stride = (uint64_t)hgt_bs16_row_bytes(cblk.ld);
+      if (((reinterpret_cast<uintptr_t>(e.m) | reinterpret_cast<uintptr_t>(e.s)) & 15) != 0) continue;
+      put_map(m, tmpl, e.m, grp.m, stride);
+      put_map(m + 1, tmpl_lo, e.s, grp.m, stride);
     } else {
       OutT* base = out + cblk.out_off;
       const uint64_t stride = (uint64_t)cblk.ld * sizeof(OutT);
@@ -323,18 +366,20 @@
   return A && (reinterpret_cast<uintptr_t>(A) & 15) == 0 && lda % 4 == 0;
 }
 
-int make_out_template(CUtensorMap* m, void* dummy, int cb_width, int elem) {
+int make_out_template(CUtensorMap* m, void* dummy, int cb_width, int elem, int scale_box = 0) {
   EncodeTiledFn fn = get_encode_fn();
   HGT_REQUIRE(fn != nullptr, "hgt_typed_linear: cuTensorMapEncodeTiled not available from the driver");
-  cuuint64_t dims[2] = {(cuuint64_t)cb_width, 64};
-  cuuint64_t strides[1] = {(cuuint64_t)hgt_align_up((size_t)cb_width * elem, 16)};
-  cuuint32_t box[2] = {elem == 1 ? 64u : 128 / (cuuint32_t)elem, 64};
+  const int cols = scale_box ? cb_width / 16 : cb_width;
+  cuuint64_t dims[2] = {(cuuint64_t)cols, 64};
+  cuuint64_t strides[1] = {(cuuint64_t)hgt_align_up((size_t)cols * elem, 16)};
+  cuuint32_t box[2] = {scale_box ? (cuuint32_t)scale_box : elem == 1 ? 64u : 128 / (cuuint32_t)elem, 64};
   cuuint32_t estr[2] = {1, 1};
   const CUtensorMapDataType type = elem == 4 ? CU_TENSOR_MAP_DATA_TYPE_FLOAT32
                                    : elem == 2 ? CU_TENSOR_MAP_DATA_TYPE_BFLOAT16 : CU_TENSOR_MAP_DATA_TYPE_UINT8;
   CUresult r = fn(m, type, 2, dummy, dims, strides, box, estr, CU_TENSOR_MAP_INTERLEAVE_NONE,
-                  elem == 1 ? CU_TENSOR_MAP_SWIZZLE_64B : CU_TENSOR_MAP_SWIZZLE_128B, CU_TENSOR_MAP_L2_PROMOTION_NONE,
-                  CU_TENSOR_MAP_FLOAT_OOB_FILL_NONE);
+                  scale_box ? CU_TENSOR_MAP_SWIZZLE_NONE
+                            : elem == 1 ? CU_TENSOR_MAP_SWIZZLE_64B : CU_TENSOR_MAP_SWIZZLE_128B,
+                  CU_TENSOR_MAP_L2_PROMOTION_NONE, CU_TENSOR_MAP_FLOAT_OOB_FILL_NONE);
   HGT_REQUIRE(r == CUDA_SUCCESS, "hgt_typed_linear: cuTensorMapEncodeTiled (output) failed (%d) cb_width=%d", (int)r,
               cb_width);
   return 0;
@@ -384,11 +429,11 @@
     CUtensorMap tmpl, tmpl_lo, tmpl_f32;
     MapFirst first;
     void* dummy = const_cast<CUtensorMap*>(job.out_maps);
-    if ((rc = make_out_template(&tmpl, dummy, job.cb_width, is_t24<OutT>() ? 2 : (int)sizeof(OutT)))) return rc;
+    if ((rc = make_out_template(&tmpl, dummy, job.cb_width, is_table<OutT>() ? 2 : (int)sizeof(OutT)))) return rc;
     tmpl_lo = tmpl_f32 = tmpl;
-    if (is_t24<OutT>() && ((rc = make_out_template(&tmpl_lo, dummy, job.cb_width, 1)) ||
-                           (rc = make_out_template(&tmpl_f32, dummy, job.cb_width, 4))))
-      return rc;
+    if (is_t24<OutT>() && (rc = make_out_template(&tmpl_lo, dummy, job.cb_width, 1))) return rc;
+    if (is_bs16<OutT>() && (rc = make_out_template(&tmpl_lo, dummy, job.cb_width, 2, BN / 16))) return rc;
+    if (is_table<OutT>() && (rc = make_out_template(&tmpl_f32, dummy, job.cb_width, 4))) return rc;
     for (int g = 0; g < job.n_groups; ++g) first.v[g] = job.map_first[g];
     k_out_maps<OutT><<<job.n_groups, 64, 0, st>>>(tmpl, tmpl_lo, tmpl_f32, job.groups, job.cblocks, job.out, job.out32,
                                                   job.t24_off, first, const_cast<CUtensorMap*>(job.out_maps));
@@ -518,6 +563,14 @@
                 workspace, workspace_bytes, st, out32, t24_off);
 }
 
+int hgt_typed_linear_tc(const float* A, int64_t lda, const float* W, const float* bias, int32_t K, int32_t cb_width,
+                        const hgt_lin_group* groups, const hgt_lin_group* h_groups, int32_t n_groups,
+                        const hgt_lin_cblock* cblocks, float* out32, int64_t t24_off, hgt_bs16* out,
+                        int32_t products, void* workspace, size_t workspace_bytes, cudaStream_t st) {
+  return tc_run(A, lda, nullptr, nullptr, W, bias, K, cb_width, groups, h_groups, n_groups, cblocks, out, products,
+                workspace, workspace_bytes, st, out32, t24_off);
+}
+
 extern "C" int hgt_typed_linear_presplit_workspace_bytes(const hgt_lin_group* h_groups, int32_t n_groups, int32_t K,
                                                          int32_t cb_width, size_t* out_bytes) {
   HGT_REQUIRE(out_bytes && (h_groups || n_groups == 0), "hgt_typed_linear_presplit_workspace_bytes: NULL argument");
@@ -574,6 +627,17 @@
                                              void* workspace, size_t workspace_bytes, void* stream_) {
   return typed_linear_presplit(a_hi, a_lo, W, bias, K, cb_width, groups, h_groups, n_groups, cblocks,
                                static_cast<hgt_t24*>(out24), workspace, workspace_bytes, (cudaStream_t)stream_, out,
+                               t24_off);
+}
+
+extern "C" int hgt_typed_linear_presplit_bs16(const void* a_hi, const void* a_lo, const float* W, const float* bias,
+                                              int32_t K, int32_t cb_width, const hgt_lin_group* groups,
+                                              const hgt_lin_group* h_groups, int32_t n_groups,
+                                              const hgt_lin_cblock* cblocks, float* out, int64_t t24_off, void* out16,
+                                              void* workspace, size_t workspace_bytes, void* stream_) {
+  HGT_REQUIRE(cb_width % 16 == 0, "hgt_typed_linear_presplit_bs16: needs cb_width %% 16 == 0 (cb_width=%d)", cb_width);
+  return typed_linear_presplit(a_hi, a_lo, W, bias, K, cb_width, groups, h_groups, n_groups, cblocks,
+                               static_cast<hgt_bs16*>(out16), workspace, workspace_bytes, (cudaStream_t)stream_, out,
                                t24_off);
 }
 
diff --git a/pyhgt_b200/csrc/tc_ptx.cuh b/pyhgt_b200/csrc/tc_ptx.cuh
--- a/pyhgt_b200/csrc/tc_ptx.cuh
+++ b/pyhgt_b200/csrc/tc_ptx.cuh
@@ -303,42 +303,76 @@
 }
 
 template <class OutT> constexpr bool is_t24() { return std::is_same<OutT, hgt_t24>::value; }
-template <class OutT> constexpr int out_maps_per_block() { return is_t24<OutT>() ? 2 : 1; }
+template <class OutT> constexpr bool is_bs16() { return std::is_same<OutT, hgt_bs16>::value; }
+template <class OutT> constexpr bool is_table() { return is_t24<OutT>() || is_bs16<OutT>(); }
+template <class OutT> constexpr int out_maps_per_block() { return is_table<OutT>() ? 2 : 1; }
 
 template <int BN, class OutT, class Pair>
 __device__ __forceinline__ void store_tma(const float* acc, unsigned char* stage, int c, int wq, int lane, Pair pair,
                                           const CUtensorMap* map, int col0, int row0, int cols) {
   static_assert(BN % 128 == 0, "the two buffers alternate across tiles only for an even number of 64-column blocks");
-  constexpr bool T24 = is_t24<OutT>();
-  constexpr int BOX_COLS = T24 ? 64 : 128 / (int)sizeof(OutT);
+  constexpr bool T24 = is_t24<OutT>(), BS16 = is_bs16<OutT>();
+  constexpr int BOX_COLS = T24 || BS16 ? 64 : 128 / (int)sizeof(OutT);
   const bool issuer = wq == 0 && lane == 0;
   const int r0 = 16 * wq + (lane >> 2), c0 = 2 * (lane & 3);
   if (issuer) {
     tensormap_acquire(map);
-    if constexpr (T24) tensormap_acquire(map + 1);
-  }
+    if constexpr (T24 || BS16) tensormap_acquire(map + 1);
+  }
+  unsigned char* const scale_box = stage + 8192;
 #pragma unroll
   for (int blk = 0; blk < BN / 64; ++blk) {
     unsigned char* buf = stage + (blk & 1) * TMA_BUF_BYTES;
-    if (issuer) bulk_wait_read<1>();
+    if (issuer) {
+      if (BS16 && blk == 0) bulk_wait_read<0>();
+      else bulk_wait_read<1>();
+    }
     bar_sync_named(1 + c, 128);
-#pragma unroll
-    for (int j = 8 * blk; j < 8 * blk + 8; ++j) {
+    if constexpr (BS16) {
 #pragma unroll
       for (int h = 0; h < 2; ++h) {
-        const int r = r0 + 8 * h, lc = 8 * j + c0 - 64 * blk;
-        const float2 v = pair(r, 8 * j + c0, acc[4 * j + 2 * h], acc[4 * j + 2 * h + 1]);
-        if constexpr (T24) {
-          uint32_t hi, lo;
-          t24_pair(v, hi, lo);
-          const uint32_t x = (uint32_t)lc * 2;
-          *reinterpret_cast<uint32_t*>(buf + r * 128 + ((((x >> 4) ^ (r & 7)) << 4) | (x & 15))) = hi;
-          *reinterpret_cast<uint16_t*>(buf + 8192 + r * 64 + ((((lc >> 4) ^ ((r >> 1) & 3)) << 4) | (lc & 15))) =
-              (uint16_t)lo;
-        } else {
-          const uint32_t x = (uint32_t)(lc % BOX_COLS) * sizeof(OutT);
-          put2(reinterpret_cast<OutT*>(buf + (lc / BOX_COLS) * 8192 + r * 128 + ((((x >> 4) ^ (r & 7)) << 4) | (x & 15))),
-               v);
+        const int r = r0 + 8 * h;
+        uint32_t sc[4];
+#pragma unroll
+        for (int k = 0; k < 4; ++k) {
+          const int j = 8 * blk + 2 * k;
+          const float2 v0 = pair(r, 8 * j + c0, acc[4 * j + 2 * h], acc[4 * j + 2 * h + 1]);
+          const float2 v1 = pair(r, 8 * j + 8 + c0, acc[4 * j + 4 + 2 * h], acc[4 * j + 4 + 2 * h + 1]);
+          const uint32_t a = hgt_bs16_quad_amax(max(max(hgt_abs_bits(v0.x), hgt_abs_bits(v0.y)),
+                                                    max(hgt_abs_bits(v1.x), hgt_abs_bits(v1.y))));
+          float rc;
+          sc[k] = hgt_bs16_scale(a, rc);
+#pragma unroll
+          for (int u = 0; u < 2; ++u) {
+            const float2 v = u ? v1 : v0;
+            const uint32_t x = (uint32_t)(16 * k + 8 * u + c0) * 2;
+            *reinterpret_cast<uint32_t*>(buf + r * 128 + ((((x >> 4) ^ (r & 7)) << 4) | (x & 15))) =
+                hgt_bs16_pack(v.x, v.y, rc, sc[k]);
+          }
+        }
+        if ((lane & 3) == h)
+          *reinterpret_cast<uint2*>(scale_box + r * (BN / 8) + 8 * blk) =
+              make_uint2(sc[0] | (sc[1] << 16), sc[2] | (sc[3] << 16));
+      }
+    } else {
+#pragma unroll
+      for (int j = 8 * blk; j < 8 * blk + 8; ++j) {
+#pragma unroll
+        for (int h = 0; h < 2; ++h) {
+          const int r = r0 + 8 * h, lc = 8 * j + c0 - 64 * blk;
+          const float2 v = pair(r, 8 * j + c0, acc[4 * j + 2 * h], acc[4 * j + 2 * h + 1]);
+          if constexpr (T24) {
+            uint32_t hi, lo;
+            t24_pair(v, hi, lo);
+            const uint32_t x = (uint32_t)lc * 2;
+            *reinterpret_cast<uint32_t*>(buf + r * 128 + ((((x >> 4) ^ (r & 7)) << 4) | (x & 15))) = hi;
+            *reinterpret_cast<uint16_t*>(buf + 8192 + r * 64 + ((((lc >> 4) ^ ((r >> 1) & 3)) << 4) | (lc & 15))) =
+                (uint16_t)lo;
+          } else {
+            const uint32_t x = (uint32_t)(lc % BOX_COLS) * sizeof(OutT);
+            put2(reinterpret_cast<OutT*>(buf + (lc / BOX_COLS) * 8192 + r * 128 + ((((x >> 4) ^ (r & 7)) << 4) | (x & 15))),
+                 v);
+          }
         }
       }
     }
@@ -350,6 +384,8 @@
         if (64 * blk + BOX_COLS * bx < cols) tma_store_2d(map, s_u32(buf + bx * 8192), col0 + 64 * blk + BOX_COLS * bx, row0);
       if constexpr (T24)
         if (64 * blk < cols) tma_store_2d(map + 1, s_u32(buf + 8192), col0 + 64 * blk, row0);
+      if constexpr (BS16)
+        if (blk == BN / 64 - 1) tma_store_2d(map + 1, s_u32(scale_box), col0 / 16, row0);
       bulk_commit();
     }
   }
```
